# apache/arrow

Hardware: AMD Instinct MI355X
Metric: filter_take_mrows_per_s (higher is better)
Workload: dtype int64; 1 GPU; Filter+Take int64[1000000000] + validity (10% null), boolean mask 10% true, FilterOptions::DROP; take indices = the mask's row numbers (monotonic; indices_nonzero: uint64 through CallFunction, GetTakeIndices: uint32 in the mirror), no boundscheck; inputs = splitmix64 streams of SURVEY.md 8(d) (seeds 1,2,3); rows=1000000000, selected_rows=99992053, parallelism=single-gpu

## Files before the change

### arrow_amd/_lib.py

```python
from __future__ import annotations

import ctypes as C
import os

_HERE = os.path.dirname(os.path.abspath(__file__))
LIB_PATH = os.path.join(_HERE, "libarrow_amd.so")

ARX_OK = 0
ARX_OUT_OF_MEMORY = -1
ARX_INVALID = -4
ARX_CAPACITY_ERROR = -6
ARX_INDEX_ERROR = -7
ARX_NOT_IMPLEMENTED = -10
ARX_DEVICE_ERROR = -100

ABI_VERSION = 5

FILTER_DROP, FILTER_EMIT_NULL = 0, 1
SORT_ASCENDING, SORT_DESCENDING = 0, 1
NULLS_AT_START, NULLS_AT_END = 0, 1


class ArrowAmdError(Exception):
    """Base class; subclasses mirror pyarrow.lib.ArrowInvalid & friends."""


class ArrowInvalid(ArrowAmdError, ValueError):
    pass


class ArrowIndexError(ArrowAmdError, IndexError):
    pass


class ArrowCapacityError(ArrowAmdError):
    pass


class ArrowNotImplementedError(ArrowAmdError, NotImplementedError):
    pass


class ArrowDeviceError(ArrowAmdError, RuntimeError):
    pass


class ArrowMemoryError(ArrowAmdError, MemoryError):
    pass


_ERRORS = {
    ARX_INVALID: ArrowInvalid,
    ARX_CAPACITY_ERROR: ArrowCapacityError,
    ARX_INDEX_ERROR: ArrowIndexError,
    ARX_NOT_IMPLEMENTED: ArrowNotImplementedError,
    ARX_DEVICE_ERROR: ArrowDeviceError,
    ARX_OUT_OF_MEMORY: ArrowMemoryError,
}


class ArxSpan(C.Structure):

    _fields_ = [
        ("validity", C.c_void_p),
        ("data", C.c_void_p),
        ("offset", C.c_int64),
        ("length", C.c_int64),
        ("null_count", C.c_int64),
    ]


class ArxSortKeyWindow(C.Structure):

    _fields_ = [("key_min", C.c_uint64), ("shift", C.c_int32), ("reserved", C.c_int32)]


class ArxRangePlan(C.Structure):

    _fields_ = [("key_min", C.c_int32), ("width", C.c_int32), ("partitions", C.c_int32), ("reserved", C.c_int32),
                ("slots", C.c_int64), ("state_bytes", C.c_uint64), ("workspace_bytes", C.c_uint64)]


class ArxBinarySpan(C.Structure):

    _fields_ = [
        ("validity", C.c_void_p),
        ("offsets", C.c_void_p),
        ("data", C.c_void_p),
        ("offset", C.c_int64),
        ("length", C.c_int64),
        ("null_count", C.c_int64),
    ]


_p, _i64, _int, _u64, _u32, _sz = C.c_void_p, C.c_int64, C.c_int, C.c_uint64, C.c_uint32, C.c_size_t
_span = C.POINTER(ArxSpan)
_bspan = C.POINTER(ArxBinarySpan)

SIGNATURES = {
    "arx_last_error": (C.c_char_p, []),
    "arx_abi_version": (_int, []),
    "arx_device_count": (_int, []),
    "arx_set_option": (_int, [C.c_char_p, _i64]),
    "arx_get_option": (_int, [C.c_char_p, C.POINTER(_i64)]),
    "arx_get_counter": (_i64, [C.c_char_p]),
    "arx_filter_workspace_bytes": (_sz, [_i64]),
    "arx_filter_count": (_int, [_span, _int, _p, _sz, C.POINTER(_i64), _p]),
    "arx_filter_count_async": (_int, [_span, _int, _p, _sz, _p]),
    "arx_filter_count_nulls": (_int, [_span, _span, _int, _p, _sz, C.POINTER(_i64), C.POINTER(_i64), _p]),
    "arx_filter_exec": (_int, [_span, _int, _span, _int, _p, _i64, _p, _p, _p]),
    "arx_mask_to_indices": (_int, [_span, _int, _p, _i64, _int, _p, _p, _p]),
    "arx_filter_compact_form": (_int, [_int, _int, _int, _int, _i64, _i64]),
    "arx_take_workspace_bytes": (_sz, []),
    "arx_check_index_bounds": (_int, [_span, _int, _u64, _p, _sz, _p]),
    "arx_take": (_int, [_span, _int, _span, _int, _p, _p, _p, _p]),
    "arx_take_rows": (_int, [_span, _i64, _span, _int, _p, _p, _p, _p]),
    "arx_take_bits": (_int, [_span, _span, _int, _p, _p, _p, _p]),
    "arx_binary_take_workspace_bytes": (_sz, [_i64]),
    "arx_binary_take_offsets": (_int, [_bspan, _span, _int, _p, _sz, _p, _p, _p, C.POINTER(_i64), _p]),
    "arx_binary_take_data": (_int, [_bspan, _i64, _p, _sz, _p, _i64, _p, _p]),
    "arx_large_binary_take_workspace_bytes": (_sz, [_i64]),
    "arx_large_binary_take_offsets": (_int, [_bspan, _span, _int, _p, _sz, _p, _p, _p, C.POINTER(_i64), _p]),
    "arx_large_binary_take_data": (_int, [_bspan, _i64, _p, _sz, _p, _i64, _p, _p]),
    "arx_list_take_data": (_int, [_bspan, _int, _i64, _p, _sz, _p, _i64, _p, _p]),
    "arx_large_list_take_data": (_int, [_bspan, _int, _i64, _p, _sz, _p, _i64, _p, _p]),
    "arx_plain_byte_array_offsets": (_int, [_p, _sz, _i64, C.c_int32, _p]),
    "arx_rle_scan_runs": (_int, [_p, _sz, _int, _i64, _u32, _u64, _p, _i64, C.POINTER(_i64), C.POINTER(_i64)]),
    "arx_rle_decode_u32": (_int, [_p, _sz, _p, _i64, _int, _i64, _p, _p]),
    "arx_rle_decode_equals_bitmap": (_int, [_p, _sz, _p, _i64, _int, _i64, _u32, _p, _p]),
    "arx_expand_by_mask": (_int, [_p, _int, _span, _p, _p, _p]),
    "arx_rle_levels_to_bitmap": (_int, [_p, _p, _i64, _p, _p, _p, _p]),
    "arx_rle_scan_runs_equals": (_int, [_p, _sz, _int, _i64, _u32, _u32, _u64, _p, _i64, C.POINTER(_i64), C.POINTER(_i64)]),
    "arx_levels_to_list_workspace_bytes": (_sz, [_i64]),
    "arx_def_rep_levels_to_list": (_int, [_p, _p, _i64, _int, _int, _int, _i64, _p, _p, _p, _p, _sz, _p]),
    "arx_levels_ge_bitmap": (_int, [_p, _i64, _u32, _p, _p, _p]),
    "arx_lz4_decompress_streams": (_int, [_p, _p, _p, _i64, _p, _p, _p]),
    "arx_lz4_frame_scan": (_int, [_p, _sz, _u64, _p, _i64, C.POINTER(_i64), C.POINTER(_u64)]),
    "arx_bitmap_copy": (_int, [_p, _i64, _i64, _p, _p]),
    "arx_buffer_copy": (_int, [_p, _p, _i64, _p]),
    "arx_delta_scan_miniblocks": (_int, [_p, _sz, _u64, _p, _i64, C.POINTER(_i64), C.POINTER(_i64), C.POINTER(_i64),
                                         C.POINTER(_i64), C.POINTER(_sz)]),
    "arx_delta_decode_workspace_bytes": (_sz, [_i64]),
    "arx_delta_decode": (_int, [_p, _p, _i64, _i64, _i64, _i64, _int, _p, _sz, _p, _p]),
    "arx_lengths_to_offsets_i32": (_int, [_p, _i64, C.c_int32, _p, _p, _sz, _p]),
    "arx_byte_stream_split_decode": (_int, [_p, _i64, _int, _p, _p]),
    "arx_delta_byte_array_lengths": (_int, [_p, _p, _i64, _p, _i64, _p, _p, _p]),
    "arx_delta_byte_array_expand": (_int, [_p, _p, _p, _i64, _p, C.c_int32, _p, _p, _i64, _p, _p, _p]),
    "arx_bitmap_copy_at": (_int, [_p, _i64, _i64, _p, _i64, _p]),
    "arx_binary_rebase_offsets": (_int, [_p, _i64, C.c_int32, _p, _p]),
    "arx_bitmap_and": (_int, [_p, _i64, _p, _i64, _i64, _p, _p]),
    "arx_reduce_i64_init": (_int, [_p, _p]),
    "arx_reduce_i64_consume": (_int, [_span, _p, _p]),
    "arx_reduce_float_minmax": (_int, [_span, _int, _p, _p]),
    "arx_coalesce2": (_int, [_int, _span, _span, _p, _i64, _p, _p, _p]),
    "arx_sum_float_workspace_bytes": (_sz, [_i64, _i64]),
    "arx_sum_float": (_int, [_span, _int, _p, _sz, C.POINTER(C.c_double), C.POINTER(_i64), _p]),
    "arx_boolean_kleene": (_int, [_int, _span, _span, _p, _p, _p]),
    "arx_boolean_invert": (_int, [_p, _i64, _i64, _p, _p]),
    "arx_bitmap_popcount": (_int, [_p, _i64, _i64, _p, _sz, C.POINTER(_i64), _p]),
    "arx_bytes_to_bitmap": (_int, [_p, _i64, _p, _p, _p]),
    "arx_groupby_key_range_i32": (_int, [_span, _p, _p]),
    "arx_groupby_range_plan": (_int, [_i64, C.c_int32, C.c_int32, _p]),
    "arx_groupby_key_range_sampled_i32": (_int, [_span, _i64, _p, _p]),
    "arx_groupby_range_sum_i64_consume": (_int, [_p, _p, _span, _span, _p, _sz, _p]),
    "arx_groupby_range_merge": (_int, [_p, _p, C.c_int32, _i64, _int, _i64, _p]),
    "arx_groupby_range_finalize_workspace_bytes": (_sz, [_i64]),
    "arx_groupby_range_finalize": (_int, [_p, C.c_int32, C.c_int32, _i64, C.c_uint32, _p, _sz, _p, _p, _p, _p, _p, _p]),
    "arx_hash_bool_finalize": (_int, [_p, _p, _p, _i64, _int, _int, C.c_uint32, _p, _p, _p, _p]),
    "arx_sort_indices_workspace_bytes": (_sz, [_i64]),
    "arx_sort_partition_records_global": (_int, [_span, _int, _int, _int, _p, _p, _int, C.c_uint32, _p, _sz, _p, _p, _p]),
    "arx_sort_records": (_int, [_p, _i64, _p, _sz, _p, _p]),
    "arx_sort_indices": (_int, [_span, _int, _int, _int, _p, _sz, _p, _p]),
    "arx_rank_workspace_bytes": (_sz, [_i64]),
    "arx_rank": (_int, [_span, _int, _p, _int, _p, _sz, _p, _p]),
    "arx_sort_indices_64": (_int, [_span, _int, _int, _int, _p, _sz, _p, _p]),
    "arx_sort_key_histogram": (_int, [_span, _int, _int, _int, _p, _p]),
    "arx_sort_partition_by_bins": (_int, [_span, _int, _int, _int, _p, _int, _p, _sz, _p, _p, _p,
                                          C.POINTER(_i64), _p]),
    "arx_bitmap_to_indices": (_int, [_p, _i64, _i64, _int, _p, _sz, _p, C.POINTER(_i64), _p]),
    "arx_sort_partition_records": (_int, [_span, _int, _int, _int, _int, _p, _int, _p, _sz, _p, _p, C.POINTER(_i64), _p]),
    "arx_sort_key_range": (_int, [_span, _int, _int, _p, _p]),
    "arx_sort_key_histogram_window": (_int, [_span, _int, _int, _int, _p, _p, _p]),
    "arx_sort_key_range_sampled": (_int, [_span, _int, _int, _int, _p, _p]),
    "arx_sort_key_histogram_window_sampled": (_int, [_span, _int, _int, _int, _p, _int, _p, _p]),
    "arx_sort_partition_records_window": (_int, [_span, _int, _int, _int, _int, _p, _p, _int, _p, _sz, _p, _p,
                                                 C.POINTER(_i64), _p]),
    "arx_sort_unpack_records": (_int, [_p, _i64, _p, _int, _int, _p, _p, _p, _p]),
    "arx_groupby_export_partitioned": (_int, [_p, _int, _p, _sz, _p, _p, _p]),
    "arx_groupby_partials_capacity": (_i64, [_i64, _i64, _int]),
    "arx_groupby_sum_i64_consume_partials": (_int, [_p, _i64, _span, _span, _p, _sz, _int, _p, _i64, _p, _p]),
    "arx_groupby_partition_rows": (_int, [_span, _span, _int, _p, _sz, _p, _p, _p]),
    "arx_groupby_unpack_rows": (_int, [_p, _i64, _p, _p, _p, _p, _p]),
    "arx_hash_sum_consume_workspace_bytes": (_sz, [_i64, _i64]),
    "arx_hash_sum_i64_consume_ws": (_int, [_span, _int, _i64, _p, _i64, _i64, _p, _p, _p, _p, _sz, _p]),
    "arx_hash_mean_i64_finalize": (_int, [_p, _p, _i64, C.c_uint64, _p, _p, _p]),
    "arx_compare_numeric": (_int, [_int, _int, _p, _p, _p, _p, _i64, _p, _p]),
    "arx_arith_numeric": (_int, [_int, _int, _int, _p, _p, _p, _i64, _p, _p, _p, _i64, _i64, _p, _p, _p]),
    "arx_divide_numeric": (_int, [_int, _int, _p, _p, _p, _i64, _p, _p, _p, _i64, _i64, _p, _p, _p]),
    "arx_delta_decode_pages": (_int, [_p, _p, _p, _i64, _i64, _int, _p, _sz, _p, _p]),
    "arx_copy_segments": (_int, [_p, _i64, _u64, _p]),
    "arx_bitmap_copy_segments": (_int, [_p, _i64, _i64, _p]),
    "arx_take_columns": (_int, [_p, _p, _int, _span, _int, _p, _p, _p, _p]),
    "arx_grouper_state_bytes": (_sz, [_i64]),
    "arx_grouper_init": (_int, [_p, _i64, _p]),
    "arx_grouper_consume_workspace_bytes": (_sz, [_i64]),
    "arx_grouper_consume": (_int, [_p, _i64, _p, _p, _int, _p, _sz, _p, _p]),
    "arx_grouper_lookup": (_int, [_p, _i64, _p, _p, _int, _p, _sz, _p, _p, _p]),
    "arx_grouper_num_groups": (_int, [_p, _p, _p]),
    "arx_group_ids_skip_group": (_int, [_p, _i64, _u32, _p]),
    "arx_grouper_get_uniques": (_int, [_p, _i64, _p, _int, _int, _p, _p, _p, _p]),
    "arx_binary_key_lengths": (_int, [_bspan, _p, _p, _p, _p]),
    "arx_binary_key_chunk": (_int, [_bspan, _i64, _p, _p, _p]),
    "arx_binary_sort_chunk": (_int, [_bspan, _i64, _p, _p]),
    "arx_binary_key_hash": (_int, [_bspan, _int, _p, _p]),
    "arx_set_lookup_state_bytes": (_sz, [_i64, _int]),
    "arx_set_lookup_build": (_int, [_p, _span, _int, _p]),
    "arx_set_lookup_build_binary": (_int, [_p, _bspan, _int, _int, _p]),
    "arx_set_lookup_is_in": (_int, [_p, _i64, _int, _span, _int, _p, _p]),
    "arx_set_lookup_index_in": (_int, [_p, _i64, _int, _span, _int, _p, _p, _p]),
    "arx_set_lookup_is_in_binary": (_int, [_p, _bspan, _int, _int, _bspan, _int, _int, _p, _p]),
    "arx_set_lookup_index_in_binary": (_int, [_p, _bspan, _int, _int, _bspan, _int, _int, _p, _p, _p]),
    "arx_match_substring": (_int, [_bspan, _int, _int, _p, _i64, _i64, _int, _p, _p]),
    "arx_string_length": (_int, [_bspan, _int, _int, _i64, _int, _p, _p]),
    "arx_string_slice_workspace_bytes": (_sz, [_i64, _int]),
    "arx_string_slice_offsets": (_int, [_bspan, _int, _int, _i64, _i64, _i64, _int, _p, _sz, _p, C.POINTER(_i64), _p]),
    "arx_string_slice_data": (_int, [_bspan, _int, _p, _sz, _p, _i64, _p, _p]),
    "arx_string_trim_offsets": (_int, [_bspan, _int, _int, _int, _p, _i64, _p, _sz, _p, C.POINTER(_i64), _p]),
    "arx_if_else": (_int, [_int, _span, _span, _p, _span, _p, _i64, _p, _p, _p]),
    "arx_temporal_component": (_int, [_int, _int, _span, _i64, _int, _int, _p, _p, _p]),
    "arx_hash_join_workspace_bytes": (_sz, [_i64]),
    "arx_hash_join_key_validity": (_int, [_span, _int, _i64, _p, _p]),
    "arx_hash_join_bool_key": (_int, [_span, _p, _p]),
    "arx_hash_join_group_offsets": (_int, [_p, _p, _i64, _i64, _p, _p, _sz, _p]),
    "arx_hash_join_probe_count": (_int, [_p, _p, _i64, _p, _i64, _int, _p, _i64, _p, _p, _sz, C.POINTER(_i64), _p]),
    "arx_hash_join_expand": (_int, [_p, _p, _p, _i64, _p, _p, _int, _i64, _p, _p, _p, _p]),
    "arx_hash_join_build_mask": (_int, [_p, _p, _i64, _p, _int, _p, _p]),
    "arx_hash_join_append_build_rows": (_int, [_p, _i64, _i64, _p, _p, _p, _p, _p]),
    "arx_hash_join_filter_count": (_int, [_span, _p, _p, _i64, _int, _p, _p, _i64, _p, _p, _p, _p, _sz, C.POINTER(_i64), _p]),
    "arx_hash_join_filter_compact": (_int, [_p, _p, _i64, _p, _p, _i64, _p, _p, _int, _i64, _p, _p, _p, _p]),
    "arx_hash_join_flags_to_mask": (_int, [_p, _i64, _int, _p, _p]),
    "arx_binary_key_verify": (_int, [_bspan, _p, _p, C.POINTER(_i64), _p, _p]),
    "arx_group_first_rows": (_int, [_p, _i64, _i64, _p, _p]),
    "arx_group_edge_rows": (_int, [_p, _p, _i64, _i64, _i64, _int, _p, _p, _p]),
    "arx_ree_bool_expand": (_int, [_p, _int, _i64, _span, _i64, _i64, _p, _p, _p]),
    "arx_snappy_decompress_pages": (_int, [_p, _p, _i64, _p, _p, _p]),
    "arx_gzip_decompress_pages": (_int, [_p, _p, _i64, _p, _p, _p]),
    "arx_cast_numeric": (_int, [_span, _int, _int, _int, _int, _p, _sz, _p, _p]),
    "arx_groupby_mean_i64_finalize": (_int, [_p, _p, _p, _p, _p, _i64, _int, _u32, _p, _p, _p, _p]),
    "arx_groupby_sum_i64_merge_records": (_int, [_p, _i64, _p, _i64, _p]),
    "arx_groupby_state_bytes": (_sz, [_i64]),
    "arx_groupby_init": (_int, [_p, _i64, _p]),
    "arx_groupby_consume_workspace_bytes": (_sz, [_i64, _i64]),
    "arx_groupby_sum_i64_consume": (_int, [_p, _i64, _span, _span, _p, _sz, _p]),
    "arx_groupby_sum_i64_merge": (_int, [_p, _i64, _p, _p, _p, _p, _p, _i64, _p]),
    "arx_groupby_num_groups": (_int, [_p, C.POINTER(_i64), _p]),
    "arx_groupby_sum_i64_export": (_int, [_p, _p, _p, _p, _p, _p, _p]),
    "arx_groupby_lookup_i32": (_int, [_p, _i64, _span, _p, _p]),
    "arx_groupby_minmax_bytes": (_sz, [_i64]),
    "arx_groupby_minmax_init": (_int, [_p, _i64, _p]),
    "arx_groupby_minmax_i64_consume": (_int, [_p, _p, _i64, _span, _span, _p]),
    "arx_groupby_export": (_int, [_p, _p, _p, _p, _p, _p, _p, _p, _p, _p]),
    "arx_groupby_minmax_merge": (_int, [_p, _p, _i64, _p, _p, _p, _p, _p, _i64, _p]),
    "arx_groupby_minmax_finalize": (_int, [_p, _p, _p, _i64, _int, _p, _p]),
    "arx_groupby_sum_i64_finalize": (_int, [_p, _p, _i64, _int, _u32, _p, _p]),
    "arx_hash_sum_i64_consume": (_int, [_span, _int, _i64, _p, _i64, _p, _p, _p, _p]),
    "arx_hash_sum_i64_merge": (_int, [_p, _p, _p, _p, _p, _p, _p, _i64, _p]),
    "arx_hash_sum_dec128_consume": (_int, [_span, _int, C.c_uint64, C.c_uint64, _p, _i64, _p, _p, _p, _p, _p]),
    "arx_hash_sum_dec128_merge": (_int, [_p, _p, _p, _p, _p, _p, _p, _p, _p, _i64, _p]),
# ... 61 lines not shown
```

### arrow_amd/csrc/arrow_plugin.cc

```cpp
#include <arrow/acero/exec_plan.h>
#include <arrow/acero/hash_join_node.h>
#include <arrow/acero/options.h>
#include <arrow/api.h>
#include <arrow/c/abi.h>
#include <arrow/c/bridge.h>
#include <arrow/c/dlpack_abi.h>
#include <arrow/compute/api.h>
#include <arrow/compute/initialize.h>
#include <arrow/compute/kernel.h>
#include <arrow/compute/registry.h>
#include <arrow/device.h>
#include <arrow/util/bit_util.h>
#include <arrow/util/bitmap_builders.h>
#include <arrow/util/bitmap_ops.h>
#include <arrow/acero/util.h>
#include <arrow/acero/query_context.h>

#include <hip/hip_runtime_api.h>
#include <parquet/column_page.h>
#include <parquet/column_reader.h>
#include <parquet/file_reader.h>
#include <parquet/metadata.h>
#include <parquet/schema.h>
#include <parquet/arrow/schema.h>
// ... 398 lines not shown
int64_t arrow_amd_plugin_sharded_sort_records_runs(void) { return g_sharded_sort_records_runs.load(); }
void arrow_amd_plugin_pool_stats(int64_t* cached_bytes, int64_t* hits, int64_t* misses) {
  DevicePool::Get().Stats(cached_bytes, hits, misses);
}
void arrow_amd_plugin_pool_trim(void) { DevicePool::Get().Trim(); }
int arrow_amd_parquet_read_column(const char* path, int row_group, int column, struct ArrowDeviceArray* out,
                                  struct ArrowSchema* out_schema) {
  auto run = [&]() -> Status {
    try {
      ARROW_ASSIGN_OR_RAISE(auto data, ParquetChunkToDevice(path, row_group, column));
      ARROW_RETURN_NOT_OK(arrow::ExportType(*data->type, out_schema));
      return arrow::ExportDeviceArray(*arrow::MakeArray(data), nullptr, out);
    } catch (const parquet::ParquetException& e) {
      return Status::IOError("Parquet: ", e.what());
    }
  };
  const Status st = run();
  if (!st.ok()) {
    t_error = st.ToString();
    return -1;
  }
  return 0;
}
int arrow_amd_parquet_read_field(const char* path, int row_group, int field, struct ArrowDeviceArray* out,
                                 struct ArrowSchema* out_schema) {
  auto run = [&]() -> Status {
    try {
      ARROW_ASSIGN_OR_RAISE(auto data, ParquetFieldToDevice(path, row_group, field));
      ARROW_RETURN_NOT_OK(arrow::ExportType(*data->type, out_schema));
      return arrow::ExportDeviceArray(*arrow::MakeArray(data), nullptr, out);
    } catch (const parquet::ParquetException& e) {
      return Status::IOError("Parquet: ", e.what());
    }
  };
  const Status st = run();
  if (!st.ok()) {
    t_error = st.ToString();
    return -1;
  }
  return 0;
}
namespace {
class ChunkWorkers {
 public:
  static ChunkWorkers& Get() {
#ifdef ARX_EMULATED_HIP_RUNTIME
    static ChunkWorkers* pool = new ChunkWorkers(1);
#else
    static ChunkWorkers* pool = new ChunkWorkers(4);
#endif
    return *pool;
  }
  void Run(int n, const std::function<void(int)>& fn) {
    std::unique_lock<std::mutex> lock(mu_);
    idle_.wait(lock, [&] { return !busy_; });
    busy_ = true;
    fn_ = &fn;
    next_ = 0;
    count_ = n;
    left_ = n;
    work_.notify_all();
    done_.wait(lock, [&] { return left_ == 0; });
    fn_ = nullptr;
    busy_ = false;
    idle_.notify_one();
  }

 private:
  explicit ChunkWorkers(int k) {
    for (int i = 0; i < k; ++i) std::thread([this] { Loop(); }).detach();
  }
  void Loop() {
    std::unique_lock<std::mutex> lock(mu_);
    for (;;) {
      work_.wait(lock, [&] { return fn_ != nullptr && next_ < count_; });
      const int i = next_++;
      const std::function<void(int)>* fn = fn_;
      lock.unlock();
      (*fn)(i);
      lock.lock();
      if (--left_ == 0) done_.notify_all();
    }
  }
  std::mutex mu_;
  std::condition_variable work_, done_, idle_;
  const std::function<void(int)>* fn_ = nullptr;
  int next_ = 0, count_ = 0, left_ = 0;
  bool busy_ = false;
};
}

int arrow_amd_parquet_read_columns(const char* path, int row_group, const int* columns, int num_columns,
                                   struct ArrowDeviceArray* outs, struct ArrowSchema* out_schemas) {
  if (path == nullptr || columns == nullptr || num_columns < 0 || (num_columns > 0 && (outs == nullptr || out_schemas == nullptr))) {
    t_error = "arrow_amd_parquet_read_columns: NULL argument";
    return -1;
  }
  std::vector<arrow::Result<std::shared_ptr<ArrayData>>> results(static_cast<size_t>(num_columns),
                                                                  arrow::Result<std::shared_ptr<ArrayData>>(Status::UnknownError("not run")));
  const std::string file(path);
  int device = 0;
  (void)hipGetDevice(&device);
  ChunkWorkers::Get().Run(num_columns, [&](int i) {
    (void)hipSetDevice(device);
    try {
      results[i] = ParquetChunkToDevice(file, row_group, columns[i]);
    } catch (const parquet::ParquetException& e) {
      results[i] = Status::IOError("Parquet: ", e.what());
    } catch (const std::exception& e) {
      results[i] = Status::UnknownError(e.what());
    }
  });
  for (int i = 0; i < num_columns; ++i) {
    if (!results[i].ok()) {
      t_error = results[i].status().ToString();
      return -1;
    }
  }
  int exported = 0;
  Status st;
  for (; exported < num_columns && st.ok(); ++exported) {
    const std::shared_ptr<ArrayData>& data = *results[exported];
    st = arrow::ExportType(*data->type, &out_schemas[exported]);
    if (st.ok()) {
      st = arrow::ExportDeviceArray(*arrow::MakeArray(data), nullptr, &outs[exported]);
      if (!st.ok() && out_schemas[exported].release != nullptr) out_schemas[exported].release(&out_schemas[exported]);
    }
  }
  if (!st.ok()) {
    for (int i = 0; i + 1 < exported; ++i) {
      if (outs[i].array.release != nullptr) outs[i].array.release(&outs[i].array);
      if (out_schemas[i].release != nullptr) out_schemas[i].release(&out_schemas[i]);
    }
    t_error = st.ToString();
    return -1;
  }
  return 0;
}
int64_t arrow_amd_plugin_acero_guard(int what) {
  return what == 1 ? g_guard_takeovers.load() : what == 2 ? g_guard_refusals.load() : (g_acero_guard_installed.load() ? 1 : 0);
}
int arrow_amd_override_acero_factories(int on) {
  const Status st = OverrideAceroFactories(on);
  if (!st.ok()) {
    t_error = st.ToString();
    return -1;
  }
  return 0;
}
void arrow_amd_plugin_set_min_rows(int64_t n) { g_min_rows.store(n); }
void arrow_amd_plugin_set_string_key_hash_bits(int64_t bits) { g_string_key_hash_bits.store(bits < 0 ? 0 : (bits > 64 ? 64 : bits)); }
int64_t arrow_amd_plugin_string_key_hash_collisions(void) { return g_string_key_hash_collisions.load(); }
void arrow_amd_plugin_set_filter_morsel_rows(int64_t n) { g_filter_morsel_rows.store(n); }
void arrow_amd_plugin_set_parquet_device_snappy(int on) { g_parquet_device_snappy.store(on != 0); }
void arrow_amd_plugin_set_parquet_device_levels(int on) { g_parquet_device_levels.store(on != 0); }
void arrow_amd_plugin_set_parquet_pinned_staging(int on) { g_parquet_pinned_staging.store(on != 0); }
void arrow_amd_plugin_set_parquet_read_threads(int n, int64_t min_part_bytes) {
  g_parquet_read_threads.store(n < 1 ? 1 : (n > 16 ? 16 : n));
  g_parquet_read_part_bytes.store(min_part_bytes < 4096 ? 4096 : min_part_bytes);
}
int64_t arrow_amd_plugin_parquet_device_snappy_pages(void) { return g_parquet_device_snappy_pages.load(); }
void arrow_amd_plugin_set_parquet_device_gzip(int on) { g_parquet_device_gzip.store(on != 0); }
int64_t arrow_amd_plugin_parquet_device_gzip_pages(void) { return g_parquet_device_gzip_pages.load(); }
int64_t arrow_amd_plugin_parquet_copied_pages(void) { return g_parquet_copied_pages.load(); }
void arrow_amd_plugin_set_aggregate_stage_nulls(int on) { g_aggregate_stage_nulls.store(on != 0); }
void arrow_amd_plugin_set_aggregate_flush_rows(int64_t rows) { g_aggregate_flush_rows.store(rows < 1 ? 1 : rows); }
int64_t arrow_amd_plugin_aggregate_flushes(void) { return g_aggregate_flushes.load(); }
void arrow_amd_plugin_set_aggregate_direct_rows(int64_t rows) { g_aggregate_direct_rows.store(rows < 1 ? 1 : rows); }
int64_t arrow_amd_plugin_aggregate_direct_batches(void) { return g_aggregate_direct_batches.load(); }
void arrow_amd_plugin_set_aggregate_range_state(int on) { g_aggregate_range_state.store(on != 0); }
void arrow_amd_plugin_set_aggregate_range_min_rows(int64_t rows) { g_aggregate_range_min_rows.store(rows < 1 ? 1 : rows); }
int64_t arrow_amd_plugin_aggregate_range_plans(void) { return g_aggregate_range_plans.load(); }
int64_t arrow_amd_plugin_aggregate_range_declined(void) { return g_aggregate_range_declined.load(); }
void arrow_amd_plugin_set_aggregate_device_output(int on) { g_aggregate_device_output.store(on != 0); }
void arrow_amd_plugin_set_results_kernel_copy(int on) { g_results_kernel_copy.store(on != 0); }
void arrow_amd_plugin_set_pinned_results(int on) { g_pinned_results.store(on != 0); }
void arrow_amd_plugin_set_coalesce_rows(int64_t rows) { g_coalesce_rows.store(rows < 1 ? 1 : rows); }
int64_t arrow_amd_plugin_coalesced_batches(void) { return g_coalesced_batches.load(); }
void arrow_amd_plugin_set_table_source_rows(int64_t rows) { g_table_source_rows.store(rows < 1 ? 1 : rows); }
void arrow_amd_plugin_set_min_rows_streaming(int64_t n) { g_min_rows_streaming.store(n); }

}
```

### arrow_amd/csrc/plugin/common.inc

```

std::atomic<int64_t> g_gpu_calls{0};
std::atomic<int64_t> g_stock_calls{0};
std::atomic<int64_t> g_min_rows{1 << 16};
std::atomic<int64_t> g_min_rows_streaming{INT64_MAX};
std::atomic<int64_t> g_filter_morsel_rows{[] {
  const char* env = std::getenv("ARROW_AMD_FILTER_MORSEL_ROWS");
  return env != nullptr ? static_cast<int64_t>(std::strtoll(env, nullptr, 10)) : int64_t(1) << 20;
}()};

std::atomic<bool> g_parquet_pinned_staging{true};
std::atomic<bool> g_parquet_device_levels{true};
std::atomic<int> g_parquet_read_threads{4};
std::atomic<int64_t> g_parquet_read_part_bytes{int64_t(1) << 23};
std::atomic<bool> g_parquet_device_snappy{[] {
  const char* env = std::getenv("ARROW_AMD_PARQUET_DEVICE_SNAPPY");
  return env == nullptr || std::strtoll(env, nullptr, 10) != 0;
}()};
std::atomic<int64_t> g_parquet_device_snappy_pages{0};
std::atomic<bool> g_parquet_device_gzip{true};
std::atomic<int64_t> g_parquet_device_gzip_pages{0};
std::atomic<int64_t> g_parquet_copied_pages{0};

std::atomic<int64_t> g_aggregate_flush_rows{[] {
  const char* env = std::getenv("ARROW_AMD_AGGREGATE_FLUSH_ROWS");
  return env != nullptr ? std::max<int64_t>(1, std::strtoll(env, nullptr, 10)) : int64_t(1) << 21;
}()};
std::atomic<int64_t> g_aggregate_direct_rows{int64_t(1) << 22};
std::atomic<int64_t> g_aggregate_direct_batches{0};
std::atomic<bool> g_aggregate_range_state{true};
std::atomic<int64_t> g_aggregate_range_min_rows{int64_t(1) << 22};
std::atomic<int64_t> g_aggregate_range_sample_rows{int64_t(1) << 20};
std::atomic<int64_t> g_aggregate_range_plans{0};
std::atomic<int64_t> g_aggregate_range_declined{0};
std::atomic<int64_t> g_select_k_min_rows{int64_t(1) << 22};
std::atomic<int64_t> g_select_k_threshold_runs{0};
std::atomic<bool> g_sharded_range_state{true};
std::atomic<int64_t> g_sharded_range_min_rows{int64_t(1) << 22};
std::atomic<int64_t> g_sharded_range_runs{0};
std::atomic<int64_t> g_sharded_range_declined{0};
std::atomic<bool> g_sharded_sort_records{true};
std::atomic<int> g_sharded_sort_sample_shift{4};
std::atomic<int64_t> g_sharded_sort_sample_min_rows{int64_t(1) << 20};
std::atomic<int64_t> g_sharded_sort_records_runs{0};
std::atomic<int64_t> g_coalesce_rows{int64_t(1) << 26};
std::atomic<int64_t> g_coalesced_batches{0};
std::atomic<int64_t> g_table_source_rows{int64_t(1) << 27};
std::atomic<bool> g_pinned_results{[] {
  const char* env = std::getenv("ARROW_AMD_PINNED_RESULTS");
  return env == nullptr || std::strtoll(env, nullptr, 10) != 0;
}()};
std::atomic<bool> g_results_kernel_copy{true};
std::atomic<bool> g_aggregate_device_output{false};
std::atomic<bool> g_aggregate_stage_nulls{true};
std::atomic<int64_t> g_aggregate_flushes{0};
std::atomic<int64_t> g_string_key_hash_bits{64};
std::atomic<int64_t> g_string_key_hash_collisions{0};

enum Fn { kFnFilter = 0, kFnTake, kFnGreater, kFnSort, kFnCast, kFnHashSum, kFnAdd, kFnBoolean, kFnCompare, kFnParquet,
          kFnReduce, kFnOrderBy, kFnTakeColumns, kFnUnique, kFnCoalesce, kFnIsIn, kFnIndexIn, kFnHashJoin,
          kFnMatchSubstring, kFnStartsWith, kFnEndsWith, kFnIfElse, kFnYear, kFnQuarter, kFnMonth, kFnDay, kFnDayOfWeek,
          kFnDayOfYear, kFnIsoYear, kFnIsoWeek, kFnHour, kFnMinute, kFnSecond, kFnMillisecond, kFnMicrosecond, kFnNanosecond,
          kFnBinaryLength, kFnUtf8Length, kFnBinarySlice, kFnUtf8SliceCodeunits, kFnAsciiTrimWhitespace, kFnAsciiLtrimWhitespace,
          kFnAsciiRtrimWhitespace, kFnUtf8TrimWhitespace, kFnUtf8LtrimWhitespace, kFnUtf8RtrimWhitespace, kFnAsciiTrim, kFnAsciiLtrim,
          kFnAsciiRtrim, kFnUtf8Trim, kFnUtf8Ltrim, kFnUtf8Rtrim, kNumFn };
const char* const kFnNames[kNumFn] = {"array_filter", "array_take", "greater", "array_sort_indices",
                                      "cast", "hash_sum", "add", "boolean", "compare", "parquet", "reduce", "order_by",
                                      "take_columns", "unique", "coalesce", "is_in", "index_in", "hashjoin",
                                      "match_substring", "starts_with", "ends_with", "if_else", "year", "quarter", "month", "day",
                                      "day_of_week", "day_of_year", "iso_year", "iso_week", "hour", "minute", "second",
                                      "millisecond", "microsecond", "nanosecond", "binary_length", "utf8_length", "binary_slice",
                                      "utf8_slice_codeunits", "ascii_trim_whitespace", "ascii_ltrim_whitespace",
                                      "ascii_rtrim_whitespace", "utf8_trim_whitespace", "utf8_ltrim_whitespace",
                                      "utf8_rtrim_whitespace", "ascii_trim", "ascii_ltrim", "ascii_rtrim", "utf8_trim", "utf8_ltrim",
                                      "utf8_rtrim"};
std::atomic<int64_t> g_fn_gpu[kNumFn];
std::atomic<int64_t> g_fn_stock[kNumFn];
void CountGpu(Fn f) {
  g_gpu_calls.fetch_add(1, std::memory_order_relaxed);
  g_fn_gpu[f].fetch_add(1, std::memory_order_relaxed);
}
void CountStock(Fn f) {
  g_stock_calls.fetch_add(1, std::memory_order_relaxed);
  g_fn_stock[f].fetch_add(1, std::memory_order_relaxed);
}
thread_local std::string t_error;

Status FromArx(int rc) {
  if (rc == ARX_OK) return Status::OK();
  const std::string msg = arx_last_error();
  switch (rc) {
    case ARX_INVALID: return Status::Invalid(msg);
    case ARX_CAPACITY_ERROR: return Status::CapacityError(msg);
    case ARX_INDEX_ERROR: return Status::IndexError(msg);
    case ARX_NOT_IMPLEMENTED: return Status::NotImplemented(msg);
    case ARX_OUT_OF_MEMORY: return Status::OutOfMemory(msg);
    default: return Status::UnknownError(msg);
  }
}

#define HIP_RETURN_NOT_OK(call)                                                        \
  do {                                                                                 \
    hipError_t e__ = (call);                                                           \
    if (e__ != hipSuccess)                                                             \
      return Status::IOError("HIP: ", hipGetErrorString(e__), " in " #call);           \
  } while (0)

thread_local hipStream_t t_stream = nullptr;

class DeviceScratch {
 public:
  ~DeviceScratch() {
    for (auto& s : slots_) {
      if (s.ptr) (void)hipFree(s.ptr);
    }
  }
  hipStream_t PeekStream() const { return stream_; }
  Status Stream(hipStream_t* out) {
    if (!stream_) {
      HIP_RETURN_NOT_OK(hipStreamCreateWithFlags(&stream_, hipStreamNonBlocking));
      t_stream = stream_;
    }
    *out = stream_;
    return Status::OK();
  }
  Status Get(int slot, size_t bytes, void** out) {
    if (slots_.size() <= static_cast<size_t>(slot)) slots_.resize(slot + 1);
    Slot& s = slots_[slot];
    bytes = (bytes + 255) & ~size_t(255);
    if (s.size < bytes) {
      if (s.ptr) HIP_RETURN_NOT_OK(hipFree(s.ptr));
      s.ptr = nullptr;
      s.size = 0;
      const size_t want = std::max<size_t>(bytes + bytes / 4, 1 << 20);
      HIP_RETURN_NOT_OK(hipMalloc(&s.ptr, want));
      s.size = want;
    }
    *out = s.ptr;
    return Status::OK();
  }

 private:
  struct Slot { void* ptr = nullptr; size_t size = 0; };
  std::vector<Slot> slots_;
  hipStream_t stream_ = nullptr;
};
thread_local DeviceScratch t_scratch;

class PinnedStaging {
 public:
  ~PinnedStaging() {
    if (ptr_) (void)hipHostFree(ptr_);
  }
  Status Reserve(size_t bytes, uint8_t** out) {
    if (size_ < bytes) {
      if (ptr_) HIP_RETURN_NOT_OK(hipHostFree(ptr_));
      ptr_ = nullptr;
      size_ = 0;
      const size_t want = std::max<size_t>(bytes + bytes / 4, size_t(1) << 20);
      HIP_RETURN_NOT_OK(hipHostMalloc(&ptr_, want, hipHostMallocDefault));
      size_ = want;
    }
    *out = static_cast<uint8_t*>(ptr_);
    return Status::OK();
  }
  void Trim(size_t keep_at_most) {
    if (size_ > keep_at_most && ptr_ != nullptr) {
      (void)hipHostFree(ptr_);
      ptr_ = nullptr;
      size_ = 0;
    }
  }

 private:
  void* ptr_ = nullptr;
  size_t size_ = 0;
};
thread_local PinnedStaging t_pinned;

enum Slot { kValues = 0, kValidity, kArg2, kArg2Validity, kOutData, kOutValidity, kWs, kCounter, kBinWs, kFlag };

Status Upload(const ArraySpan& a, int byte_width_or_0_for_bool, int data_slot, int validity_slot,
              hipStream_t st, ArxSpan* out) {
  const int64_t o8 = a.offset % 8;
  const int64_t first = a.offset - o8;
  out->offset = o8;
  out->length = a.length;
  out->null_count = a.null_count;
  out->validity = nullptr;
  out->data = nullptr;
  const int64_t span_elems = o8 + a.length;
  if (a.buffers[1].data != nullptr && a.length > 0) {
    const uint8_t* src;
    size_t bytes;
    if (byte_width_or_0_for_bool == 0) {
      src = a.buffers[1].data + first / 8;
      bytes = static_cast<size_t>(arrow::bit_util::BytesForBits(span_elems));
    } else {
      src = a.buffers[1].data + first * byte_width_or_0_for_bool;
      bytes = static_cast<size_t>(span_elems) * byte_width_or_0_for_bool;
    }
    void* d = nullptr;
    ARROW_RETURN_NOT_OK(t_scratch.Get(data_slot, bytes + 16, &d));
    HIP_RETURN_NOT_OK(hipMemcpyAsync(d, src, bytes, hipMemcpyHostToDevice, st));
    out->data = d;
  }
  if (a.buffers[0].data != nullptr && a.null_count != 0 && a.length > 0) {
    const size_t bytes = static_cast<size_t>(arrow::bit_util::BytesForBits(span_elems));
    void* d = nullptr;
    ARROW_RETURN_NOT_OK(t_scratch.Get(validity_slot, bytes + 16, &d));
    HIP_RETURN_NOT_OK(hipMemcpyAsync(d, a.buffers[0].data + first / 8, bytes, hipMemcpyHostToDevice, st));
    out->validity = d;
  } else if (a.null_count != 0 && a.buffers[0].data == nullptr) {
    out->null_count = 0;
  }
  return Status::OK();
}

bool IsHost(const ArraySpan& a) {
  for (int i = 0; i < 2; ++i) {
    if (a.buffers[i].owner != nullptr && *a.buffers[i].owner != nullptr &&
        !(*a.buffers[i].owner)->is_cpu()) {
      return false;
    }
  }
  return true;
}

int FixedByteWidth(const arrow::DataType& t) {
  switch (t.id()) {
    case Type::INT8: case Type::UINT8: return 1;
    case Type::INT16: case Type::UINT16: case Type::HALF_FLOAT: return 2;
    case Type::INT32: case Type::UINT32: case Type::FLOAT: case Type::DATE32: case Type::TIME32:
    case Type::INTERVAL_MONTHS: case Type::DECIMAL32: return 4;
    case Type::INT64: case Type::UINT64: case Type::DOUBLE: case Type::DATE64: case Type::TIME64:
    case Type::TIMESTAMP: case Type::DURATION: case Type::INTERVAL_DAY_TIME: case Type::DECIMAL64: return 8;
    case Type::DECIMAL128: case Type::INTERVAL_MONTH_DAY_NANO: return 16;
    case Type::DECIMAL256: return 32;
    case Type::FIXED_SIZE_BINARY: {
      const int w = static_cast<const arrow::FixedSizeBinaryType&>(t).byte_width();
      return (w == 1 || w == 2 || w == 4 || w == 8 || w == 16 || w == 32) ? w : 0;
    }
    default: return 0;
  }
}

int BinaryOffsetWidth(Type::type id) { return (id == Type::LARGE_STRING || id == Type::LARGE_BINARY) ? 8 : 4; }

template <typename Options>
struct ShimState : public cp::KernelState {
  std::unique_ptr<cp::KernelState> stock;
  Options options;
};

struct StockKernel {
  cp::KernelInit init;
  cp::ArrayKernelExec exec = nullptr;
  cp::VectorKernel::ChunkedExec exec_chunked = nullptr;
};

template <class Exec, class Batch, class Out>
Status RunStock(Fn fn, Exec exec, std::optional<cp::KernelState*> stock_state, cp::KernelContext* ctx, const Batch& batch,
                Out* out) {
  CountStock(fn);
  if (!stock_state.has_value()) return exec(ctx, batch, out);
  cp::KernelState* mine = ctx->state();
  ctx->SetState(*stock_state);
  Status st = exec(ctx, batch, out);
  ctx->SetState(mine);
  return st;
}
Status RunStock(Fn fn, const StockKernel& k, cp::KernelState* stock_state, cp::KernelContext* ctx,
                const cp::ExecSpan& batch, cp::ExecResult* out) {
  return RunStock(fn, k.exec, std::optional<cp::KernelState*>(stock_state), ctx, batch, out);
}
```

### arrow_amd/csrc/plugin/selection.inc

```
StockKernel g_stock_filter;

arrow::Result<std::unique_ptr<cp::KernelState>> FilterInit(cp::KernelContext* ctx,
                                                           const cp::KernelInitArgs& args) {
  auto state = std::make_unique<ShimState<cp::FilterOptions>>();
  if (g_stock_filter.init) {
    ARROW_ASSIGN_OR_RAISE(state->stock, g_stock_filter.init(ctx, args));
  }
  if (args.options != nullptr) {
    state->options = *static_cast<const cp::FilterOptions*>(args.options);
  }
  return state;
}

Status BooleanTakeOnDevice(const ArxSpan& dv, const ArxSpan& di, int tid, hipStream_t st, ArrayData* out_arr) {
  const int64_t m = di.length;
  const int64_t bytes = ((m + 63) / 64) * 8;
  const bool allocate_validity = dv.null_count != 0 || di.null_count != 0;
  out_arr->length = m;
  out_arr->buffers.resize(2);
  out_arr->buffers[0] = nullptr;
  ARROW_ASSIGN_OR_RAISE(out_arr->buffers[1], AllocDevice(bytes));
  void* d_valid = nullptr;
  void* d_counter = nullptr;
  if (allocate_validity) {
    ARROW_ASSIGN_OR_RAISE(out_arr->buffers[0], AllocDevice(bytes));
    d_valid = reinterpret_cast<void*>(out_arr->buffers[0]->mutable_address());
    ARROW_RETURN_NOT_OK(t_scratch.Get(kCounter, 64, &d_counter));
    HIP_RETURN_NOT_OK(hipMemsetAsync(d_counter, 0, 8, st));
  }
  ARROW_RETURN_NOT_OK(FromArx(arx_take_bits(&dv, &di, tid, reinterpret_cast<void*>(out_arr->buffers[1]->mutable_address()),
                                            d_valid, static_cast<int64_t*>(d_counter), st)));
  int64_t valid_count = m;
  if (allocate_validity) HIP_RETURN_NOT_OK(hipMemcpyAsync(&valid_count, d_counter, 8, hipMemcpyDeviceToHost, st));
  HIP_RETURN_NOT_OK(hipStreamSynchronize(st));
  out_arr->null_count = m - valid_count;
  return Status::OK();
}

bool ReeFilterOnRocm(const ArraySpan& filter) {
  return filter.type->id() == Type::RUN_END_ENCODED && filter.child_data.size() == 2 &&
         OnRocm(filter.child_data[0]) && OnRocm(filter.child_data[1]);
}
Status ExpandReeFilterOnDevice(const ArraySpan& filter, hipStream_t st, ArxSpan* dm) {
  const ArraySpan& run_ends = filter.child_data[0];
  const ArraySpan& run_values = filter.child_data[1];
  const int rw = FixedByteWidth(*run_ends.type);
  if (run_values.type->id() != Type::BOOL || (rw != 2 && rw != 4 && rw != 8)) {
    return Status::NotImplemented("arrow_amd: filter of type ", filter.type->ToString());
  }
  ArxSpan ends{}, vals{};
  ARROW_RETURN_NOT_OK(DeviceSpan(run_ends, &ends));
  ARROW_RETURN_NOT_OK(DeviceSpan(run_values, &vals));
  const int64_t n = filter.length;
  const size_t bytes = static_cast<size_t>((n + 63) / 64) * 8 + 64;
  void *d_bits = nullptr, *d_valid = nullptr;
  ARROW_RETURN_NOT_OK(t_scratch.Get(kArg2, bytes, &d_bits));
  const bool may_have_nulls = vals.validity != nullptr && vals.null_count != 0;
  if (may_have_nulls) ARROW_RETURN_NOT_OK(t_scratch.Get(kArg2Validity, bytes, &d_valid));
  ARROW_RETURN_NOT_OK(FromArx(arx_ree_bool_expand(static_cast<const uint8_t*>(ends.data) + ends.offset * rw, rw, run_ends.length,
                                                  &vals, filter.offset, n, d_bits, d_valid, st)));
  *dm = ArxSpan{d_valid, d_bits, 0, n, may_have_nulls ? arrow::kUnknownNullCount : 0};
  return Status::OK();
}

Status FilterExec(cp::KernelContext* ctx, const cp::ExecSpan& batch, cp::ExecResult* out) {
  auto* state = static_cast<ShimState<cp::FilterOptions>*>(ctx->state());
  const ArraySpan& values = batch[0].array;
  const ArraySpan& filter = batch[1].array;
  const int w = FixedByteWidth(*values.type);
  const int null_sel = state->options.null_selection_behavior == cp::FilterOptions::EMIT_NULL
                           ? ARX_FILTER_EMIT_NULL : ARX_FILTER_DROP;
  const bool ree = filter.type->id() == Type::RUN_END_ENCODED;
  const bool on_device = OnRocm(values) || OnRocm(filter) || (ree && ReeFilterOnRocm(filter));
  if (on_device && ree && (!OnRocm(values) || !ReeFilterOnRocm(filter))) {
    return Status::NotImplemented("arrow_amd: a run-end encoded filter and its values must both be device-resident");
  }
  if (on_device) {
    if (values.type->id() == Type::BOOL && ree) {
      return Status::NotImplemented("arrow_amd: run-end encoded filter of boolean values on device-resident arrays");
    }
    if (values.type->id() == Type::BOOL && filter.type->id() == Type::BOOL) {
      if (filter.length > 0xFFFFFFFFll) {
        return Status::NotImplemented("Filter length exceeds UINT32_MAX, consider a different strategy for selecting elements");
      }
      hipStream_t st;
      ARROW_RETURN_NOT_OK(t_scratch.Stream(&st));
      ArxSpan dv{}, dm{};
      ARROW_RETURN_NOT_OK(DeviceSpan(values, &dv));
      ARROW_RETURN_NOT_OK(DeviceSpan(filter, &dm));
      const size_t ws_bytes = arx_filter_workspace_bytes(filter.length);
      void* ws = nullptr;
      ARROW_RETURN_NOT_OK(t_scratch.Get(kWs, ws_bytes, &ws));
      int64_t out_len = 0;
      ARROW_RETURN_NOT_OK(FromArx(arx_filter_count(&dm, null_sel, ws, ws_bytes, &out_len, st)));
      const bool emit = null_sel == ARX_FILTER_EMIT_NULL && dm.null_count != 0;
      void* d_idx = nullptr;
      void* d_idx_valid = nullptr;
      ARROW_RETURN_NOT_OK(t_scratch.Get(kArg2, static_cast<size_t>(out_len) * 4 + 64, &d_idx));
      if (emit) ARROW_RETURN_NOT_OK(t_scratch.Get(kArg2Validity, static_cast<size_t>((out_len + 63) / 64) * 8 + 64, &d_idx_valid));
      ARROW_RETURN_NOT_OK(FromArx(arx_mask_to_indices(&dm, null_sel, ws, out_len, 4, d_idx, d_idx_valid, st)));
      ArxSpan di{d_idx_valid, d_idx, 0, out_len, emit ? arrow::kUnknownNullCount : 0};
      ARROW_RETURN_NOT_OK(BooleanTakeOnDevice(dv, di, ARX_UINT32, st, out->array_data().get()));
      CountGpu(kFnFilter);
      return Status::OK();
    }
    if (w == 0 || (filter.type->id() != Type::BOOL && !ree)) {
      return Status::NotImplemented("arrow_amd: filter of ", values.type->ToString(),
                                    " on device-resident arrays");
    }
    hipStream_t st;
    ARROW_RETURN_NOT_OK(t_scratch.Stream(&st));
    ArxSpan dv{}, dm{};
    ARROW_RETURN_NOT_OK(DeviceSpan(values, &dv));
    if (ree) {
      ARROW_RETURN_NOT_OK(ExpandReeFilterOnDevice(filter, st, &dm));
    } else {
      ARROW_RETURN_NOT_OK(DeviceSpan(filter, &dm));
    }
    const size_t ws_bytes = arx_filter_workspace_bytes(filter.length);
    void* ws = nullptr;
    ARROW_RETURN_NOT_OK(t_scratch.Get(kWs, ws_bytes, &ws));
    ArrayData* out_arr = out->array_data().get();
    const bool allocate_validity = dv.null_count != 0 || dm.null_count != 0;
    if (filter.length > 0 && filter.length <= g_filter_morsel_rows.load()) {
      const int64_t n = filter.length;
      ARROW_RETURN_NOT_OK(FromArx(arx_filter_count_async(&dm, null_sel, ws, ws_bytes, st)));
      out_arr->buffers.resize(2);
      ARROW_ASSIGN_OR_RAISE(out_arr->buffers[1], AllocDevice(n * w));
      out_arr->buffers[0] = nullptr;
      void* d_valid = nullptr;
      if (allocate_validity) {
        ARROW_ASSIGN_OR_RAISE(out_arr->buffers[0], AllocDevice(((n + 63) / 64) * 8));
        d_valid = reinterpret_cast<void*>(out_arr->buffers[0]->mutable_address());
      }
      ARROW_RETURN_NOT_OK(FromArx(arx_filter_exec(&dv, w, &dm, null_sel, ws, n,
                                                  reinterpret_cast<void*>(out_arr->buffers[1]->mutable_address()),
                                                  d_valid, st)));
      int64_t selected = 0, set_bits = 0;
      HIP_RETURN_NOT_OK(hipMemcpyAsync(&selected, ws, 8, hipMemcpyDeviceToHost, st));
      if (allocate_validity) {
        void* cws = nullptr;
        ARROW_RETURN_NOT_OK(t_scratch.Get(kCounter, 64, &cws));
        ARROW_RETURN_NOT_OK(FromArx(arx_bitmap_popcount(d_valid, 0, n, cws, 64, &set_bits, st)));
      } else {
        HIP_RETURN_NOT_OK(hipStreamSynchronize(st));
      }
      out_arr->length = selected;
      out_arr->null_count = allocate_validity ? selected - set_bits : 0;
      static_cast<RocmBuffer*>(out_arr->buffers[1].get())->Shrink(selected * w);
      if (allocate_validity) static_cast<RocmBuffer*>(out_arr->buffers[0].get())->Shrink(((selected + 63) / 64) * 8);
      CountGpu(kFnFilter);
      return Status::OK();
    }
    int64_t out_len = 0, out_nulls = 0;
    if (allocate_validity) {
      ARROW_RETURN_NOT_OK(FromArx(arx_filter_count_nulls(&dv, &dm, null_sel, ws, ws_bytes, &out_len, &out_nulls, st)));
    } else {
      ARROW_RETURN_NOT_OK(FromArx(arx_filter_count(&dm, null_sel, ws, ws_bytes, &out_len, st)));
    }
    out_arr->length = out_len;
    out_arr->buffers.resize(2);
    ARROW_ASSIGN_OR_RAISE(out_arr->buffers[1], AllocDevice(out_len * w));
    out_arr->buffers[0] = nullptr;
    void* d_valid = nullptr;
    if (allocate_validity) {
      ARROW_ASSIGN_OR_RAISE(out_arr->buffers[0], AllocDevice(((out_len + 63) / 64) * 8));
      d_valid = reinterpret_cast<void*>(out_arr->buffers[0]->mutable_address());
    }
    ARROW_RETURN_NOT_OK(FromArx(arx_filter_exec(&dv, w, &dm, null_sel, ws, out_len,
                                                reinterpret_cast<void*>(out_arr->buffers[1]->mutable_address()),
                                                d_valid, st)));
    out_arr->null_count = allocate_validity ? out_nulls : 0;
    HIP_RETURN_NOT_OK(hipStreamSynchronize(st));
    CountGpu(kFnFilter);
    return Status::OK();
  }
  if (w == 0 || filter.type->id() != Type::BOOL || values.length < g_min_rows.load() ||
      !IsHost(values) || !IsHost(filter)) {
    return RunStock(kFnFilter, g_stock_filter, state->stock.get(), ctx, batch, out);
  }
  hipStream_t st;
  ARROW_RETURN_NOT_OK(t_scratch.Stream(&st));
  ArxSpan dv{}, dm{};
  ARROW_RETURN_NOT_OK(Upload(values, w, kValues, kValidity, st, &dv));
  ARROW_RETURN_NOT_OK(Upload(filter, 0, kArg2, kArg2Validity, st, &dm));
  const size_t ws_bytes = arx_filter_workspace_bytes(filter.length);
  void* ws = nullptr;
  ARROW_RETURN_NOT_OK(t_scratch.Get(kWs, ws_bytes, &ws));
  int64_t out_len = 0;
  ARROW_RETURN_NOT_OK(FromArx(arx_filter_count(&dm, null_sel, ws, ws_bytes, &out_len, st)));

  ArrayData* out_arr = out->array_data().get();
  const bool filter_null_count_is_zero = filter.null_count == 0;
  if (values.null_count == 0 && (null_sel == ARX_FILTER_DROP || filter_null_count_is_zero)) {
    out_arr->null_count = 0;
  } else {
    out_arr->null_count = arrow::kUnknownNullCount;
  }
  const bool allocate_validity = values.null_count != 0 || !filter_null_count_is_zero;
  out_arr->length = out_len;
  out_arr->buffers.resize(2);
  ARROW_ASSIGN_OR_RAISE(out_arr->buffers[1], ctx->Allocate(out_len * w));
  void* d_out = nullptr;
  void* d_out_valid = nullptr;
  ARROW_RETURN_NOT_OK(t_scratch.Get(kOutData, static_cast<size_t>(out_len) * w + 16, &d_out));
  const size_t vbytes = static_cast<size_t>((out_len + 63) / 64) * 8;
  if (allocate_validity) {
    ARROW_ASSIGN_OR_RAISE(out_arr->buffers[0], ctx->AllocateBitmap(out_len));
    ARROW_RETURN_NOT_OK(t_scratch.Get(kOutValidity, vbytes + 16, &d_out_valid));
  } else {
    out_arr->buffers[0] = nullptr;
  }
  ARROW_RETURN_NOT_OK(FromArx(arx_filter_exec(&dv, w, &dm, null_sel, ws, out_len, d_out, d_out_valid, st)));
  if (out_len > 0) {
    HIP_RETURN_NOT_OK(hipMemcpyAsync(out_arr->buffers[1]->mutable_data(), d_out,
                                     static_cast<size_t>(out_len) * w, hipMemcpyDeviceToHost, st));
    if (allocate_validity) {
      HIP_RETURN_NOT_OK(hipMemcpyAsync(out_arr->buffers[0]->mutable_data(), d_out_valid,
                                       static_cast<size_t>(arrow::bit_util::BytesForBits(out_len)),
                                       hipMemcpyDeviceToHost, st));
    }
  }
  HIP_RETURN_NOT_OK(hipStreamSynchronize(st));
  CountGpu(kFnFilter);
  return Status::OK();
}

int IndexTypeId(const arrow::DataType& t);

StockKernel g_stock_filter_bin, g_stock_take_bin, g_stock_filter_large_bin, g_stock_take_large_bin;

arrow::Result<std::unique_ptr<cp::KernelState>> BinaryFilterInit(cp::KernelContext* ctx,
                                                                 const cp::KernelInitArgs& args) {
  auto state = std::make_unique<ShimState<cp::FilterOptions>>();
  const bool large_in = !args.inputs.empty() && args.inputs[0].type != nullptr && BinaryOffsetWidth(args.inputs[0].type->id()) == 8;
  const StockKernel& stock_k = large_in ? g_stock_filter_large_bin : g_stock_filter_bin;
  if (stock_k.init) {
    ARROW_ASSIGN_OR_RAISE(state->stock, stock_k.init(ctx, args));
  }
  if (args.options != nullptr) state->options = *static_cast<const cp::FilterOptions*>(args.options);
  return state;
}

arrow::Result<std::unique_ptr<cp::KernelState>> BinaryTakeInit(cp::KernelContext* ctx,
                                                               const cp::KernelInitArgs& args) {
  auto state = std::make_unique<ShimState<cp::TakeOptions>>();
  const bool large_in = !args.inputs.empty() && args.inputs[0].type != nullptr && BinaryOffsetWidth(args.inputs[0].type->id()) == 8;
  const StockKernel& stock_k = large_in ? g_stock_take_large_bin : g_stock_take_bin;
  if (stock_k.init) {
    ARROW_ASSIGN_OR_RAISE(state->stock, stock_k.init(ctx, args));
  }
  if (args.options != nullptr) state->options = *static_cast<const cp::TakeOptions*>(args.options);
  return state;
}

Status CheckBoundsOnDevice(const ArxSpan& indices, int index_type, int64_t values_length, hipStream_t st) {
  void* ws = nullptr;
  ARROW_RETURN_NOT_OK(t_scratch.Get(kWs, arx_take_workspace_bytes(), &ws));
  return FromArx(arx_check_index_bounds(&indices, index_type, static_cast<uint64_t>(values_length), ws,
                                        arx_take_workspace_bytes(), st));
}

bool OnRocm3(const ArraySpan& a) {
  if (OnRocm(a)) return true;
  return a.buffers[2].owner != nullptr && *a.buffers[2].owner != nullptr &&
         (*a.buffers[2].owner)->device_type() == arrow::DeviceAllocationType::kROCM;
}

Status DeviceBinarySpan(const ArraySpan& a, ArxBinarySpan* out) {
  const void* addr[3] = {nullptr, nullptr, nullptr};
  for (int i = 0; i < 3; ++i) {
    const auto* owner = a.buffers[i].owner;
    if (owner == nullptr || *owner == nullptr) continue;
    if ((*owner)->device_type() != arrow::DeviceAllocationType::kROCM) {
      return Status::Invalid("arrow_amd: mixed host / device buffers in one array");
    }
    addr[i] = reinterpret_cast<const void*>((*owner)->address());
  }
  out->validity = addr[0];
  out->offsets = static_cast<const int32_t*>(addr[1]);
  out->data = addr[2];
  out->offset = a.offset;
  out->length = a.length;
  out->null_count = addr[0] == nullptr ? 0 : (a.null_count > 0 ? a.null_count : arrow::kUnknownNullCount);
  return Status::OK();
}

Status BinaryTakeOnDevice(const ArxBinarySpan& dv, const ArxSpan& di, int tid, hipStream_t st, ArrayData* out_arr, bool large = false) {
  const int64_t m = di.length;
  const bool allocate_validity = dv.null_count != 0 || di.null_count != 0;
  out_arr->length = m;
  out_arr->buffers.resize(3);
  out_arr->buffers[0] = nullptr;
  ARROW_ASSIGN_OR_RAISE(out_arr->buffers[1], AllocDevice((m + 1) * (large ? 8 : 4)));
  void* d_valid = nullptr;
  void* d_counter = nullptr;
  if (allocate_validity) {
    ARROW_ASSIGN_OR_RAISE(out_arr->buffers[0], AllocDevice(((m + 63) / 64) * 8));
    d_valid = reinterpret_cast<void*>(out_arr->buffers[0]->mutable_address());
    ARROW_RETURN_NOT_OK(t_scratch.Get(kCounter, 64, &d_counter));
    HIP_RETURN_NOT_OK(hipMemsetAsync(d_counter, 0, 8, st));
  }
  const size_t ws_bytes = large ? arx_large_binary_take_workspace_bytes(m) : arx_binary_take_workspace_bytes(m);
  void* ws = nullptr;
  ARROW_RETURN_NOT_OK(t_scratch.Get(kBinWs, ws_bytes, &ws));
  void* d_off = reinterpret_cast<void*>(out_arr->buffers[1]->mutable_address());
  int64_t total = 0;
  if (large) {
    ARROW_RETURN_NOT_OK(FromArx(arx_large_binary_take_offsets(&dv, &di, tid, ws, ws_bytes, static_cast<int64_t*>(d_off), d_valid,
                                                              static_cast<int64_t*>(d_counter), &total, st)));
  } else {
    ARROW_RETURN_NOT_OK(FromArx(arx_binary_take_offsets(&dv, &di, tid, ws, ws_bytes, static_cast<int32_t*>(d_off), d_valid,
                                                        static_cast<int64_t*>(d_counter), &total, st)));
  }
  ARROW_ASSIGN_OR_RAISE(out_arr->buffers[2], AllocDevice(total));
  void* d_data = reinterpret_cast<void*>(out_arr->buffers[2]->mutable_address());
  if (large) {
    ARROW_RETURN_NOT_OK(FromArx(arx_large_binary_take_data(&dv, m, ws, ws_bytes, static_cast<const int64_t*>(d_off), total, d_data, st)));
  } else {
    ARROW_RETURN_NOT_OK(FromArx(arx_binary_take_data(&dv, m, ws, ws_bytes, static_cast<const int32_t*>(d_off), total, d_data, st)));
  }
  int64_t valid_count = m;
  if (allocate_validity) {
    HIP_RETURN_NOT_OK(hipMemcpyAsync(&valid_count, d_counter, 8, hipMemcpyDeviceToHost, st));
  }
  HIP_RETURN_NOT_OK(hipStreamSynchronize(st));
  out_arr->null_count = m - valid_count;
  return Status::OK();
}

bool IsInt32Binary(const arrow::DataType& t) { return t.id() == Type::STRING || t.id() == Type::BINARY; }

Status BinaryTakeExec(cp::KernelContext* ctx, const cp::ExecSpan& batch, cp::ExecResult* out) {
  auto* state = static_cast<ShimState<cp::TakeOptions>*>(ctx->state());
  const ArraySpan& values = batch[0].array;
  const ArraySpan& indices = batch[1].array;
  if (!OnRocm3(values) && !OnRocm(indices)) {
    return RunStock(kFnTake, BinaryOffsetWidth(values.type->id()) == 8 ? g_stock_take_large_bin : g_stock_take_bin, state->stock.get(), ctx, batch, out);
  }
  const int tid = IndexTypeId(*indices.type);
  const bool large = BinaryOffsetWidth(values.type->id()) == 8;
  if (tid < 0 || !(IsInt32Binary(*values.type) || large)) {
    return Status::NotImplemented("arrow_amd: take of ", values.type->ToString(), " by ",
                                  indices.type->ToString(), " on device-resident arrays");
  }
  hipStream_t st;
  ARROW_RETURN_NOT_OK(t_scratch.Stream(&st));
  ArxBinarySpan dv{};
  ArxSpan di{};
  ARROW_RETURN_NOT_OK(DeviceBinarySpan(values, &dv));
  ARROW_RETURN_NOT_OK(DeviceSpan(indices, &di));
  if (state->options.boundscheck) ARROW_RETURN_NOT_OK(CheckBoundsOnDevice(di, tid, values.length, st));
  ARROW_RETURN_NOT_OK(BinaryTakeOnDevice(dv, di, tid, st, out->array_data().get(), large));
  CountGpu(kFnTake);
  return Status::OK();
}

Status BinaryFilterExec(cp::KernelContext* ctx, const cp::ExecSpan& batch, cp::ExecResult* out) {
  auto* state = static_cast<ShimState<cp::FilterOptions>*>(ctx->state());
  const ArraySpan& values = batch[0].array;
  const ArraySpan& filter = batch[1].array;
  if (!OnRocm3(values) && !OnRocm(filter)) {
    return RunStock(kFnFilter, BinaryOffsetWidth(values.type->id()) == 8 ? g_stock_filter_large_bin : g_stock_filter_bin, state->stock.get(), ctx, batch, out);
  }
  const bool large = BinaryOffsetWidth(values.type->id()) == 8;
  if (filter.type->id() != Type::BOOL || !(IsInt32Binary(*values.type) || large)) {
    return Status::NotImplemented("arrow_amd: filter of ", values.type->ToString(), " on device-resident arrays");
  }
  if (filter.length > 0xFFFFFFFFll) {
    return Status::NotImplemented("Filter length exceeds UINT32_MAX, consider a different strategy for selecting elements");
  }
  const int null_sel = state->options.null_selection_behavior == cp::FilterOptions::EMIT_NULL
                           ? ARX_FILTER_EMIT_NULL : ARX_FILTER_DROP;
  hipStream_t st;
  ARROW_RETURN_NOT_OK(t_scratch.Stream(&st));
  ArxBinarySpan dv{};
  ArxSpan dm{};
  ARROW_RETURN_NOT_OK(DeviceBinarySpan(values, &dv));
  ARROW_RETURN_NOT_OK(DeviceSpan(filter, &dm));
  const size_t ws_bytes = arx_filter_workspace_bytes(filter.length);
  void* ws = nullptr;
  ARROW_RETURN_NOT_OK(t_scratch.Get(kWs, ws_bytes, &ws));
  int64_t out_len = 0;
  ARROW_RETURN_NOT_OK(FromArx(arx_filter_count(&dm, null_sel, ws, ws_bytes, &out_len, st)));
  const bool emit = null_sel == ARX_FILTER_EMIT_NULL && dm.null_count != 0;
  void* d_idx = nullptr;
  void* d_idx_valid = nullptr;
  ARROW_RETURN_NOT_OK(t_scratch.Get(kArg2, static_cast<size_t>(out_len) * 4 + 64, &d_idx));
  if (emit) ARROW_RETURN_NOT_OK(t_scratch.Get(kArg2Validity, static_cast<size_t>((out_len + 63) / 64) * 8 + 64, &d_idx_valid));
  ARROW_RETURN_NOT_OK(FromArx(arx_mask_to_indices(&dm, null_sel, ws, out_len, 4, d_idx, d_idx_valid, st)));
  ArxSpan di{d_idx_valid, d_idx, 0, out_len, emit ? arrow::kUnknownNullCount : 0};
  ARROW_RETURN_NOT_OK(BinaryTakeOnDevice(dv, di, ARX_UINT32, st, out->array_data().get(), large));
  CountGpu(kFnFilter);
  return Status::OK();
}

StockKernel g_stock_take;

arrow::Result<std::unique_ptr<cp::KernelState>> TakeInit(cp::KernelContext* ctx,
                                                         const cp::KernelInitArgs& args) {
  auto state = std::make_unique<ShimState<cp::TakeOptions>>();
  if (g_stock_take.init) {
    ARROW_ASSIGN_OR_RAISE(state->stock, g_stock_take.init(ctx, args));
  }
  if (args.options != nullptr) state->options = *static_cast<const cp::TakeOptions*>(args.options);
  return state;
}

int IndexTypeId(const arrow::DataType& t) {
  switch (t.id()) {
    case Type::UINT8: return ARX_UINT8;
    case Type::INT8: return ARX_INT8;
    case Type::UINT16: return ARX_UINT16;
    case Type::INT16: return ARX_INT16;
    case Type::UINT32: return ARX_UINT32;
    case Type::INT32: return ARX_INT32;
    case Type::UINT64: return ARX_UINT64;
    case Type::INT64: return ARX_INT64;
    default: return -1;
  }
}

Status TakeExec(cp::KernelContext* ctx, const cp::ExecSpan& batch, cp::ExecResult* out) {
  auto* state = static_cast<ShimState<cp::TakeOptions>*>(ctx->state());
  const ArraySpan& values = batch[0].array;
  const ArraySpan& indices = batch[1].array;
  const int w = FixedByteWidth(*values.type);
  const int tid = IndexTypeId(*indices.type);
  static const int kIdxWidth[8] = {1, 1, 2, 2, 4, 4, 8, 8};
  if (OnRocm(values) || OnRocm(indices)) {
    if (values.type->id() == Type::BOOL && tid >= 0) {
      hipStream_t st;
      ARROW_RETURN_NOT_OK(t_scratch.Stream(&st));
      ArxSpan dv{}, di{};
      ARROW_RETURN_NOT_OK(DeviceSpan(values, &dv));
      ARROW_RETURN_NOT_OK(DeviceSpan(indices, &di));
      if (state->options.boundscheck) ARROW_RETURN_NOT_OK(CheckBoundsOnDevice(di, tid, values.length, st));
      ARROW_RETURN_NOT_OK(BooleanTakeOnDevice(dv, di, tid, st, out->array_data().get()));
      CountGpu(kFnTake);
      return Status::OK();
    }
    if (w == 0 || tid < 0) {
      return Status::NotImplemented("arrow_amd: take of ", values.type->ToString(), " by ",
                                    indices.type->ToString(), " on device-resident arrays");
    }
    hipStream_t st;
    ARROW_RETURN_NOT_OK(t_scratch.Stream(&st));
    ArxSpan dv{}, di{};
    ARROW_RETURN_NOT_OK(DeviceSpan(values, &dv));
    ARROW_RETURN_NOT_OK(DeviceSpan(indices, &di));
    if (state->options.boundscheck) ARROW_RETURN_NOT_OK(CheckBoundsOnDevice(di, tid, values.length, st));
    const int64_t m = indices.length;
    const bool allocate_validity = dv.null_count != 0 || di.null_count != 0;
    ArrayData* out_arr = out->array_data().get();
    out_arr->length = m;
    out_arr->buffers.resize(2);
    ARROW_ASSIGN_OR_RAISE(out_arr->buffers[1], AllocDevice(m * w));
    out_arr->buffers[0] = nullptr;
    void* d_valid = nullptr;
    void* d_counter = nullptr;
    if (allocate_validity) {
      ARROW_ASSIGN_OR_RAISE(out_arr->buffers[0], AllocDevice(((m + 63) / 64) * 8));
      d_valid = reinterpret_cast<void*>(out_arr->buffers[0]->mutable_address());
      ARROW_RETURN_NOT_OK(t_scratch.Get(kCounter, 64, &d_counter));
      HIP_RETURN_NOT_OK(hipMemsetAsync(d_counter, 0, 8, st));
    }
    ARROW_RETURN_NOT_OK(FromArx(arx_take(&dv, w, &di, tid,
                                         reinterpret_cast<void*>(out_arr->buffers[1]->mutable_address()), d_valid,
                                         static_cast<int64_t*>(d_counter), st)));
    int64_t valid_count = m;
    if (allocate_validity) {
      HIP_RETURN_NOT_OK(hipMemcpyAsync(&valid_count, d_counter, 8, hipMemcpyDeviceToHost, st));
    }
    HIP_RETURN_NOT_OK(hipStreamSynchronize(st));
    out_arr->null_count = m - valid_count;
    CountGpu(kFnTake);
    return Status::OK();
  }
  if (w == 0 || tid < 0 || indices.length < g_min_rows.load() || !IsHost(values) || !IsHost(indices)) {
    return RunStock(kFnTake, g_stock_take, state->stock.get(), ctx, batch, out);
  }
  hipStream_t st;
  ARROW_RETURN_NOT_OK(t_scratch.Stream(&st));
  ArxSpan dv{}, di{};
  ARROW_RETURN_NOT_OK(Upload(values, w, kValues, kValidity, st, &dv));
  ARROW_RETURN_NOT_OK(Upload(indices, kIdxWidth[tid], kArg2, kArg2Validity, st, &di));
  if (state->options.boundscheck) ARROW_RETURN_NOT_OK(CheckBoundsOnDevice(di, tid, values.length, st));
  const int64_t m = indices.length;
  const bool allocate_validity = values.MayHaveNulls() || indices.MayHaveNulls();
  ArrayData* out_arr = out->array_data().get();
  out_arr->length = m;
  out_arr->buffers.resize(2);
  ARROW_ASSIGN_OR_RAISE(out_arr->buffers[1], ctx->Allocate(m * w));
  void* d_out = nullptr;
  void* d_out_valid = nullptr;
  void* d_counter = nullptr;
  ARROW_RETURN_NOT_OK(t_scratch.Get(kOutData, static_cast<size_t>(m) * w + 16, &d_out));
  if (allocate_validity) {
    ARROW_ASSIGN_OR_RAISE(out_arr->buffers[0], ctx->AllocateBitmap(m));
    ARROW_RETURN_NOT_OK(t_scratch.Get(kOutValidity, static_cast<size_t>((m + 63) / 64) * 8 + 16, &d_out_valid));
    ARROW_RETURN_NOT_OK(t_scratch.Get(kCounter, 64, &d_counter));
    HIP_RETURN_NOT_OK(hipMemsetAsync(d_counter, 0, 8, st));
  } else {
    out_arr->buffers[0] = nullptr;
  }
  ARROW_RETURN_NOT_OK(FromArx(arx_take(&dv, w, &di, tid, d_out, d_out_valid,
                                       static_cast<int64_t*>(d_counter), st)));
  HIP_RETURN_NOT_OK(hipMemcpyAsync(out_arr->buffers[1]->mutable_data(), d_out, static_cast<size_t>(m) * w,
                                   hipMemcpyDeviceToHost, st));
  int64_t valid_count = m;
  if (allocate_validity) {
    HIP_RETURN_NOT_OK(hipMemcpyAsync(out_arr->buffers[0]->mutable_data(), d_out_valid,
                                     static_cast<size_t>(arrow::bit_util::BytesForBits(m)),
                                     hipMemcpyDeviceToHost, st));
    HIP_RETURN_NOT_OK(hipMemcpyAsync(&valid_count, d_counter, 8, hipMemcpyDeviceToHost, st));
  }
  HIP_RETURN_NOT_OK(hipStreamSynchronize(st));
  out_arr->null_count = m - valid_count;
  CountGpu(kFnTake);
  return Status::OK();
}
```

### arrow_amd/csrc/plugin/vector_hash.inc

```
enum HashVectorKind { kHashUnique = 0, kHashValueCounts, kHashDictEncode };

struct DeviceHashState : public cp::KernelState {
  HashVectorKind kind = kHashUnique;
  std::unique_ptr<cp::KernelState> stock;
  bool used_stock = false, used_device = false;
  bool encode_nulls = false;
  std::shared_ptr<arrow::DataType> type;
  int width = 0;
  std::shared_ptr<Buffer> table_buf, counts_buf;
  void* table = nullptr;
  int64_t max_groups = 0, num_groups = 0, counts_cap = 0;
};

StockKernel g_stock_unique, g_stock_value_counts, g_stock_dict_encode;
cp::VectorKernel::FinalizeFunc g_stock_unique_finalize = nullptr, g_stock_value_counts_finalize = nullptr,
                               g_stock_dict_encode_finalize = nullptr;

template <HashVectorKind KIND>
const StockKernel& StockHashKernel() {
  return KIND == kHashUnique ? g_stock_unique : KIND == kHashValueCounts ? g_stock_value_counts : g_stock_dict_encode;
}

Status HashUniques(DeviceHashState* s, hipStream_t st, std::shared_ptr<Buffer>* values, std::shared_ptr<Buffer>* validity,
                   int64_t* null_count) {
// ... 163 lines not shown

Status CompactByBitmap(const ArxSpan& dv, int width, const void* mask_bits, int64_t mask_offset, int64_t n, hipStream_t st,
                       std::shared_ptr<Buffer>* out_values, std::shared_ptr<Buffer>* out_validity, int64_t* out_length,
                       int64_t* out_null_count) {
  ArxSpan dm{nullptr, mask_bits, mask_offset, n, 0};
  const size_t ws_bytes = arx_filter_workspace_bytes(n);
  void* ws = nullptr;
  ARROW_RETURN_NOT_OK(t_scratch.Get(kWs, ws_bytes, &ws));
  int64_t out_len = 0;
  ARROW_RETURN_NOT_OK(FromArx(arx_filter_count(&dm, ARX_FILTER_DROP, ws, ws_bytes, &out_len, st)));
  ARROW_ASSIGN_OR_RAISE(*out_values, AllocDevice(std::max<int64_t>(out_len, 1) * width));
  void* d_valid = nullptr;
  *out_validity = nullptr;
  if (dv.validity != nullptr && dv.null_count != 0) {
    ARROW_ASSIGN_OR_RAISE(*out_validity, AllocDevice(((out_len + 63) / 64) * 8 + 8));
    d_valid = reinterpret_cast<void*>((*out_validity)->mutable_address());
  }
  ARROW_RETURN_NOT_OK(FromArx(arx_filter_exec(&dv, width, &dm, ARX_FILTER_DROP, ws, out_len,
                                              reinterpret_cast<void*>((*out_values)->mutable_address()), d_valid, st)));
  *out_length = out_len;
  *out_null_count = 0;
  if (d_valid != nullptr) {
    ARROW_ASSIGN_OR_RAISE(*out_null_count, DeviceNullCount(**out_validity, out_len, st));
  }
  HIP_RETURN_NOT_OK(hipStreamSynchronize(st));
  return Status::OK();
}

arrow::Result<std::shared_ptr<ArrayData>> HashDictionary(DeviceHashState* s, bool drop_null, hipStream_t st, int64_t* null_id) {
  std::shared_ptr<Buffer> values, validity;
  int64_t nulls = 0;
  ARROW_RETURN_NOT_OK(HashUniques(s, st, &values, &validity, &nulls));
  HIP_RETURN_NOT_OK(hipStreamSynchronize(st));
  const int64_t g = s->num_groups;
  *null_id = -1;
  if (nulls == 0) return ArrayData::Make(s->type, g, {nullptr, std::move(values)}, 0);
  if (!drop_null) return ArrayData::Make(s->type, g, {std::move(validity), std::move(values)}, nulls);
  void* d_idx = nullptr;
  ARROW_RETURN_NOT_OK(t_scratch.Get(kArg2, 256, &d_idx));
  {
    ARROW_ASSIGN_OR_RAISE(auto inv, AllocDevice(((g + 63) / 64) * 8 + 8));
    ARROW_RETURN_NOT_OK(FromArx(arx_boolean_invert(reinterpret_cast<const void*>(validity->address()), 0, g,
                                                   reinterpret_cast<void*>(inv->mutable_address()), st)));
    ArxSpan dm{nullptr, reinterpret_cast<const void*>(inv->address()), 0, g, 0};
    const size_t ws_bytes = arx_filter_workspace_bytes(g);
    void* ws = nullptr;
    ARROW_RETURN_NOT_OK(t_scratch.Get(kWs, ws_bytes, &ws));
    int64_t cnt = 0;
    ARROW_RETURN_NOT_OK(FromArx(arx_filter_count(&dm, ARX_FILTER_DROP, ws, ws_bytes, &cnt, st)));
    if (cnt != 1) return Status::Invalid("arrow_amd: internal error (", cnt, " null entries among the unique values)");
    ARROW_RETURN_NOT_OK(FromArx(arx_mask_to_indices(&dm, ARX_FILTER_DROP, ws, cnt, 4, d_idx, nullptr, st)));
    uint32_t pos = 0;
    HIP_RETURN_NOT_OK(hipMemcpyAsync(&pos, d_idx, 4, hipMemcpyDeviceToHost, st));
    HIP_RETURN_NOT_OK(hipStreamSynchronize(st));
    *null_id = pos;
  }
  ArxSpan dv{nullptr, reinterpret_cast<const void*>(values->address()), 0, g, 0};
  std::shared_ptr<Buffer> kept, kept_validity;
  int64_t kept_len = 0, kept_nulls = 0;
  ARROW_RETURN_NOT_OK(CompactByBitmap(dv, s->width, reinterpret_cast<const void*>(validity->address()), 0, g, st, &kept,
                                      &kept_validity, &kept_len, &kept_nulls));
  return ArrayData::Make(s->type, kept_len, {nullptr, std::move(kept)}, 0);
}

class RocmDropNullMetaFunction : public cp::MetaFunction {
 public:
  explicit RocmDropNullMetaFunction(std::shared_ptr<cp::Function> stock)
      : cp::MetaFunction("drop_null", cp::Arity::Unary(), stock->doc()), stock_(std::move(stock)) {}

  arrow::Result<arrow::Datum> ExecuteImpl(const std::vector<arrow::Datum>& args, const cp::FunctionOptions* options,
                                          cp::ExecContext* ctx) const override {
    if (args.size() == 1 && args[0].is_array() && DataOnRocm(*args[0].array())) {
      const ArrayData& in = *args[0].array();
      const int w = FixedByteWidth(*in.type);
      if (w == 0) return Status::NotImplemented("arrow_amd: drop_null of device-resident ", in.type->ToString(), " arrays");
      if (in.buffers[0] == nullptr || in.null_count.load() == 0 || in.length == 0) return args[0];
      hipStream_t st;
      ARROW_RETURN_NOT_OK(t_scratch.Stream(&st));
      ArxSpan dv{};
      ARROW_RETURN_NOT_OK(DeviceSpan(ArraySpan(in), &dv));
      const void* bits = dv.validity;
      dv.validity = nullptr;
      dv.null_count = 0;
      std::shared_ptr<Buffer> values, validity;
      int64_t len = 0, nulls = 0;
      ARROW_RETURN_NOT_OK(CompactByBitmap(dv, w, bits, in.offset, in.length, st, &values, &validity, &len, &nulls));
      CountGpu(kFnFilter);
      return arrow::Datum(ArrayData::Make(in.type, len, {nullptr, std::move(values)}, 0));
    }
    return stock_->Execute(args, options, ctx);
  }

 private:
  std::shared_ptr<cp::Function> stock_;
};

StockKernel g_stock_nonzero;

int NonZeroNumericTypeId(Type::type id) {
  switch (id) {
    case Type::INT8: return ARX_NUM_INT8;
    case Type::UINT8: return ARX_NUM_UINT8;
    case Type::INT16: return ARX_NUM_INT16;
    case Type::UINT16: return ARX_NUM_UINT16;
    case Type::INT32: return ARX_NUM_INT32;
    case Type::UINT32: return ARX_NUM_UINT32;
    case Type::INT64: return ARX_NUM_INT64;
    case Type::UINT64: return ARX_NUM_UINT64;
    case Type::FLOAT: return ARX_NUM_FLOAT32;
    case Type::DOUBLE: return ARX_NUM_FLOAT64;
    default: return -1;
  }
}

Status IndicesNonZeroExecRocm(cp::KernelContext* ctx, const cp::ExecSpan& batch, cp::ExecResult* out) {
  const ArraySpan& in = batch[0].array;
  if (!OnRocm(in)) {
    CountStock(kFnFilter);
    return g_stock_nonzero.exec(ctx, batch, out);
  }
  const int64_t n = in.length;
  if (n > 0xFFFFFFFFll) return Status::NotImplemented("arrow_amd: indices_nonzero of more than UINT32_MAX device rows");
  hipStream_t st;
  ARROW_RETURN_NOT_OK(t_scratch.Stream(&st));
  ArxSpan dv{};
  ARROW_RETURN_NOT_OK(DeviceSpan(in, &dv));
  ArxSpan dm{dv.validity, nullptr, dv.offset, n, dv.null_count};
  std::shared_ptr<Buffer> bits, rebased;
  if (in.type->id() == Type::BOOL) {
    dm.data = dv.data;
  } else {
    const int num = NonZeroNumericTypeId(in.type->id());
    if (num < 0) return Status::NotImplemented("arrow_amd: indices_nonzero of device-resident ", in.type->ToString(), " arrays");
    static const int widths[10] = {1, 1, 2, 2, 4, 4, 8, 8, 4, 8};
    ARROW_ASSIGN_OR_RAISE(bits, AllocDevice(((n + 63) / 64) * 8 + 8));
    const uint64_t zero = 0;
    const uint8_t* base = static_cast<const uint8_t*>(dv.data) + dv.offset * widths[num];
    if (n > 0) {
      ARROW_RETURN_NOT_OK(FromArx(arx_compare_numeric(ARX_CMP_NOT_EQUAL, num, base, nullptr, nullptr, &zero, n,
                                                      reinterpret_cast<uint64_t*>(bits->mutable_address()), st)));
    }
    dm.data = reinterpret_cast<const void*>(bits->address());
    dm.offset = 0;
    if (dm.validity != nullptr && dv.offset != 0) {
      ARROW_ASSIGN_OR_RAISE(rebased, AllocDevice(((n + 63) / 64) * 8 + 8));
      ARROW_RETURN_NOT_OK(FromArx(arx_bitmap_copy(dv.validity, dv.offset, n, reinterpret_cast<void*>(rebased->mutable_address()), st)));
      dm.validity = reinterpret_cast<const void*>(rebased->address());
    }
  }
  const size_t ws_bytes = arx_filter_workspace_bytes(n);
  void* ws = nullptr;
  ARROW_RETURN_NOT_OK(t_scratch.Get(kWs, ws_bytes, &ws));
  int64_t cnt = 0;
  if (n > 0) ARROW_RETURN_NOT_OK(FromArx(arx_filter_count(&dm, ARX_FILTER_DROP, ws, ws_bytes, &cnt, st)));
  void* d_idx = nullptr;
  ARROW_RETURN_NOT_OK(t_scratch.Get(kArg2, static_cast<size_t>(cnt) * 4 + 64, &d_idx));
  ARROW_ASSIGN_OR_RAISE(auto out_values, AllocDevice(std::max<int64_t>(cnt, 1) * 8));
  bool direct = false;
  if (cnt > 0) {
    direct = arx_mask_to_indices(&dm, ARX_FILTER_DROP, ws, cnt, 8, reinterpret_cast<void*>(out_values->mutable_address()), nullptr, st) == ARX_OK;
  }
  if (cnt > 0 && !direct) {
    ARROW_RETURN_NOT_OK(FromArx(arx_mask_to_indices(&dm, ARX_FILTER_DROP, ws, cnt, 4, d_idx, nullptr, st)));
    ArxSpan di{nullptr, d_idx, 0, cnt, 0};
    void* flag = nullptr;
    ARROW_RETURN_NOT_OK(t_scratch.Get(kFlag, 64, &flag));
    ARROW_RETURN_NOT_OK(FromArx(arx_cast_numeric(&di, ARX_NUM_UINT32, ARX_NUM_UINT64, 1, 1, flag, 64,
                                                 reinterpret_cast<void*>(out_values->mutable_address()), st)));
  }
  HIP_RETURN_NOT_OK(hipStreamSynchronize(st));
  CountGpu(kFnFilter);
  out->value = ArrayData::Make(arrow::uint64(), cnt, {nullptr, std::move(out_values)}, 0);
  return Status::OK();
}

Status RegisterIndicesNonZero(cp::FunctionRegistry* reg) {
  ARROW_ASSIGN_OR_RAISE(auto fn, reg->GetFunction("indices_nonzero"));
  if (fn->kind() != cp::Function::VECTOR) return Status::Invalid("indices_nonzero is not a vector function");
  auto* vfn = static_cast<cp::VectorFunction*>(fn.get());
  for (const auto& ty : {arrow::boolean(), arrow::int8(), arrow::uint8(), arrow::int16(), arrow::uint16(), arrow::int32(),
                         arrow::uint32(), arrow::int64(), arrow::uint64(), arrow::float32(), arrow::float64()}) {
    ARROW_ASSIGN_OR_RAISE(const cp::Kernel* k0, vfn->DispatchExact({ty}));
    cp::VectorKernel copy = *static_cast<const cp::VectorKernel*>(k0);
    if (g_stock_nonzero.exec == nullptr) g_stock_nonzero.exec = copy.exec;
    if (g_stock_nonzero.exec != copy.exec) continue;
    copy.exec = IndicesNonZeroExecRocm;
    ARROW_RETURN_NOT_OK(vfn->AddKernel(std::move(copy)));
  }
  return Status::OK();
}

struct HashValueType {
  std::shared_ptr<arrow::DataType> probe;
  cp::InputType match;
};
std::vector<HashValueType> HashVectorTypes() {
  using arrow::TimeUnit;
  std::vector<HashValueType> t;
  for (const auto& ty : {arrow::int8(), arrow::uint8(), arrow::int16(), arrow::uint16(), arrow::int32(), arrow::uint32(),
                         arrow::int64(), arrow::uint64(), arrow::float32(), arrow::float64(), arrow::date32(), arrow::date64()}) {
    t.push_back({ty, cp::InputType(ty)});
  }
  t.push_back({arrow::time32(TimeUnit::SECOND), cp::InputType(Type::TIME32)});
  t.push_back({arrow::time64(TimeUnit::NANO), cp::InputType(Type::TIME64)});
  t.push_back({arrow::timestamp(TimeUnit::NANO), cp::InputType(Type::TIMESTAMP)});
  t.push_back({arrow::duration(TimeUnit::NANO), cp::InputType(Type::DURATION)});
  return t;
}

template <HashVectorKind KIND>
Status RegisterHashVector(cp::FunctionRegistry* reg, const char* name, StockKernel* stock,
                          cp::VectorKernel::FinalizeFunc* stock_finalize) {
  ARROW_ASSIGN_OR_RAISE(auto fn, reg->GetFunction(name));
  if (fn->kind() != cp::Function::VECTOR) return Status::Invalid(name, " is not a vector function");
  auto* vfn = static_cast<cp::VectorFunction*>(fn.get());
  const std::vector<HashValueType> types = HashVectorTypes();
  for (const auto& vt : types) {
    ARROW_ASSIGN_OR_RAISE(const cp::Kernel* k0, vfn->DispatchExact({vt.probe}));
    cp::VectorKernel copy = *static_cast<const cp::VectorKernel*>(k0);
    if (stock->exec == nullptr) {
      stock->exec = copy.exec;
      *stock_finalize = copy.finalize;
    } else if (stock->exec != copy.exec) {
      continue;
    }
    stock->init = nullptr;
    const cp::KernelInit stock_init = copy.init;
    copy.init = [stock_init](cp::KernelContext* ctx, const cp::KernelInitArgs& args)
        -> arrow::Result<std::unique_ptr<cp::KernelState>> {
      auto state = std::make_unique<DeviceHashState>();
      state->kind = KIND;
      state->type = args.inputs[0].GetSharedPtr();
      state->width = FixedByteWidth(*state->type);
      if (KIND == kHashDictEncode && args.options != nullptr) {
        state->encode_nulls = static_cast<const cp::DictionaryEncodeOptions*>(args.options)->null_encoding_behavior ==
                              cp::DictionaryEncodeOptions::ENCODE;
      }
      ARROW_ASSIGN_OR_RAISE(state->stock, stock_init(ctx, args));
      return state;
    };
    copy.signature = cp::KernelSignature::Make({vt.match}, copy.signature->out_type());
    copy.exec = HashVectorExec<KIND>;
    copy.finalize = HashVectorFinalize<KIND>;
    copy.mem_allocation = cp::MemAllocation::NO_PREALLOCATE;
    ARROW_RETURN_NOT_OK(vfn->AddKernel(std::move(copy)));
  }
  return Status::OK();
}
```

### arrow_amd/csrc/selection.hip

```cpp
#include "arx_common.h"

#include <string.h>

#include <algorithm>
#include <type_traits>

namespace arx {

struct FilterWsHeader {
  int64_t total;
  int64_t ntiles;
  int64_t ngroups;
  int64_t length;
  int64_t valid;
  int64_t pad[3];
};
static_assert(sizeof(FilterWsHeader) == 64, "header is one 64-byte line");

struct FilterWsView {
  FilterWsHeader* hdr;
  int64_t* group_excl;
  int64_t* group_total;
  uint32_t* tile_counts;
  int64_t* group_valid;
};

static inline int64_t num_tiles(int64_t length) { return ceil_div(length, kTileRows); }
static inline int64_t num_groups(int64_t length) {
  return ceil_div(num_tiles(length), kTilesPerGroup);
}

static inline FilterWsView ws_view(void* ws, int64_t length) {
  FilterWsView v;
  const int64_t ng = num_groups(length);
  uint8_t* p = static_cast<uint8_t*>(ws);
  v.hdr = reinterpret_cast<FilterWsHeader*>(p);
  v.group_excl = reinterpret_cast<int64_t*>(p + 64);
  v.group_total = v.group_excl + ng;
  v.tile_counts = reinterpret_cast<uint32_t*>(v.group_total + ng);
  v.group_valid = reinterpret_cast<int64_t*>(v.tile_counts + ng * kTilesPerGroup);
  return v;
}

__device__ __forceinline__ uint64_t emit_word(const Bits& mask, const Bits& mvalid, int64_t w,
                                              bool emit_null, bool invert,
                                              uint64_t* mask_valid_out) {
  uint64_t m = load_word(mask, w);
  const uint64_t mv = load_word(mvalid, w);
  *mask_valid_out = mv;
  if (emit_null || invert) {
    const uint64_t in_range = load_word(Bits{nullptr, 0, mask.length, 0}, w);
    if (invert) m = ~m & in_range;
    if (emit_null) return (m | ~mv) & in_range;
  }
  return m & mv;
}

template <bool VALID>
__global__ __launch_bounds__(kBlock) void count_kernel(Bits mask, Bits mvalid, Bits vvalid, int emit_null,
                                                       int invert, int64_t ntiles,
                                                       uint32_t* tile_counts,
                                                       int64_t* group_total, int64_t* group_valid) {
  __shared__ uint32_t wave_sums[kWavesPerBlock];
  __shared__ uint32_t wave_valid[kWavesPerBlock];
  const int lane = lane_id();
  const int wave = threadIdx.x >> 6;
  const int64_t group = blockIdx.x;
  const int64_t t0 = group * kTilesPerGroup + wave * 16;
  uint32_t mine = 0;
  uint32_t kv = 0;
#pragma unroll 4
  for (int i = 0; i < 16; ++i) {
    const int64_t t = t0 + i;
    uint32_t k = 0;
    if (t < ntiles) {
      uint64_t mv;
      const uint64_t e = emit_word(mask, mvalid, t * 64 + lane, emit_null != 0, invert != 0, &mv);
      k = __popcll(e);
      if constexpr (VALID) kv += __popcll(e & mv & load_word(vvalid, t * 64 + lane));
    }
    const uint32_t s = wave_reduce_sum_u32(k);
    if (lane == i) mine = s;
  }
  if (lane < 16) tile_counts[t0 + lane] = mine;
  const uint32_t wsum = wave_reduce_sum_u32(lane < 16 ? mine : 0u);
  if (lane == 0) wave_sums[wave] = wsum;
  if constexpr (VALID) {
    const uint32_t vsum = wave_reduce_sum_u32(kv);
    if (lane == 0) wave_valid[wave] = vsum;
  }
  __syncthreads();
  if (threadIdx.x == 0) {
    int64_t s = 0, v = 0;
    for (int i = 0; i < kWavesPerBlock; ++i) {
      s += wave_sums[i];
      if constexpr (VALID) v += wave_valid[i];
    }
    group_total[group] = s;
    if constexpr (VALID) group_valid[group] = v;
  }
}

__global__ __launch_bounds__(1024) void scan_kernel(const int64_t* group_total, int64_t ngroups,
                                                    int64_t* group_excl, FilterWsHeader* hdr,
                                                    const int64_t* group_valid = nullptr) {
  __shared__ int64_t wave_tot[16];
  __shared__ int64_t carry_s;
  __shared__ unsigned long long valid_s;
  const int tid = threadIdx.x;
  const int lane = tid & 63;
  const int wave = tid >> 6;
  if (tid == 0) carry_s = 0;
  if (tid == 0) valid_s = 0;
  __syncthreads();
  if (group_valid != nullptr) {
    int64_t mine = 0;
    for (int64_t i = tid; i < ngroups; i += 1024) mine += group_valid[i];
#pragma unroll
    for (int d = 32; d >= 1; d >>= 1) mine += __shfl_xor(mine, d, 64);
    if (lane == 0 && mine != 0) atomicAdd(&valid_s, static_cast<unsigned long long>(mine));
    __syncthreads();
  }
  for (int64_t base = 0; base < ngroups; base += 1024) {
    const int64_t i = base + tid;
    const int64_t v = i < ngroups ? group_total[i] : 0;
    int64_t x = v;
#pragma unroll
    for (int d = 1; d < 64; d <<= 1) {
      const int64_t n = __shfl_up(x, d, 64);
      if (lane >= d) x += n;
    }
    if (lane == 63) wave_tot[wave] = x;
    __syncthreads();
    int64_t wave_prefix = 0;
    for (int k = 0; k < wave; ++k) wave_prefix += wave_tot[k];
    const int64_t carry = carry_s;
    if (i < ngroups) group_excl[i] = carry + wave_prefix + x - v;
    __syncthreads();
    if (tid == 1023) carry_s = carry + wave_prefix + x;
    __syncthreads();
  }
  if (tid == 0) {
    hdr->total = carry_s;
    hdr->valid = static_cast<int64_t>(valid_s);
  }
}

struct CompactArgs {
  const uint8_t* values;
  Bits mask;
  Bits mvalid;
  Bits vvalid;
  int64_t length;
  int64_t ntiles;
  const uint32_t* tile_counts;
  const int64_t* group_excl;
  uint8_t* out_data;
  uint64_t* out_validity;
  int emit_null;
  int invert;
  int values_aligned16;
};

constexpr int kFlushBytes = 2048;

template <int RING>
struct __attribute__((aligned(16))) CompactLds {
  uint8_t ring[kWavesPerBlock][RING];
  uint64_t vbits[kWavesPerBlock][72];
};

template <int W>
struct ElemT;
template <> struct ElemT<1> { using type = uint8_t; };
template <> struct ElemT<2> { using type = uint16_t; };
template <> struct ElemT<4> { using type = uint32_t; };
template <> struct ElemT<8> { using type = uint64_t; };
template <> struct ElemT<16> { using type = uint4; };
struct Elem32 { uint4 lo, hi; };
template <> struct ElemT<32> { using type = Elem32; };

template <int W>
__device__ __forceinline__ typename ElemT<W>::type zero_elem() {
  if constexpr (W == 32) {
    return Elem32{make_uint4(0, 0, 0, 0), make_uint4(0, 0, 0, 0)};
  } else if constexpr (W == 16) {
    return make_uint4(0, 0, 0, 0);
  } else {
    return 0;
  }
}

constexpr int kSelNt = 3;

template <int W>
__device__ __forceinline__ typename ElemT<W>::type sel_load(const typename ElemT<W>::type* p, bool nt) {
  using E = typename ElemT<W>::type;
  if constexpr (W == 32) {
    return *p;
  } else if constexpr (W == 16) {
    return nt ? nt_load16(p) : *p;
  } else {
    return nt ? nt_load<E>(p) : *p;
  }
}
template <int W>
__device__ __forceinline__ void sel_store(typename ElemT<W>::type* p, typename ElemT<W>::type v) {
  using E = typename ElemT<W>::type;
  if constexpr (W == 32) {
    *p = v;
  } else if constexpr (W == 16) {
    if constexpr ((kSelNt & 2) != 0) nt_store16(p, v); else *p = v;
  } else {
    if constexpr ((kSelNt & 2) != 0) nt_store<E>(p, v); else *p = v;
  }
}

__device__ __forceinline__ void wave_lds_sync() {
  __builtin_amdgcn_fence(__ATOMIC_RELEASE, "wavefront");
  __builtin_amdgcn_wave_barrier();
  __builtin_amdgcn_fence(__ATOMIC_ACQUIRE, "wavefront");
}

template <int W, int RING>
__device__ __forceinline__ void flush_region(const uint8_t* ring, uint8_t* gbase, int64_t F,
                                             int64_t lo, int64_t hi, int lane) {
  using E = typename ElemT<W>::type;
  constexpr int R = 16 / W;
  const int ring_off = static_cast<int>(F & (RING - 1));
#pragma unroll
  for (int h = 0; h < kFlushBytes / (16 * kWave); ++h) {
    const int g = h * kWave + lane;
    const int64_t gs = F + g * 16;
    const int64_t ge = gs + 16;
    if (ge <= lo || gs >= hi) continue;
    const uint8_t* src = ring + ring_off + g * 16;
    uint8_t* dst = gbase + gs;
    if (gs >= lo && ge <= hi) {
      sel_store<16>(reinterpret_cast<uint4*>(dst), *reinterpret_cast<const uint4*>(src));
    } else {
#pragma unroll
      for (int e = 0; e < R; ++e) {
        const int64_t es = gs + e * W;
        if (es >= lo && es + W <= hi) {
          *reinterpret_cast<E*>(dst + e * W) = *reinterpret_cast<const E*>(src + e * W);
        }
      }
    }
  }
}

template <int W, int B>
struct Batch {
  using E = typename ElemT<W>::type;
  static constexpr int R = 16 / W;
  uint32_t bits[B];
  uint32_t zbits[B];
  uint32_t rank[B];
  E v[B][R];
};

template <int R, bool EMIT>
__device__ __forceinline__ void select_words(uint64_t Ew, uint32_t p, uint64_t Zw,
                                             int widx_base, int lane, uint64_t* wE, uint32_t* wp,
                                             uint64_t* wZ) {
  constexpr int kLanesPerWord = 64 / R;
  const int q_mine = lane / kLanesPerWord;
  uint64_t e = 0, z = 0;
  uint32_t pp = 0;
#pragma unroll
  for (int q = 0; q < R; ++q) {
    const int src = widx_base + q;
    const uint32_t lo = __builtin_amdgcn_readlane(static_cast<uint32_t>(Ew), src);
    const uint32_t hi = __builtin_amdgcn_readlane(static_cast<uint32_t>(Ew >> 32), src);
    const uint32_t pq = __builtin_amdgcn_readlane(p, src);
    uint64_t zq = 0;
    if constexpr (EMIT) {
      const uint32_t zlo = __builtin_amdgcn_readlane(static_cast<uint32_t>(Zw), src);
      const uint32_t zhi = __builtin_amdgcn_readlane(static_cast<uint32_t>(Zw >> 32), src);
      zq = (static_cast<uint64_t>(zhi) << 32) | zlo;
    }
    if (q == q_mine) {
      e = (static_cast<uint64_t>(hi) << 32) | lo;
      pp = pq;
      z = zq;
    }
  }
  *wE = e;
  *wp = pp;
  *wZ = z;
}

struct TileCtx {
  uint64_t Ew, Zw;
  uint32_t p;
  int lane;
  int64_t tile_row0;
  const uint8_t* values;
  __amdgpu_buffer_rsrc_t rsrc;
};

template <int W, bool IOTA, bool EMIT, bool ALIGNED, int B>
__device__ __forceinline__ void issue_batch(const TileCtx& c, int j0, Batch<W, B>& b) {
  using E = typename ElemT<W>::type;
  constexpr int R = 16 / W;
  constexpr int kRowsPerIter = kWave * R;
#pragma unroll
  for (int i = 0; i < B; ++i) {
    const int j = j0 + i;
    const int row_in_tile = j * kRowsPerIter + c.lane * R;
    const int bpos = row_in_tile & 63;
    uint64_t wE, wZ;
    uint32_t wp;
    select_words<R, EMIT>(c.Ew, c.p, c.Zw, j * R, c.lane, &wE, &wp, &wZ);
    b.bits[i] = static_cast<uint32_t>(wE >> bpos) & ((1u << R) - 1u);
    b.zbits[i] = static_cast<uint32_t>(wZ >> bpos) & ((1u << R) - 1u);
    b.rank[i] = wp + __popcll(wE & low_mask64(bpos));
    if constexpr (IOTA) {
#pragma unroll
      for (int r = 0; r < R; ++r) b.v[i][r] = static_cast<E>(c.tile_row0 + row_in_tile + r);
    } else {
      const int64_t row = c.tile_row0 + row_in_tile;
      const uint8_t* src = c.values + row * static_cast<int64_t>(W);
      if constexpr (ALIGNED) {
        const uint32_t voff = b.bits[i] != 0 ? static_cast<uint32_t>(row_in_tile * W) : kBufferSkip;
        const uint4 q = (kSelNt & 1) ? buffer_load_b128_nt(c.rsrc, voff) : buffer_load_b128(c.rsrc, voff);
        if constexpr (W == 16) {
          b.v[i][0] = q;
        } else {
          const E* qe = reinterpret_cast<const E*>(&q);
#pragma unroll
          for (int r = 0; r < R; ++r) b.v[i][r] = qe[r];
        }
      } else {
#pragma unroll
        for (int r = 0; r < R; ++r) {
          b.v[i][r] = zero_elem<W>();
          if ((b.bits[i] >> r) & 1u) {
            if constexpr (W == 16) {
              const uint64_t* s64 = reinterpret_cast<const uint64_t*>(src + r * W);
              const uint64_t lo64 = s64[0], hi64 = s64[1];
              b.v[i][r] = make_uint4(static_cast<uint32_t>(lo64), static_cast<uint32_t>(lo64 >> 32),
                                     static_cast<uint32_t>(hi64), static_cast<uint32_t>(hi64 >> 32));
            } else {
              b.v[i][r] = *reinterpret_cast<const E*>(src + r * W);
            }
          }
        }
      }
    }
  }
}

template <int W, int B, int RING>
__device__ __forceinline__ void consume_batch(const Batch<W, B>& b, uint8_t* ring, int64_t a0) {
  using E = typename ElemT<W>::type;
  constexpr int R = 16 / W;
#pragma unroll
  for (int i = 0; i < B; ++i) {
    if (b.bits[i] != 0) {
      uint32_t rk = b.rank[i];
#pragma unroll
      for (int r = 0; r < R; ++r) {
        if ((b.bits[i] >> r) & 1u) {
          E e = b.v[i][r];
          if ((b.zbits[i] >> r) & 1u) e = zero_elem<W>();
          const int ro = static_cast<int>((a0 + static_cast<int64_t>(rk) * W) & (RING - 1));
          *reinterpret_cast<E*>(ring + ro) = e;
          ++rk;
        }
      }
    }
  }
}

template <int W, bool IOTA, bool EMIT, bool ALIGNED, int B, bool PIPE>
__global__ __launch_bounds__(kBlock) void compact_kernel(CompactArgs a) {
  using E = typename ElemT<W>::type;
  constexpr int R = 16 / W;
  constexpr int kRowsPerIter = kWave * R;
  constexpr int kIters = kTileRows / kRowsPerIter;
  constexpr int kWordsPerIter = kRowsPerIter / 64;
  constexpr int kBatches = kIters / B;
  constexpr int RING = (B <= 2) ? 4096 : 8192;
  static_assert(kIters % B == 0, "batch must divide the iteration count");
  static_assert(!PIPE || kBatches % 2 == 0, "pipelined form walks the batches in pairs");

  __shared__ CompactLds<RING> lds;

  const int lane = lane_id();
  const int wave = __builtin_amdgcn_readfirstlane(threadIdx.x >> 6);
  const int64_t t = static_cast<int64_t>(blockIdx.x) * kWavesPerBlock + wave;
  if (t >= a.ntiles) return;

  const int64_t w = t * 64 + lane;
  uint64_t mv;
  const uint64_t Ew = emit_word(a.mask, a.mvalid, w, EMIT, a.invert != 0, &mv);
  const uint32_t k = __popcll(Ew);
  const uint32_t incl = wave_inclusive_scan_u32(k);
  const uint32_t p = incl - k;
  const uint32_t total = __shfl(incl, 63, 64);
  if (total == 0) return;

  const int64_t grp = t >> 6;
  const int tin = static_cast<int>(t & 63);
  const uint32_t cprev = lane < tin ? a.tile_counts[grp * kTilesPerGroup + lane] : 0u;
  const int64_t off = a.group_excl[grp] + wave_reduce_sum_u32(cprev);

  uint8_t* ring = lds.ring[wave];
  const int64_t a0 =
      static_cast<int64_t>((reinterpret_cast<uint64_t>(a.out_data) + static_cast<uint64_t>(off) * W) &
                           (kFlushBytes - 1));
  uint8_t* gbase = a.out_data + (off * static_cast<int64_t>(W) - a0);
  int64_t flushed = 0;

  TileCtx c;
  c.Ew = Ew;
  c.Zw = EMIT ? (Ew & ~mv) : 0;
  c.p = p;
  c.lane = lane;
  c.tile_row0 = t * kTileRows;
  c.values = a.values;
  c.rsrc = make_rsrc(IOTA ? nullptr : a.values + c.tile_row0 * static_cast<int64_t>(W),
                     static_cast<uint32_t>(kTileRows * W));

  auto flush_check = [&](int next_batch) {
    const uint32_t cum = next_batch < kBatches
                             ? __builtin_amdgcn_readlane(p, next_batch * B * kWordsPerIter)
                             : total;
    const int64_t written = a0 + static_cast<int64_t>(cum) * W;
    if (written - flushed >= kFlushBytes) {
      wave_lds_sync();
      while (written - flushed >= kFlushBytes) {
        flush_region<W, RING>(ring, gbase, flushed, a0, written, lane);
        flushed += kFlushBytes;
      }
      wave_lds_sync();
    }
  };

  bool tile_done = false;
  if constexpr (IOTA) {
    if (a0 + static_cast<int64_t>(total) * W <= RING) {
      uint64_t m = Ew;
      uint32_t rk = p;
      while (m != 0) {
        const int bpos = __ffsll(static_cast<unsigned long long>(m)) - 1;
        m &= m - 1;
        E val = static_cast<E>(c.tile_row0 + lane * 64 + bpos);
        if constexpr (EMIT) {
          if ((c.Zw >> bpos) & 1ull) val = 0;
        }
        *reinterpret_cast<E*>(ring + a0 + static_cast<int64_t>(rk) * W) = val;
        ++rk;
      }
      tile_done = true;
    }
  }

  if (tile_done) {
  } else if constexpr (PIPE) {
    Batch<W, B> b0, b1;
    issue_batch<W, IOTA, EMIT, ALIGNED, B>(c, 0, b0);
    int jb = 0;
    for (; jb + 2 < kBatches; jb += 2) {
      issue_batch<W, IOTA, EMIT, ALIGNED, B>(c, (jb + 1) * B, b1);
      consume_batch<W, B, RING>(b0, ring, a0);
      flush_check(jb + 1);
      issue_batch<W, IOTA, EMIT, ALIGNED, B>(c, (jb + 2) * B, b0);
      consume_batch<W, B, RING>(b1, ring, a0);
      flush_check(jb + 2);
    }
    issue_batch<W, IOTA, EMIT, ALIGNED, B>(c, (jb + 1) * B, b1);
    consume_batch<W, B, RING>(b0, ring, a0);
    flush_check(jb + 1);
    consume_batch<W, B, RING>(b1, ring, a0);
    flush_check(jb + 2);
  } else {
    for (int jb = 0; jb < kBatches; ++jb) {
      Batch<W, B> b0;
      issue_batch<W, IOTA, EMIT, ALIGNED, B>(c, jb * B, b0);
      consume_batch<W, B, RING>(b0, ring, a0);
      flush_check(jb + 1);
    }
  }

  {
    const int64_t written = a0 + static_cast<int64_t>(total) * W;
    wave_lds_sync();
    while (flushed < written) {
      flush_region<W, RING>(ring, gbase, flushed, a0, written, lane);
      flushed += kFlushBytes;
    }
  }

  if (a.out_validity != nullptr) {
    uint64_t* vb = lds.vbits[wave];
    vb[lane] = 0;
    if (lane < 8) vb[64 + lane] = 0;
    wave_lds_sync();

    const uint64_t vv = load_word(a.vvalid, w);
    const uint64_t Vs = vv & mv;
    uint64_t cbits;
    if (__any((Ew & ~Vs) != 0)) {
      cbits = pext64(Vs, Ew);
    } else {
      cbits = low_mask64(static_cast<int>(k));
    }
    const int64_t obit = (off & 63) + p;
    const int word = static_cast<int>(obit >> 6);
    const int sh = static_cast<int>(obit & 63);
    if (k != 0) {
      atomicOr(reinterpret_cast<unsigned long long*>(&vb[word]),
               static_cast<unsigned long long>(cbits << sh));
      if (sh != 0 && (sh + static_cast<int>(k)) > 64) {
        atomicOr(reinterpret_cast<unsigned long long*>(&vb[word + 1]),
                 static_cast<unsigned long long>(cbits >> (64 - sh)));
      }
    }
    wave_lds_sync();

    const int64_t gw0 = off >> 6;
    const int64_t bit_lo = off;
    const int64_t bit_hi = off + total;
#pragma unroll
    for (int h = 0; h < 2; ++h) {
      const int j = h * 64 + lane;
      if (j <= 64) {
        const int64_t wlo = (gw0 + j) << 6;
        const int64_t whi = wlo + 64;
        if (whi > bit_lo && wlo < bit_hi) {
          const uint64_t val = vb[j];
          if (wlo >= bit_lo && whi <= bit_hi) {
            a.out_validity[gw0 + j] = val;
          } else if (val != 0) {
            atomicOr(reinterpret_cast<unsigned long long*>(&a.out_validity[gw0 + j]),
                     static_cast<unsigned long long>(val));
          }
        }
      }
    }
  }
}


constexpr int kSparseWindow = 1024;
constexpr int kSparseU = 2;

struct __attribute__((aligned(16))) SparseLds {
  uint16_t sel[kWavesPerBlock][kSparseWindow];
  uint64_t vs[kWavesPerBlock][64];
  uint64_t zw[kWavesPerBlock][64];
};

template <int W, bool EMIT, bool IOTA>
__global__ __launch_bounds__(kBlock) void compact_sparse_kernel(CompactArgs a) {
  using E = typename ElemT<W>::type;
  constexpr int U = kSparseU;
  __shared__ SparseLds lds;

  const int lane = lane_id();
  const int wave = __builtin_amdgcn_readfirstlane(threadIdx.x >> 6);
  const int64_t t = static_cast<int64_t>(blockIdx.x) * kWavesPerBlock + wave;
  if (t >= a.ntiles) return;

  const int64_t w = t * 64 + lane;
  uint64_t mv;
  const uint64_t Ew = emit_word(a.mask, a.mvalid, w, EMIT, a.invert != 0, &mv);
  const uint32_t k = __popcll(Ew);
  const uint32_t incl = wave_inclusive_scan_u32(k);
  const uint32_t p = incl - k;
  const int total = static_cast<int>(__shfl(incl, 63, 64));
  if (total == 0) return;

  const int64_t grp = t >> 6;
  const int tin = static_cast<int>(t & 63);
  const uint32_t cprev = lane < tin ? a.tile_counts[grp * kTilesPerGroup + lane] : 0u;
  const int64_t off = a.group_excl[grp] + wave_reduce_sum_u32(cprev);

  uint16_t* sel = lds.sel[wave];
  const bool want_validity = a.out_validity != nullptr;
  if (want_validity) lds.vs[wave][lane] = load_word(a.vvalid, w) & mv;
  if constexpr (EMIT) lds.zw[wave][lane] = Ew & ~mv;

  const E* __restrict__ values = IOTA ? nullptr : reinterpret_cast<const E*>(a.values) + t * kTileRows;
  E* __restrict__ out = reinterpret_cast<E*>(a.out_data);
  const int head = static_cast<int>(off & 63);
  const int nsteps = (head + total + 63) >> 6;
  const int64_t word0 = off >> 6;
  constexpr int kStepsPerWindow = kSparseWindow / 64;

  uint64_t m = Ew;
  uint32_t rk = p;
  for (int step0 = 0; step0 < nsteps; step0 += kStepsPerWindow) {
    const int win_lo = step0 * 64 - head;
    const int win_hi = win_lo + kSparseWindow;
    while (m != 0 && static_cast<int>(rk) < win_hi) {
      const int bpos = __ffsll(static_cast<unsigned long long>(m)) - 1;
      m &= m - 1;
      sel[static_cast<int>(rk) - win_lo] = static_cast<uint16_t>(lane * 64 + bpos);
      ++rk;
    }
    wave_lds_sync();
    const int step_end = (step0 + kStepsPerWindow) < nsteps ? (step0 + kStepsPerWindow) : nsteps;
    const int first_listed = win_lo < 0 ? 0 : win_lo;
    for (int i0 = step0; i0 < step_end; i0 += U) {
      int s[U];
      bool act[U];
      int r[U];
      E v[U];
#pragma unroll
      for (int u = 0; u < U; ++u) {
        s[u] = (i0 + u) * 64 + lane - head;
        act[u] = s[u] >= 0 && s[u] < total && (i0 + u) < step_end;
        r[u] = sel[(act[u] ? s[u] : first_listed) - win_lo];
      }
#pragma unroll
      for (int u = 0; u < U; ++u) {
        if constexpr (IOTA) {
          if constexpr (W <= 8) v[u] = static_cast<E>(t * kTileRows + r[u]);
        } else {
          v[u] = sel_load<W>(values + r[u], (kSelNt & 1) != 0);
        }
      }
#pragma unroll
      for (int u = 0; u < U; ++u) {
        if ((i0 + u) >= step_end) break;
        E e = v[u];
        if constexpr (EMIT) {
          if ((lds.zw[wave][r[u] >> 6] >> (r[u] & 63)) & 1ull) e = zero_elem<W>();
        }
        if (act[u]) sel_store<W>(out + off + s[u], e);
        if (want_validity) {
          const bool vbit = act[u] && ((lds.vs[wave][r[u] >> 6] >> (r[u] & 63)) & 1ull);
          const uint64_t bal = __ballot(vbit);
          const uint64_t owned = __ballot(act[u]);
          if (lane == 0) {
            uint64_t* dst = a.out_validity + word0 + i0 + u;
            if (owned == ~uint64_t(0)) {
              *dst = bal;
            } else if (bal != 0) {
              atomicOr(reinterpret_cast<unsigned long long*>(dst), static_cast<unsigned long long>(bal));
            }
          }
        }
      }
    }
    wave_lds_sync();
  }
}

template <int W>
__global__ __launch_bounds__(kBlock) void expand_kernel(CompactArgs a) {
  using E = typename ElemT<W>::type;
  __shared__ uint64_t words[kWavesPerBlock][64];
  __shared__ uint32_t before[kWavesPerBlock][64];
  const int lane = lane_id();
  const int wave = __builtin_amdgcn_readfirstlane(threadIdx.x >> 6);
  const int64_t t = static_cast<int64_t>(blockIdx.x) * kWavesPerBlock + wave;
  if (t >= a.ntiles) return;
  uint64_t mv;
  const uint64_t mw = emit_word(a.mask, a.mvalid, t * 64 + lane, false, false, &mv);
  const uint32_t k = __popcll(mw);
  const uint32_t incl = wave_inclusive_scan_u32(k);
  words[wave][lane] = mw;
  before[wave][lane] = incl - k;
  const int64_t grp = t >> 6;
  const int tin = static_cast<int>(t & 63);
  const uint32_t cprev = lane < tin ? a.tile_counts[grp * kTilesPerGroup + lane] : 0u;
  const int64_t off = a.group_excl[grp] + wave_reduce_sum_u32(cprev);
  wave_lds_sync();
  const E* __restrict__ dense = reinterpret_cast<const E*>(a.values);
  E* __restrict__ out = reinterpret_cast<E*>(a.out_data);
  const int64_t row0 = t * kTileRows;
  const uint64_t below = lane == 0 ? 0ull : (~0ull >> (64 - lane));
#pragma unroll 4
  for (int j = 0; j < 64; ++j) {
    const int64_t row = row0 + j * 64 + lane;
    if (row >= a.length) break;
    const uint64_t wj = words[wave][j];
    E e = zero_elem<W>();
    if ((wj >> lane) & 1ull) e = dense[off + before[wave][j] + __popcll(wj & below)];
    out[row] = e;
  }
}

template <typename R>
__global__ __launch_bounds__(kBlock) void ree_bool_expand_kernel(const R* __restrict__ run_ends, int64_t num_runs,
                                                                 Bits vsel, Bits vvalid, int64_t logical_offset,
                                                                 int64_t length, uint64_t* __restrict__ out_bits,
                                                                 uint64_t* __restrict__ out_valid) {
  const int64_t nwords = (length + 63) >> 6;
  const int64_t stride = static_cast<int64_t>(gridDim.x) * blockDim.x;
  for (int64_t w = static_cast<int64_t>(blockIdx.x) * blockDim.x + threadIdx.x; w < nwords; w += stride) {
    const int64_t row0 = w << 6;
    const int64_t rows = length - row0 < 64 ? length - row0 : 64;
    const int64_t p0 = logical_offset + row0;
    int64_t lo = 0, hi = num_runs;
    while (lo < hi) {
      const int64_t mid = (lo + hi) >> 1;
      if (static_cast<int64_t>(run_ends[mid]) > p0) hi = mid; else lo = mid + 1;
    }
    uint64_t bits = 0, valid = 0;
    int64_t done = 0;
    for (int64_t r = lo; r < num_runs && done < rows; ++r) {
      const int64_t end = static_cast<int64_t>(run_ends[r]) - p0;
      const int64_t upto = end < rows ? end : rows;
      if (upto > done) {
        const uint64_t span = (upto - done >= 64 ? ~uint64_t(0) : ((uint64_t(1) << (upto - done)) - 1)) << done;
        if ((load_word(vsel, r >> 6) >> (r & 63)) & 1ull) bits |= span;
        if ((load_word(vvalid, r >> 6) >> (r & 63)) & 1ull) valid |= span;
        done = upto;
      }
    }
    out_bits[w] = bits;
    if (out_valid != nullptr) out_valid[w] = valid;
  }
}

struct TakeArgs {
  const uint8_t* values;
  Bits vvalid_unused;
  const uint8_t* src_valid_bytes;
  int64_t src_valid_offset;
  const uint8_t* indices;
  Bits ivalid;
  int64_t length;
  uint8_t* out_data;
  uint64_t* out_validity;
  unsigned long long* valid_count;
};

template <int W, typename IdxT, bool HAS_IV, bool HAS_SV>
__global__ __launch_bounds__(kBlock) void take_kernel(TakeArgs a) {
  using E = typename ElemT<W>::type;
  constexpr int U = 8;
  const int lane = lane_id();
  const int64_t nwaves = static_cast<int64_t>(gridDim.x) * kWavesPerBlock;
  const int64_t wave_g = static_cast<int64_t>(blockIdx.x) * kWavesPerBlock +
                         __builtin_amdgcn_readfirstlane(threadIdx.x >> 6);
  const int64_t nchunks = (a.length + 64 * U - 1) / (64 * U);
  const int64_t last = a.length - 1;
  const IdxT* __restrict__ indices = reinterpret_cast<const IdxT*>(a.indices);
  const E* __restrict__ values = reinterpret_cast<const E*>(a.values);
  E* __restrict__ out = reinterpret_cast<E*>(a.out_data);
  uint64_t nvalid = 0;
  for (int64_t c = wave_g; c < nchunks; c += nwaves) {
    const int64_t base = c * (64 * U);
    int64_t pos[U];
    uint64_t idx[U];
    bool ok[U];
#pragma unroll
    for (int u = 0; u < U; ++u) {
      const int64_t p = base + u * 64 + lane;
      pos[u] = p <= last ? p : last;
      idx[u] = static_cast<uint64_t>((kSelNt & 1) ? nt_load<IdxT>(indices + pos[u]) : indices[pos[u]]);
    }
#pragma unroll
    for (int u = 0; u < U; ++u) {
      ok[u] = (base + u * 64 + lane) <= last;
      if constexpr (HAS_IV) {
        const uint64_t wbits = load_word_nb(a.ivalid, (base >> 6) + u);
        ok[u] = ok[u] && ((wbits >> lane) & 1ull);
      }
    }
    E val[U];
#pragma unroll
    for (int u = 0; u < U; ++u) {
      const E* src = ok[u] ? (values + idx[u]) : (out + pos[u]);
      val[u] = sel_load<W>(src, (kSelNt & 4) != 0);
    }
    if constexpr (HAS_SV) {
      uint8_t vb[U];
#pragma unroll
      for (int u = 0; u < U; ++u) {
        const uint64_t bit = ok[u] ? static_cast<uint64_t>(a.src_valid_offset) + idx[u] : 0;
        vb[u] = a.src_valid_bytes[bit >> 3];
      }
#pragma unroll
      for (int u = 0; u < U; ++u) {
        const uint64_t bit = static_cast<uint64_t>(a.src_valid_offset) + idx[u];
        ok[u] = ok[u] && ((vb[u] >> (bit & 7)) & 1);
      }
    }
#pragma unroll
    for (int u = 0; u < U; ++u) {
      const int64_t p = base + u * 64 + lane;
      if (p <= last) sel_store<W>(out + p, ok[u] ? val[u] : zero_elem<W>());
      const uint64_t vbal = __ballot(ok[u]);
      nvalid += __popcll(vbal);
      if (a.out_validity != nullptr && lane == 0 && (base + u * 64) <= last) {
        a.out_validity[(base >> 6) + u] = vbal;
      }
    }
  }
  if (a.valid_count != nullptr && lane == 0 && nvalid != 0) atomicAdd(a.valid_count, nvalid);
}

template <int UB> struct RowUnit;
template <> struct RowUnit<1> { typedef uint8_t type; };
template <> struct RowUnit<2> { typedef uint16_t type; };
template <> struct RowUnit<4> { typedef uint32_t type; };
template <> struct RowUnit<8> { typedef uint64_t type; };
template <> struct RowUnit<16> { typedef arx_u32x4 type; };

template <int UB, typename IdxT, bool HAS_IV, bool HAS_SV>
__global__ __launch_bounds__(kBlock) void take_rows_kernel(TakeArgs a, uint32_t units_per_row) {
  using E = typename RowUnit<UB>::type;
  const int lane = lane_id();
  const int64_t nwaves = static_cast<int64_t>(gridDim.x) * kWavesPerBlock;
  const int64_t wave_g = static_cast<int64_t>(blockIdx.x) * kWavesPerBlock + __builtin_amdgcn_readfirstlane(threadIdx.x >> 6);
  const int64_t nchunks = (a.length + 63) >> 6;
  const int64_t last = a.length - 1;
  const IdxT* __restrict__ indices = reinterpret_cast<const IdxT*>(a.indices);
  const E* __restrict__ values = reinterpret_cast<const E*>(a.values);
  E* __restrict__ out = reinterpret_cast<E*>(a.out_data);
  uint64_t nvalid = 0;
  for (int64_t c = wave_g; c < nchunks; c += nwaves) {
    const int64_t base = c << 6;
    const int64_t p = base + lane <= last ? base + lane : last;
    uint64_t idx = static_cast<uint64_t>(indices[p]);
    bool ok = base + lane <= last;
    if constexpr (HAS_IV) ok = ok && ((load_word_nb(a.ivalid, base >> 6) >> lane) & 1ull);
    if constexpr (HAS_SV) {
      const uint64_t bit = ok ? static_cast<uint64_t>(a.src_valid_offset) + idx : 0;
      ok = ok && ((a.src_valid_bytes[bit >> 3] >> (bit & 7)) & 1);
    }
    if (!ok) idx = 0;
    const uint64_t vbal = __ballot(ok);
    nvalid += __popcll(vbal);
    if (a.out_validity != nullptr && lane == 0) a.out_validity[base >> 6] = vbal;
    const int rows_here = static_cast<int>(last - base + 1 < 64 ? last - base + 1 : 64);
    const uint32_t total = static_cast<uint32_t>(rows_here) * units_per_row;
    const uint32_t idx_lo = static_cast<uint32_t>(idx), idx_hi = static_cast<uint32_t>(idx >> 32);
    for (uint32_t t = lane; t < ((total + 63u) & ~63u); t += 64) {
      const uint32_t tt = t < total ? t : total - 1;
      const uint32_t row = tt / units_per_row;
      const uint32_t j = tt - row * units_per_row;
      const uint64_t src = (static_cast<uint64_t>(__shfl(idx_hi, static_cast<int>(row), 64)) << 32) | __shfl(idx_lo, static_cast<int>(row), 64);
      const bool row_ok = (vbal >> row) & 1ull;
      E v = E{};
      if (row_ok) v = values[src * units_per_row + j];
      if (t < total) out[(static_cast<uint64_t>(base) + row) * units_per_row + j] = v;
    }
  }
  if (a.valid_count != nullptr && lane == 0 && nvalid != 0) atomicAdd(a.valid_count, nvalid);
}

constexpr int kTakeMaxCols = 16;
struct TakeColsArgs {
  const uint8_t* values[kTakeMaxCols];
  const uint8_t* src_valid_bytes[kTakeMaxCols];
  int64_t src_valid_offset[kTakeMaxCols];
  uint8_t* out_data[kTakeMaxCols];
  uint64_t* out_validity[kTakeMaxCols];
  int width[kTakeMaxCols];
  int num_cols;
  const uint8_t* indices;
  Bits ivalid;
  int64_t length;
  unsigned long long* valid_counts;
};

template <int W, int U>
__device__ __forceinline__ uint64_t take_one_column(const TakeColsArgs& a, int c, const int64_t (&pos)[U],
                                                    const uint64_t (&idx)[U], const bool (&ok0)[U], int64_t base,
                                                    int64_t last, int lane) {
  using E = typename ElemT<W>::type;
  const E* __restrict__ values = reinterpret_cast<const E*>(a.values[c]);
  E* __restrict__ out = reinterpret_cast<E*>(a.out_data[c]);
  const uint8_t* __restrict__ svb = a.src_valid_bytes[c];
  const uint64_t svo = static_cast<uint64_t>(a.src_valid_offset[c]);
  E val[U];
  bool ok[U];
#pragma unroll
  for (int u = 0; u < U; ++u) {
    const E* src = ok0[u] ? (values + idx[u]) : (out + pos[u]);
    val[u] = *src;
    ok[u] = ok0[u];
  }
  if (svb != nullptr) {
    uint8_t vb[U];
#pragma unroll
    for (int u = 0; u < U; ++u) vb[u] = svb[(ok0[u] ? svo + idx[u] : 0) >> 3];
#pragma unroll
    for (int u = 0; u < U; ++u) ok[u] = ok[u] && ((vb[u] >> ((svo + idx[u]) & 7)) & 1);
  }
  uint64_t nvalid = 0;
#pragma unroll
  for (int u = 0; u < U; ++u) {
    const int64_t p = base + u * 64 + lane;
    if (p <= last) out[p] = ok[u] ? val[u] : zero_elem<W>();
    const uint64_t vbal = __ballot(ok[u]);
    nvalid += __popcll(vbal);
    if (a.out_validity[c] != nullptr && lane == 0 && (base + u * 64) <= last) a.out_validity[c][(base >> 6) + u] = vbal;
  }
  return nvalid;
}

template <typename IdxT, bool HAS_IV>
__global__ __launch_bounds__(kBlock) void take_columns_kernel(TakeColsArgs a) {
  constexpr int U = 4;
  const int lane = lane_id();
  const int64_t nwaves = static_cast<int64_t>(gridDim.x) * kWavesPerBlock;
  const int64_t wave_g = static_cast<int64_t>(blockIdx.x) * kWavesPerBlock +
                         __builtin_amdgcn_readfirstlane(threadIdx.x >> 6);
  const int64_t nchunks = (a.length + 64 * U - 1) / (64 * U);
  const int64_t last = a.length - 1;
  const IdxT* __restrict__ indices = reinterpret_cast<const IdxT*>(a.indices);
  uint64_t nvalid[kTakeMaxCols];
  for (int c = 0; c < kTakeMaxCols; ++c) nvalid[c] = 0;
  for (int64_t ch = wave_g; ch < nchunks; ch += nwaves) {
    const int64_t base = ch * (64 * U);
    int64_t pos[U];
    uint64_t idx[U];
    bool ok0[U];
#pragma unroll
    for (int u = 0; u < U; ++u) {
      const int64_t p = base + u * 64 + lane;
      pos[u] = p <= last ? p : last;
      idx[u] = static_cast<uint64_t>(indices[pos[u]]);
    }
#pragma unroll
    for (int u = 0; u < U; ++u) {
      ok0[u] = (base + u * 64 + lane) <= last;
      if constexpr (HAS_IV) {
        const uint64_t wbits = load_word_nb(a.ivalid, (base >> 6) + u);
        ok0[u] = ok0[u] && ((wbits >> lane) & 1ull);
      }
    }
    for (int c = 0; c < a.num_cols; ++c) {
      uint64_t nv;
      switch (a.width[c]) {
        case 1: nv = take_one_column<1, U>(a, c, pos, idx, ok0, base, last, lane); break;
        case 2: nv = take_one_column<2, U>(a, c, pos, idx, ok0, base, last, lane); break;
        case 4: nv = take_one_column<4, U>(a, c, pos, idx, ok0, base, last, lane); break;
        case 8: nv = take_one_column<8, U>(a, c, pos, idx, ok0, base, last, lane); break;
        case 16: nv = take_one_column<16, U>(a, c, pos, idx, ok0, base, last, lane); break;
        default: nv = take_one_column<32, U>(a, c, pos, idx, ok0, base, last, lane); break;
      }
      nvalid[c] += nv;
    }
  }
  if (a.valid_counts != nullptr && lane == 0) {
    for (int c = 0; c < a.num_cols; ++c) {
      if (nvalid[c] != 0) atomicAdd(a.valid_counts + c, nvalid[c]);
    }
  }
}

template <typename IdxT>
__global__ __launch_bounds__(kBlock) void take_bits_kernel(TakeArgs a, int64_t value_bit_offset) {
  const int lane = lane_id();
  const int64_t nwaves = static_cast<int64_t>(gridDim.x) * kWavesPerBlock;
  const int64_t wave_g = static_cast<int64_t>(blockIdx.x) * kWavesPerBlock +
                         __builtin_amdgcn_readfirstlane(threadIdx.x >> 6);
  const int64_t nwords = (a.length + 63) >> 6;
  const int64_t last = a.length - 1;
  const IdxT* __restrict__ indices = reinterpret_cast<const IdxT*>(a.indices);
  uint64_t* __restrict__ out = reinterpret_cast<uint64_t*>(a.out_data);
  uint64_t nvalid = 0;
  for (int64_t w = wave_g; w < nwords; w += nwaves) {
    const int64_t p = (w << 6) + lane;
    const int64_t pc = p <= last ? p : last;
    const uint64_t idx = static_cast<uint64_t>(indices[pc]);
    bool ok = p <= last && ((load_word(a.ivalid, w) >> lane) & 1ull);
    if (ok && a.src_valid_bytes != nullptr) {
      const uint64_t vb = static_cast<uint64_t>(a.src_valid_offset) + idx;
      ok = (a.src_valid_bytes[vb >> 3] >> (vb & 7)) & 1;
    }
    bool bit = false;
    if (ok) {
      const uint64_t b = static_cast<uint64_t>(value_bit_offset) + idx;
      bit = (a.values[b >> 3] >> (b & 7)) & 1;
    }
    const uint64_t data_bal = __ballot(bit);
    const uint64_t valid_bal = __ballot(ok);
    nvalid += __popcll(valid_bal);
    if (lane == 0) {
      out[w] = data_bal;
      if (a.out_validity != nullptr) a.out_validity[w] = valid_bal;
    }
  }
  if (a.valid_count != nullptr && lane == 0 && nvalid != 0) atomicAdd(a.valid_count, nvalid);
}

struct BoundsWs {
  unsigned long long first_bad_pos;
  long long bad_value_signed;
  unsigned long long bad_value_unsigned;
  int64_t pad[5];
};

template <typename IdxT>
__global__ __launch_bounds__(kBlock) void bounds_kernel(const uint8_t* indices, Bits ivalid,
                                                        int64_t length, uint64_t upper,
                                                        BoundsWs* ws) {
  const int64_t stride = static_cast<int64_t>(gridDim.x) * blockDim.x;
  unsigned long long bad = ~0ull;
  for (int64_t i = static_cast<int64_t>(blockIdx.x) * blockDim.x + threadIdx.x; i < length;
       i += stride) {
    const IdxT v = reinterpret_cast<const IdxT*>(indices)[i];
    const bool valid = (load_word(ivalid, i >> 6) >> (i & 63)) & 1ull;
    bool oob;
    if constexpr (std::is_signed<IdxT>::value) {
      oob = v < 0 || static_cast<uint64_t>(v) >= upper;
    } else {
      oob = static_cast<uint64_t>(v) >= upper;
    }
    if (valid && oob) {
      bad = static_cast<unsigned long long>(i);
      break;
    }
  }
  if (bad != ~0ull) atomicMin(&ws->first_bad_pos, bad);
}

template <typename IdxT>
__global__ void bounds_fetch_kernel(const uint8_t* indices, BoundsWs* ws) {
  const unsigned long long pos = ws->first_bad_pos;
  if (pos == ~0ull) return;
  const IdxT v = reinterpret_cast<const IdxT*>(indices)[pos];
  ws->bad_value_signed = static_cast<long long>(v);
  ws->bad_value_unsigned = static_cast<unsigned long long>(v);
}

static int check_mask(const ArxSpan* mask, int null_selection) {
  if (mask == nullptr) {
    set_error("filter mask is NULL");
    return ARX_INVALID;
  }
  if (mask->length < 0 || mask->offset < 0) {
    set_error("negative length/offset");
    return ARX_INVALID;
  }
  if (mask->length > 0 && mask->data == nullptr) {
    set_error("filter mask has no data buffer");
    return ARX_INVALID;
  }
  if (null_selection != ARX_FILTER_DROP && null_selection != ARX_FILTER_EMIT_NULL) {
    set_error("bad null_selection %d", null_selection);
    return ARX_INVALID;
  }
  return ARX_OK;
}

static inline const void* effective_validity(const ArxSpan* s) {
  return (s->null_count != 0) ? s->validity : nullptr;
}

static int launch_count(const ArxSpan* mask, int null_selection, void* ws, size_t ws_bytes,
                        hipStream_t st, int invert = 0, const ArxSpan* values = nullptr) {
  const int rc = check_mask(mask, null_selection);
  if (rc != ARX_OK) return rc;
  const size_t need = arx_filter_workspace_bytes(mask->length);
  if (ws == nullptr || ws_bytes < need) {
    set_error("filter workspace too small: %zu < %zu", ws_bytes, need);
    return ARX_INVALID;
  }
  if ((reinterpret_cast<uint64_t>(ws) & 63) != 0) {
    set_error("filter workspace must be 64-byte aligned");
    return ARX_INVALID;
  }
  FilterWsView v = ws_view(ws, mask->length);
  const int64_t nt = num_tiles(mask->length);
  const int64_t ng = num_groups(mask->length);
  FilterWsHeader h{};
  h.total = 0;
  h.ntiles = nt;
  h.ngroups = ng;
  h.length = mask->length;
  ARX_HIP(hipMemcpyAsync(v.hdr, &h, sizeof(h), hipMemcpyHostToDevice, st));
  if (mask->length == 0) return ARX_OK;
  const Bits mb = make_bits(mask->data, mask->offset, mask->length);
  const Bits mvb = make_bits(effective_validity(mask), mask->offset, mask->length);
  if (values != nullptr) {
    const Bits vvb = make_bits(effective_validity(values), values->offset, mask->length);
    hipLaunchKernelGGL((count_kernel<true>), dim3(static_cast<unsigned>(ng)), dim3(kBlock), 0, st, mb, mvb, vvb,
                       null_selection, invert, nt, v.tile_counts, v.group_total, v.group_valid);
    ARX_CHECK_LAUNCH("count_kernel");
    hipLaunchKernelGGL(scan_kernel, dim3(1), dim3(1024), 0, st, v.group_total, ng, v.group_excl, v.hdr,
                       static_cast<const int64_t*>(v.group_valid));
  } else {
    hipLaunchKernelGGL((count_kernel<false>), dim3(static_cast<unsigned>(ng)), dim3(kBlock), 0, st, mb, mvb, mvb,
                       null_selection, invert, nt, v.tile_counts, v.group_total, static_cast<int64_t*>(nullptr));
    ARX_CHECK_LAUNCH("count_kernel");
    hipLaunchKernelGGL(scan_kernel, dim3(1), dim3(1024), 0, st, v.group_total, ng, v.group_excl, v.hdr,
                       static_cast<const int64_t*>(nullptr));
  }
  ARX_CHECK_LAUNCH("scan_kernel");
  return ARX_OK;
}

static Knob<int> g_filter_batch{4};
static Knob<int> g_filter_pipe{1};
static Knob<int> g_filter_sparse{-1};
static const KnobRow kSelectionKnobs[] = {
    {"filter_batch", g_filter_batch, knob_snap_down<1, 4>},
    {"filter_pipe", g_filter_pipe, knob_bool},
    {"filter_sparse", g_filter_sparse, knob_tri},
};
KnobTable selection_knobs() { return knob_table(kSelectionKnobs); }

template <int W, bool IOTA, bool EMIT, bool ALIGNED>
static void launch_compact_e(const CompactArgs& a, unsigned grid, hipStream_t st) {
  constexpr int kIters = kTileRows / (kWave * (16 / W));
  constexpr int kBig = kIters >= 8 ? 4 : 2;
  if (ALIGNED && g_filter_batch >= 4 && g_filter_pipe) {
    hipLaunchKernelGGL((compact_kernel<W, IOTA, EMIT, ALIGNED, kBig, true>), dim3(grid),
                       dim3(kBlock), 0, st, a);
  } else {
    hipLaunchKernelGGL((compact_kernel<W, IOTA, EMIT, ALIGNED, 1, false>), dim3(grid), dim3(kBlock),
                       0, st, a);
  }
}

template <int W, bool IOTA>
static void launch_compact_w(const CompactArgs& a, unsigned grid, hipStream_t st) {
  const bool aligned = IOTA || a.values_aligned16 != 0;
  if (a.emit_null) {
    if (aligned) launch_compact_e<W, IOTA, true, true>(a, grid, st);
    else if constexpr (!IOTA) launch_compact_e<W, IOTA, true, false>(a, grid, st);
  } else {
    if (aligned) launch_compact_e<W, IOTA, false, true>(a, grid, st);
    else if constexpr (!IOTA) launch_compact_e<W, IOTA, false, false>(a, grid, st);
  }
}

template <int W, bool IOTA = false>
static void launch_sparse_w(const CompactArgs& a, unsigned grid, hipStream_t st) {
  if (a.emit_null) {
    hipLaunchKernelGGL((compact_sparse_kernel<W, true, IOTA>), dim3(grid), dim3(kBlock), 0, st, a);
  } else {
    hipLaunchKernelGGL((compact_sparse_kernel<W, false, IOTA>), dim3(grid), dim3(kBlock), 0, st, a);
  }
}

static int launch_compact(bool iota, int W, const CompactArgs& a, hipStream_t st,
                          int64_t out_length = -1) {
  const unsigned grid = static_cast<unsigned>(ceil_div(a.ntiles, kWavesPerBlock));
  const int filter_sparse = g_filter_sparse;
  const bool sparse = !iota && !a.invert &&
                      (filter_sparse == 1 ||
                       (filter_sparse < 0 &&
                        (W >= 8 || (out_length >= 0 && out_length * 4 <= a.length))));
  if (iota && !a.invert && filter_sparse != 0 && (W == 2 || W == 4 || W == 8)) {
    if (W == 2) launch_sparse_w<2, true>(a, grid, st);
    else if (W == 4) launch_sparse_w<4, true>(a, grid, st);
    else launch_sparse_w<8, true>(a, grid, st);
    ARX_CHECK_LAUNCH("compact_sparse_kernel<IOTA>");
    return ARX_OK;
  }
  if (sparse) {
    switch (W) {
      case 1: launch_sparse_w<1>(a, grid, st); break;
      case 2: launch_sparse_w<2>(a, grid, st); break;
      case 4: launch_sparse_w<4>(a, grid, st); break;
      case 8: launch_sparse_w<8>(a, grid, st); break;
      case 16: launch_sparse_w<16>(a, grid, st); break;
      case 32: launch_sparse_w<32>(a, grid, st); break;
      default:
        set_error("unsupported byte width %d for the gfx950 filter", W);
        return ARX_NOT_IMPLEMENTED;
    }
    ARX_CHECK_LAUNCH("compact_sparse_kernel");
    return ARX_OK;
  }
  if (iota) {
    switch (W) {
      case 2: launch_compact_w<2, true>(a, grid, st); break;
      case 4: launch_compact_w<4, true>(a, grid, st); break;
      default:
        set_error("unsupported index width %d", W);
        return ARX_NOT_IMPLEMENTED;
    }
  } else {
    switch (W) {
      case 1: launch_compact_w<1, false>(a, grid, st); break;
      case 2: launch_compact_w<2, false>(a, grid, st); break;
      case 4: launch_compact_w<4, false>(a, grid, st); break;
      case 8: launch_compact_w<8, false>(a, grid, st); break;
      case 16: launch_compact_w<16, false>(a, grid, st); break;
      default:
        set_error("unsupported byte width %d for the gfx950 filter", W);
        return ARX_NOT_IMPLEMENTED;
    }
  }
  ARX_CHECK_LAUNCH("compact_kernel");
  return ARX_OK;
}

static int compact_form(bool iota, int W, bool values_aligned16, bool invert, int64_t length, int64_t out_length) {
  const int filter_sparse = g_filter_sparse;
  if (iota) {
    if (!invert && filter_sparse != 0 && (W == 2 || W == 4 || W == 8)) return ARX_COMPACT_GATHER;
    if (W != 2 && W != 4) return ARX_NOT_IMPLEMENTED;
  } else {
    const bool sparse = !invert && (filter_sparse == 1 ||
                                    (filter_sparse < 0 && (W >= 8 || (out_length >= 0 && out_length * 4 <= length))));
    if (sparse) return W == 1 || W == 2 || W == 4 || W == 8 || W == 16 || W == 32 ? ARX_COMPACT_GATHER : ARX_NOT_IMPLEMENTED;
    if (W != 1 && W != 2 && W != 4 && W != 8 && W != 16) return ARX_NOT_IMPLEMENTED;
  }
  if (!iota && !values_aligned16) return ARX_COMPACT_SWEEP_UNALIGNED;
  return g_filter_batch >= 4 && g_filter_pipe ? ARX_COMPACT_SWEEP_PIPELINED : ARX_COMPACT_SWEEP_PLAIN;
}

static int zero_out_validity(void* out_validity, int64_t out_length, hipStream_t st) {
  if (out_validity == nullptr) return ARX_OK;
  if ((reinterpret_cast<uint64_t>(out_validity) & 7) != 0) {
    set_error("out_validity must be 8-byte aligned");
    return ARX_INVALID;
  }
  if (out_length < 0) {
    set_error("out_length (from arx_filter_count) is required when out_validity is given");
    return ARX_INVALID;
  }
  if (out_length > 0) {
    ARX_HIP(hipMemsetAsync(out_validity, 0, static_cast<size_t>(ceil_div(out_length, 64)) * 8, st));
  }
  return ARX_OK;
}

size_t selection_workspace_bytes(int64_t length) { return arx_filter_workspace_bytes(length); }

int selection_bit_positions(const void* bitmap, int64_t bit_offset, int64_t length, bool invert,
                            void* ws, size_t ws_bytes, uint32_t* out, int64_t* out_count_host,
                            hipStream_t st) {
  ArxSpan m{};
  m.validity = nullptr;
  m.data = bitmap;
  m.offset = bit_offset;
  m.length = length;
  m.null_count = 0;
  int rc = launch_count(&m, ARX_FILTER_DROP, ws, ws_bytes, st, invert ? 1 : 0);
  if (rc != ARX_OK) return rc;
  int64_t total = 0;
  ARX_HIP(hipMemcpyAsync(&total, ws, sizeof(int64_t), hipMemcpyDeviceToHost, st));
  ARX_HIP(hipStreamSynchronize(st));
  *out_count_host = total;
  if (total == 0) return ARX_OK;
  FilterWsView v = ws_view(ws, length);
  CompactArgs a{};
  a.values = nullptr;
  a.mask = make_bits(bitmap, bit_offset, length);
  a.mvalid = make_bits(nullptr, 0, length);
  a.vvalid = make_bits(nullptr, 0, length);
  a.length = length;
  a.ntiles = num_tiles(length);
  a.tile_counts = v.tile_counts;
  a.group_excl = v.group_excl;
  a.out_data = reinterpret_cast<uint8_t*>(out);
  a.out_validity = nullptr;
  a.emit_null = 0;
  a.invert = invert ? 1 : 0;
  a.values_aligned16 = 1;
  return launch_compact(true, 4, a, st);
}

}

using namespace arx;

extern "C" {

size_t arx_filter_workspace_bytes(int64_t length) {
  if (length < 0) length = 0;
  const int64_t ng = num_groups(length);
  return static_cast<size_t>(64 + ng * 16 + ng * kTilesPerGroup * 4 + ng * 8 + 64);
}

int arx_filter_count_async(const ArxSpan* mask, int null_selection, void* ws, size_t ws_bytes,
                           void* stream) {
  return launch_count(mask, null_selection, ws, ws_bytes, as_stream(stream));
}

int arx_filter_count_nulls(const ArxSpan* values, const ArxSpan* mask, int null_selection, void* ws, size_t ws_bytes,
                           int64_t* out_length, int64_t* out_null_count, void* stream) {
  if (out_length == nullptr || out_null_count == nullptr || values == nullptr) {
    set_error("values / out_length / out_null_count is NULL");
    return ARX_INVALID;
  }
  if (mask != nullptr && values->length != mask->length) {
    set_error("filter values and mask differ in length (%lld vs %lld)", static_cast<long long>(values->length),
              static_cast<long long>(mask->length));
    return ARX_INVALID;
  }
  hipStream_t st = as_stream(stream);
  const int rc = launch_count(mask, null_selection, ws, ws_bytes, st, 0, values);
  if (rc != ARX_OK) return rc;
  int64_t hdr[5] = {0, 0, 0, 0, 0};
  ARX_HIP(hipMemcpyAsync(hdr, ws, sizeof(hdr), hipMemcpyDeviceToHost, st));
  ARX_HIP(hipStreamSynchronize(st));
  *out_length = hdr[0];
  *out_null_count = mask->length == 0 ? 0 : hdr[0] - hdr[4];
  return ARX_OK;
}

int arx_filter_count(const ArxSpan* mask, int null_selection, void* ws, size_t ws_bytes,
                     int64_t* out_length, void* stream) {
  if (out_length == nullptr) {
    set_error("out_length is NULL");
    return ARX_INVALID;
  }
  hipStream_t st = as_stream(stream);
  const int rc = launch_count(mask, null_selection, ws, ws_bytes, st);
  if (rc != ARX_OK) return rc;
  int64_t total = 0;
  ARX_HIP(hipMemcpyAsync(&total, ws, sizeof(int64_t), hipMemcpyDeviceToHost, st));
  ARX_HIP(hipStreamSynchronize(st));
  *out_length = total;
  return ARX_OK;
}

int arx_filter_exec(const ArxSpan* values, int byte_width, const ArxSpan* mask, int null_selection,
                    const void* ws, int64_t out_length, void* out_data, void* out_validity,
                    void* stream) {
  int rc = check_mask(mask, null_selection);
  if (rc != ARX_OK) return rc;
  if (values == nullptr || ws == nullptr) {
    set_error("values/ws is NULL");
    return ARX_INVALID;
  }
  if (values->length != mask->length) {
    set_error("Array arguments must all be the same length (values %lld vs filter %lld)",
              static_cast<long long>(values->length), static_cast<long long>(mask->length));
    return ARX_INVALID;
  }
  if (mask->length == 0) return ARX_OK;
  if (values->data == nullptr || out_data == nullptr) {
    set_error("values/out data buffer is NULL");
    return ARX_INVALID;
  }
  hipStream_t st = as_stream(stream);
  FilterWsView v = ws_view(const_cast<void*>(ws), mask->length);
  CompactArgs a{};
  a.values = static_cast<const uint8_t*>(values->data) + values->offset * byte_width;
  a.mask = make_bits(mask->data, mask->offset, mask->length);
  a.mvalid = make_bits(effective_validity(mask), mask->offset, mask->length);
  a.vvalid = make_bits(effective_validity(values), values->offset, values->length);
  a.length = mask->length;
  a.ntiles = num_tiles(mask->length);
  a.tile_counts = v.tile_counts;
  a.group_excl = v.group_excl;
  a.out_data = static_cast<uint8_t*>(out_data);
  a.out_validity = static_cast<uint64_t*>(out_validity);
  a.emit_null = null_selection == ARX_FILTER_EMIT_NULL && a.mvalid.base != nullptr;
  a.values_aligned16 = (reinterpret_cast<uint64_t>(a.values) & 15) == 0;
  if ((reinterpret_cast<uint64_t>(out_data) % byte_width) != 0) {
    set_error("out_data is not aligned to the element width");
    return ARX_INVALID;
  }
  rc = zero_out_validity(out_validity, out_length, st);
  if (rc != ARX_OK) return rc;
  return launch_compact(false, byte_width, a, st, out_length);
}

int arx_expand_by_mask(const void* dense, int byte_width, const ArxSpan* mask, const void* ws, void* out_data,
                       void* stream) {
  int rc = check_mask(mask, ARX_FILTER_DROP);
  if (rc != ARX_OK) return rc;
  if (ws == nullptr) {
    set_error("ws is NULL (run arx_filter_count on the mask first)");
    return ARX_INVALID;
  }
  if (mask->length == 0) return ARX_OK;
  if (out_data == nullptr || (reinterpret_cast<uint64_t>(out_data) % byte_width) != 0 ||
      (dense != nullptr && (reinterpret_cast<uint64_t>(dense) % byte_width) != 0)) {
    set_error("expand: NULL or misaligned buffer");
    return ARX_INVALID;
  }
  FilterWsView v = ws_view(const_cast<void*>(ws), mask->length);
  CompactArgs a{};
  a.values = static_cast<const uint8_t*>(dense);
  a.mask = make_bits(mask->data, mask->offset, mask->length);
  a.mvalid = make_bits(effective_validity(mask), mask->offset, mask->length);
  a.length = mask->length;
  a.ntiles = num_tiles(mask->length);
  a.tile_counts = v.tile_counts;
  a.group_excl = v.group_excl;
  a.out_data = static_cast<uint8_t*>(out_data);
  const unsigned grid = static_cast<unsigned>(ceil_div(a.ntiles, kWavesPerBlock));
  hipStream_t st = as_stream(stream);
  switch (byte_width) {
    case 1: hipLaunchKernelGGL((expand_kernel<1>), dim3(grid), dim3(kBlock), 0, st, a); break;
    case 2: hipLaunchKernelGGL((expand_kernel<2>), dim3(grid), dim3(kBlock), 0, st, a); break;
    case 4: hipLaunchKernelGGL((expand_kernel<4>), dim3(grid), dim3(kBlock), 0, st, a); break;
    case 8: hipLaunchKernelGGL((expand_kernel<8>), dim3(grid), dim3(kBlock), 0, st, a); break;
    case 16: hipLaunchKernelGGL((expand_kernel<16>), dim3(grid), dim3(kBlock), 0, st, a); break;
    default:
      set_error("unsupported byte width %d for expand", byte_width);
      return ARX_NOT_IMPLEMENTED;
  }
  ARX_CHECK_LAUNCH("expand_kernel");
  return ARX_OK;
}

int arx_mask_to_indices(const ArxSpan* mask, int null_selection, const void* ws, int64_t out_length,
                        int index_width, void* out_indices, void* out_validity, void* stream) {
  int rc = check_mask(mask, null_selection);
  if (rc != ARX_OK) return rc;
  if (ws == nullptr) {
    set_error("ws is NULL");
    return ARX_INVALID;
  }
  if (index_width != 2 && index_width != 4 && index_width != 8) {
    set_error("index_width must be 2, 4 or 8");
    return ARX_INVALID;
  }
  if (index_width == 8 && (g_filter_sparse == 0 || null_selection == ARX_FILTER_EMIT_NULL)) {
    set_error("index_width 8 is served by the gather form with DROP only");
    return ARX_NOT_IMPLEMENTED;
  }
  if (mask->length > static_cast<int64_t>(UINT32_MAX)) {
    set_error("Filter length exceeds UINT32_MAX, consider a different strategy for selecting elements");
    return ARX_NOT_IMPLEMENTED;
  }
  if (index_width == 2 && mask->length > 65535) {
    set_error("index_width 2 requires length <= 65535");
    return ARX_INVALID;
  }
  if (mask->length == 0) return ARX_OK;
  if (out_indices == nullptr) {
    set_error("out_indices is NULL");
    return ARX_INVALID;
  }
  hipStream_t st = as_stream(stream);
  FilterWsView v = ws_view(const_cast<void*>(ws), mask->length);
  CompactArgs a{};
  a.values = nullptr;
  a.mask = make_bits(mask->data, mask->offset, mask->length);
  a.mvalid = make_bits(effective_validity(mask), mask->offset, mask->length);
  a.vvalid = make_bits(nullptr, 0, mask->length);
  a.length = mask->length;
  a.ntiles = num_tiles(mask->length);
  a.tile_counts = v.tile_counts;
  a.group_excl = v.group_excl;
  a.out_data = static_cast<uint8_t*>(out_indices);
  a.out_validity = static_cast<uint64_t*>(out_validity);
  a.emit_null = null_selection == ARX_FILTER_EMIT_NULL && a.mvalid.base != nullptr;
  a.values_aligned16 = 1;
  const bool emit = a.emit_null != 0;
  if (emit && out_validity == nullptr) {
    set_error("EMIT_NULL with a nullable mask needs out_validity");
    return ARX_INVALID;
  }
  rc = zero_out_validity(out_validity, out_length, st);
  if (rc != ARX_OK) return rc;
  return launch_compact(true, index_width, a, st);
}

int arx_filter_compact_form(int row_numbers, int byte_width, int values_aligned16, int invert, int64_t length,
                            int64_t out_length) {
  return compact_form(row_numbers != 0, byte_width, values_aligned16 != 0, invert != 0, length, out_length);
}

size_t arx_take_workspace_bytes(void) { return sizeof(BoundsWs); }

int arx_check_index_bounds(const ArxSpan* indices, int index_type, uint64_t upper_limit, void* ws,
                           size_t ws_bytes, void* stream) {
  if (indices == nullptr || ws == nullptr || ws_bytes < sizeof(BoundsWs)) {
    set_error("bad arguments to arx_check_index_bounds");
    return ARX_INVALID;
  }
  if (indices->length == 0) return ARX_OK;
  hipStream_t st = as_stream(stream);
  static const int widths[8] = {1, 1, 2, 2, 4, 4, 8, 8};
  if (index_type < 0 || index_type > 7) {
    set_error("Invalid index type for boundschecking");
    return ARX_INVALID;
  }
  const int iw = widths[index_type];
  const uint8_t* idx = static_cast<const uint8_t*>(indices->data) + indices->offset * iw;
  const Bits iv = make_bits(effective_validity(indices), indices->offset, indices->length);
  BoundsWs* bws = static_cast<BoundsWs*>(ws);
  BoundsWs init{};
  init.first_bad_pos = ~0ull;
  ARX_HIP(hipMemcpyAsync(bws, &init, sizeof(init), hipMemcpyHostToDevice, st));
  const int64_t blocks = std::min<int64_t>(ceil_div(indices->length, kBlock), 256 * 8);
  const dim3 grid(static_cast<unsigned>(blocks)), block(kBlock);
#define ARX_BOUNDS(T)                                                                        \
  hipLaunchKernelGGL((bounds_kernel<T>), grid, block, 0, st, idx, iv, indices->length,       \
                     upper_limit, bws);                                                      \
  hipLaunchKernelGGL((bounds_fetch_kernel<T>), dim3(1), dim3(1), 0, st, idx, bws)
  switch (index_type) {
    case ARX_UINT8: ARX_BOUNDS(uint8_t); break;
    case ARX_INT8: ARX_BOUNDS(int8_t); break;
    case ARX_UINT16: ARX_BOUNDS(uint16_t); break;
    case ARX_INT16: ARX_BOUNDS(int16_t); break;
    case ARX_UINT32: ARX_BOUNDS(uint32_t); break;
    case ARX_INT32: ARX_BOUNDS(int32_t); break;
    case ARX_UINT64: ARX_BOUNDS(uint64_t); break;
    default: ARX_BOUNDS(int64_t); break;
  }
#undef ARX_BOUNDS
  ARX_CHECK_LAUNCH("bounds_kernel");
  BoundsWs res{};
  ARX_HIP(hipMemcpyAsync(&res, bws, sizeof(res), hipMemcpyDeviceToHost, st));
  ARX_HIP(hipStreamSynchronize(st));
  if (res.first_bad_pos != ~0ull) {
    const bool is_signed = (index_type & 1) != 0;
    if (is_signed) {
      set_error("Index %lld out of bounds", res.bad_value_signed);
    } else {
      set_error("Index %llu out of bounds", res.bad_value_unsigned);
    }
    return ARX_INDEX_ERROR;
  }
  return ARX_OK;
}

int arx_take(const ArxSpan* values, int byte_width, const ArxSpan* indices, int index_type,
             void* out_data, void* out_validity, int64_t* valid_count, void* stream) {
  if (values == nullptr || indices == nullptr) {
    set_error("values/indices is NULL");
    return ARX_INVALID;
  }
  if (index_type < 0 || index_type > 7) {
    set_error("Unsupported index type %d for take", index_type);
    return ARX_NOT_IMPLEMENTED;
  }
  if (indices->length == 0) return ARX_OK;
  if (out_data == nullptr || indices->data == nullptr) {
    set_error("indices/out data buffer is NULL");
    return ARX_INVALID;
  }
  static const int widths[8] = {1, 1, 2, 2, 4, 4, 8, 8};
  const int iw = widths[index_type];
  hipStream_t st = as_stream(stream);
  TakeArgs a{};
  a.values = static_cast<const uint8_t*>(values->data) + values->offset * byte_width;
  a.src_valid_bytes = static_cast<const uint8_t*>(effective_validity(values));
  a.src_valid_offset = values->offset;
  a.indices = static_cast<const uint8_t*>(indices->data) + indices->offset * iw;
  a.ivalid = make_bits(effective_validity(indices), indices->offset, indices->length);
  a.length = indices->length;
  a.out_data = static_cast<uint8_t*>(out_data);
  a.out_validity = static_cast<uint64_t*>(out_validity);
  a.valid_count = reinterpret_cast<unsigned long long*>(valid_count);
  const bool needs_validity = a.src_valid_bytes != nullptr || a.ivalid.base != nullptr;
  if (needs_validity && out_validity == nullptr) {
    set_error("take: inputs may have nulls but out_validity is NULL");
    return ARX_INVALID;
  }
  const int64_t nchunks = ceil_div(indices->length, 512);
  const int64_t blocks = std::min<int64_t>(ceil_div(nchunks, kWavesPerBlock), 256 * 32);
  const dim3 grid(static_cast<unsigned>(blocks)), block(kBlock);
  const bool has_iv = a.ivalid.base != nullptr;
  const bool has_sv = a.src_valid_bytes != nullptr;
#define ARX_TAKE_V(WW, IT)                                                                     \
  do {                                                                                         \
    if (has_iv && has_sv) hipLaunchKernelGGL((take_kernel<WW, IT, true, true>), grid, block, 0, st, a);        \
    else if (has_iv) hipLaunchKernelGGL((take_kernel<WW, IT, true, false>), grid, block, 0, st, a);            \
    else if (has_sv) hipLaunchKernelGGL((take_kernel<WW, IT, false, true>), grid, block, 0, st, a);            \
    else hipLaunchKernelGGL((take_kernel<WW, IT, false, false>), grid, block, 0, st, a);                       \
  } while (0)
#define ARX_TAKE_W(WW)                      \
  switch (iw) {                             \
    case 1: ARX_TAKE_V(WW, uint8_t); break; \
    case 2: ARX_TAKE_V(WW, uint16_t); break;\
    case 4: ARX_TAKE_V(WW, uint32_t); break;\
    default: ARX_TAKE_V(WW, uint64_t); break;\
  }
  switch (byte_width) {
    case 1: ARX_TAKE_W(1); break;
    case 2: ARX_TAKE_W(2); break;
    case 4: ARX_TAKE_W(4); break;
    case 8: ARX_TAKE_W(8); break;
    case 16: ARX_TAKE_W(16); break;
    case 32: ARX_TAKE_W(32); break;
    default:
      set_error("Unsupported primitive type for take: byte width %d", byte_width);
      return ARX_NOT_IMPLEMENTED;
  }
#undef ARX_TAKE_W
#undef ARX_TAKE_V
  ARX_CHECK_LAUNCH("take_kernel");
  return ARX_OK;
}

int arx_take_rows(const ArxSpan* values, int64_t row_bytes, const ArxSpan* indices, int index_type, void* out_data,
                  void* out_validity, int64_t* valid_count, void* stream) {
  if (values == nullptr || indices == nullptr) {
    set_error("values/indices is NULL");
    return ARX_INVALID;
  }
  if (index_type < 0 || index_type > 7) {
    set_error("Unsupported index type %d for take", index_type);
    return ARX_NOT_IMPLEMENTED;
  }
  if (row_bytes <= 0 || row_bytes > (int64_t(1) << 24)) {
    set_error("arx_take_rows: rows of %lld bytes (1 .. 2^24)", static_cast<long long>(row_bytes));
    return row_bytes < 0 ? ARX_INVALID : ARX_NOT_IMPLEMENTED;
  }
  if (indices->length == 0) return ARX_OK;
  if (out_data == nullptr || indices->data == nullptr) {
    set_error("indices/out data buffer is NULL");
    return ARX_INVALID;
  }
  static const int widths[8] = {1, 1, 2, 2, 4, 4, 8, 8};
  const int iw = widths[index_type];
  TakeArgs a{};
  a.values = static_cast<const uint8_t*>(values->data) + values->offset * row_bytes;
  a.src_valid_bytes = static_cast<const uint8_t*>(effective_validity(values));
  a.src_valid_offset = values->offset;
  a.indices = static_cast<const uint8_t*>(indices->data) + indices->offset * iw;
  a.ivalid = make_bits(effective_validity(indices), indices->offset, indices->length);
  a.length = indices->length;
  a.out_data = static_cast<uint8_t*>(out_data);
  a.out_validity = static_cast<uint64_t*>(out_validity);
  a.valid_count = reinterpret_cast<unsigned long long*>(valid_count);
  const bool has_iv = a.ivalid.base != nullptr, has_sv = a.src_valid_bytes != nullptr;
  if ((has_iv || has_sv) && out_validity == nullptr) {
    set_error("take: inputs may have nulls but out_validity is NULL");
    return ARX_INVALID;
  }
  int ub = 16;
  while (ub > 1 && (row_bytes % ub != 0 || reinterpret_cast<uintptr_t>(a.values) % ub != 0 || reinterpret_cast<uintptr_t>(out_data) % ub != 0)) ub >>= 1;
  const uint32_t upr = static_cast<uint32_t>(row_bytes / ub);
  const int64_t nchunks = ceil_div(indices->length, 64);
  const int64_t blocks = std::min<int64_t>(ceil_div(nchunks, kWavesPerBlock), 256 * 32);
  const dim3 grid(static_cast<unsigned>(blocks)), block(kBlock);
  hipStream_t st = as_stream(stream);
#define ARX_ROWS_V(UB, IT)                                                                                        \
  do {                                                                                                            \
    if (has_iv && has_sv) hipLaunchKernelGGL((take_rows_kernel<UB, IT, true, true>), grid, block, 0, st, a, upr);  \
    else if (has_iv) hipLaunchKernelGGL((take_rows_kernel<UB, IT, true, false>), grid, block, 0, st, a, upr);      \
    else if (has_sv) hipLaunchKernelGGL((take_rows_kernel<UB, IT, false, true>), grid, block, 0, st, a, upr);      \
    else hipLaunchKernelGGL((take_rows_kernel<UB, IT, false, false>), grid, block, 0, st, a, upr);                 \
  } while (0)
#define ARX_ROWS_U(UB)                        \
  switch (iw) {                               \
    case 1: ARX_ROWS_V(UB, uint8_t); break;   \
    case 2: ARX_ROWS_V(UB, uint16_t); break;  \
    case 4: ARX_ROWS_V(UB, uint32_t); break;  \
    default: ARX_ROWS_V(UB, uint64_t); break; \
  }
  switch (ub) {
    case 16: ARX_ROWS_U(16); break;
    case 8: ARX_ROWS_U(8); break;
    case 4: ARX_ROWS_U(4); break;
    case 2: ARX_ROWS_U(2); break;
    default: ARX_ROWS_U(1); break;
  }
#undef ARX_ROWS_U
#undef ARX_ROWS_V
  ARX_CHECK_LAUNCH("take_rows_kernel");
  return ARX_OK;
}

int arx_take_columns(const ArxSpan* columns, const int32_t* byte_widths, int num_columns, const ArxSpan* indices,
                     int index_type, void* const* out_data, void* const* out_validity, int64_t* valid_counts,
                     void* stream) {
  if (columns == nullptr || byte_widths == nullptr || indices == nullptr || out_data == nullptr || out_validity == nullptr) {
    set_error("take_columns: NULL argument");
    return ARX_INVALID;
  }
  if (num_columns < 1 || num_columns > kTakeMaxCols) {
    set_error("take_columns: 1 to %d columns per call (got %d)", kTakeMaxCols, num_columns);
    return ARX_INVALID;
  }
  if (index_type < 0 || index_type > 7) {
    set_error("Unsupported index type %d for take", index_type);
    return ARX_NOT_IMPLEMENTED;
  }
  if (indices->length == 0) return ARX_OK;
  if (indices->data == nullptr) {
    set_error("indices data buffer is NULL");
    return ARX_INVALID;
  }
  static const int widths[8] = {1, 1, 2, 2, 4, 4, 8, 8};
  const int iw = widths[index_type];
  TakeColsArgs a{};
  a.num_cols = num_columns;
  a.indices = static_cast<const uint8_t*>(indices->data) + indices->offset * iw;
  a.ivalid = make_bits(effective_validity(indices), indices->offset, indices->length);
  a.length = indices->length;
  a.valid_counts = reinterpret_cast<unsigned long long*>(valid_counts);
  for (int c = 0; c < num_columns; ++c) {
    const int w = byte_widths[c];
    if (w != 1 && w != 2 && w != 4 && w != 8 && w != 16 && w != 32) {
      set_error("Unsupported primitive type for take: byte width %d", w);
      return ARX_NOT_IMPLEMENTED;
    }
    if (out_data[c] == nullptr) {
      set_error("take_columns: out data buffer of column %d is NULL", c);
      return ARX_INVALID;
    }
    a.width[c] = w;
    a.values[c] = static_cast<const uint8_t*>(columns[c].data) + columns[c].offset * w;
    a.src_valid_bytes[c] = static_cast<const uint8_t*>(effective_validity(&columns[c]));
    a.src_valid_offset[c] = columns[c].offset;
    a.out_data[c] = static_cast<uint8_t*>(out_data[c]);
    a.out_validity[c] = static_cast<uint64_t*>(out_validity[c]);
    if ((a.src_valid_bytes[c] != nullptr || a.ivalid.base != nullptr) && out_validity[c] == nullptr) {
      set_error("take: inputs may have nulls but out_validity is NULL");
      return ARX_INVALID;
    }
  }
  hipStream_t st = as_stream(stream);
  const int64_t nchunks = ceil_div(indices->length, 256);
  const int64_t blocks = std::min<int64_t>(ceil_div(nchunks, kWavesPerBlock), 256 * 32);
  const dim3 grid(static_cast<unsigned>(blocks)), block(kBlock);
  const bool has_iv = a.ivalid.base != nullptr;
#define ARX_TAKEC(IT)                                                                                   \
  do {                                                                                                  \
    if (has_iv) hipLaunchKernelGGL((take_columns_kernel<IT, true>), grid, block, 0, st, a);             \
    else hipLaunchKernelGGL((take_columns_kernel<IT, false>), grid, block, 0, st, a);                   \
  } while (0)
  switch (iw) {
    case 1: ARX_TAKEC(uint8_t); break;
    case 2: ARX_TAKEC(uint16_t); break;
    case 4: ARX_TAKEC(uint32_t); break;
    default: ARX_TAKEC(uint64_t); break;
  }
#undef ARX_TAKEC
  ARX_CHECK_LAUNCH("take_columns_kernel");
  return ARX_OK;
}

int arx_take_bits(const ArxSpan* values, const ArxSpan* indices, int index_type, void* out_bits, void* out_validity,
                  int64_t* valid_count, void* stream) {
  if (values == nullptr || indices == nullptr) {
    set_error("values/indices is NULL");
    return ARX_INVALID;
  }
  if (index_type < 0 || index_type > 7) {
    set_error("Unsupported index type %d for take", index_type);
    return ARX_NOT_IMPLEMENTED;
  }
  if (indices->length == 0) return ARX_OK;
// ... 70 lines not shown
```

### include/arrow_amd.h

```cpp
#ifndef ARROW_AMD_H_
#define ARROW_AMD_H_

#include <stddef.h>
#include <stdint.h>

#ifdef __cplusplus
extern "C" {
#endif

#define ARX_ABI_VERSION 5

typedef enum ArxStatus {
  ARX_OK = 0,
  ARX_OUT_OF_MEMORY = -1,
  ARX_INVALID = -4,
  ARX_CAPACITY_ERROR = -6,
  ARX_INDEX_ERROR = -7,
  ARX_NOT_IMPLEMENTED = -10,
  ARX_DEVICE_ERROR = -100
} ArxStatus;

enum { ARX_FILTER_DROP = 0, ARX_FILTER_EMIT_NULL = 1 };
enum { ARX_SORT_ASCENDING = 0, ARX_SORT_DESCENDING = 1 };
enum { ARX_NULLS_AT_START = 0, ARX_NULLS_AT_END = 1 };

enum {
  ARX_UINT8 = 0, ARX_INT8 = 1, ARX_UINT16 = 2, ARX_INT16 = 3,
  ARX_UINT32 = 4, ARX_INT32 = 5, ARX_UINT64 = 6, ARX_INT64 = 7
};

typedef struct ArxSpan {
  const void* validity;
  const void* data;
  int64_t offset;
  int64_t length;
  int64_t null_count;
} ArxSpan;

const char* arx_last_error(void);
int arx_abi_version(void);
int arx_device_count(void);
int arx_set_option(const char* name, int64_t value);
int arx_get_option(const char* name, int64_t* out_value);
int64_t arx_get_counter(const char* name);


size_t arx_filter_workspace_bytes(int64_t length);

int arx_filter_count(const ArxSpan* mask, int null_selection, void* ws, size_t ws_bytes,
                     int64_t* out_length, void* stream);

int arx_filter_count_nulls(const ArxSpan* values, const ArxSpan* mask, int null_selection, void* ws, size_t ws_bytes,
                           int64_t* out_length, int64_t* out_null_count, void* stream);

int arx_filter_count_async(const ArxSpan* mask, int null_selection, void* ws,
                           size_t ws_bytes, void* stream);

int arx_filter_exec(const ArxSpan* values, int byte_width, const ArxSpan* mask,
                    int null_selection, const void* ws, int64_t out_length, void* out_data,
                    void* out_validity, void* stream);

int arx_mask_to_indices(const ArxSpan* mask, int null_selection, const void* ws,
                        int64_t out_length, int index_width, void* out_indices,
                        void* out_validity, void* stream);

enum { ARX_COMPACT_GATHER = 0, ARX_COMPACT_SWEEP_PIPELINED = 1, ARX_COMPACT_SWEEP_PLAIN = 2, ARX_COMPACT_SWEEP_UNALIGNED = 3 };

int arx_filter_compact_form(int row_numbers, int byte_width, int values_aligned16, int invert,
                            int64_t length, int64_t out_length);

size_t arx_take_workspace_bytes(void);

int arx_check_index_bounds(const ArxSpan* indices, int index_type, uint64_t upper_limit,
                           void* ws, size_t ws_bytes, void* stream);

int arx_take(const ArxSpan* values, int byte_width, const ArxSpan* indices, int index_type,
             void* out_data, void* out_validity, int64_t* valid_count, void* stream);

int arx_take_rows(const ArxSpan* values, int64_t row_bytes, const ArxSpan* indices, int index_type, void* out_data,
                  void* out_validity, int64_t* valid_count, void* stream);

int arx_take_columns(const ArxSpan* columns, const int32_t* byte_widths, int num_columns, const ArxSpan* indices,
                     int index_type, void* const* out_data, void* const* out_validity, int64_t* valid_counts,
                     void* stream);
int arx_take_bits(const ArxSpan* values, const ArxSpan* indices, int index_type, void* out_bits, void* out_validity,
                  int64_t* valid_count, void* stream);

typedef struct ArxBinarySpan {
  const void* validity;
  const int32_t* offsets;
  const void* data;
  int64_t offset;
  int64_t length;
  int64_t null_count;
} ArxBinarySpan;
size_t arx_binary_take_workspace_bytes(int64_t num_indices);
int arx_binary_take_offsets(const ArxBinarySpan* values, const ArxSpan* indices, int index_type, void* ws,
                            size_t ws_bytes, int32_t* out_offsets, void* out_validity, int64_t* valid_count,
                            int64_t* out_total_bytes, void* stream);
int arx_binary_take_data(const ArxBinarySpan* values, int64_t num_indices, const void* ws, size_t ws_bytes,
                         const int32_t* out_offsets, int64_t total_bytes, void* out_data, void* stream);
size_t arx_large_binary_take_workspace_bytes(int64_t num_indices);
int arx_large_binary_take_offsets(const ArxBinarySpan* values, const ArxSpan* indices, int index_type, void* ws,
                                  size_t ws_bytes, int64_t* out_offsets, void* out_validity, int64_t* valid_count,
                                  int64_t* out_total_bytes, void* stream);
int arx_large_binary_take_data(const ArxBinarySpan* values, int64_t num_indices, const void* ws, size_t ws_bytes,
                               const int64_t* out_offsets, int64_t total_bytes, void* out_data, void* stream);

int arx_list_take_data(const ArxBinarySpan* values, int elem_shift, int64_t num_indices, const void* ws, size_t ws_bytes,
                       const int32_t* out_offsets, int64_t total_elements, void* out_data, void* stream);
int arx_large_list_take_data(const ArxBinarySpan* values, int elem_shift, int64_t num_indices, const void* ws,
                             size_t ws_bytes, const int64_t* out_offsets, int64_t total_elements, void* out_data,
                             void* stream);

enum {
  ARX_NUM_INT8 = 0, ARX_NUM_UINT8 = 1, ARX_NUM_INT16 = 2, ARX_NUM_UINT16 = 3, ARX_NUM_INT32 = 4, ARX_NUM_UINT32 = 5,
  ARX_NUM_INT64 = 6, ARX_NUM_UINT64 = 7, ARX_NUM_FLOAT32 = 8, ARX_NUM_FLOAT64 = 9
};

int arx_cast_numeric(const ArxSpan* values, int in_type, int out_type, int allow_int_overflow, int allow_float_truncate,
                     void* ws, size_t ws_bytes, void* out, void* stream);

#define ARX_CMP_EQUAL 0
#define ARX_CMP_NOT_EQUAL 1
#define ARX_CMP_GREATER 2
#define ARX_CMP_GREATER_EQUAL 3
#define ARX_CMP_LESS 4
#define ARX_CMP_LESS_EQUAL 5
int arx_compare_numeric(int op, int num_type, const void* left, const void* left_scalar, const void* right,
                        const void* right_scalar, int64_t length, uint64_t* out_bits, void* stream);

#define ARX_ARITH_ADD 0
#define ARX_ARITH_SUBTRACT 1
#define ARX_ARITH_MULTIPLY 2
int arx_arith_numeric(int op, int checked, int num_type, const void* left, const void* left_scalar,
                      const void* left_validity, int64_t left_offset, const void* right, const void* right_scalar,
                      const void* right_validity, int64_t right_offset, int64_t length, void* out,
                      uint32_t* overflow_flag, void* stream);
int arx_divide_numeric(int checked, int num_type, const void* left, const void* left_scalar, const void* left_validity,
                       int64_t left_offset, const void* right, const void* right_scalar, const void* right_validity,
                       int64_t right_offset, int64_t length, void* out, uint64_t* errors, void* stream);

int arx_buffer_copy(const void* src, void* dst, int64_t nbytes, void* stream);
int arx_bitmap_copy(const void* bits, int64_t bit_offset, int64_t length, void* out,
                    void* stream);
int arx_bitmap_and(const void* left, int64_t left_offset, const void* right,
                   int64_t right_offset, int64_t length, void* out, void* stream);
int arx_bitmap_copy_at(const void* bits, int64_t bit_offset, int64_t length, void* out,
                       int64_t out_bit_offset, void* stream);

typedef struct ArxCopySeg {
  const void* src;
  void* dst;
  uint64_t nbytes;
} ArxCopySeg;
int arx_copy_segments(const ArxCopySeg* segments, int64_t num_segments, uint64_t max_segment_bytes, void* stream);
typedef struct ArxBitSeg {
  const void* src;
  int64_t src_bit_offset;
  void* dst;
  int64_t dst_bit_offset;
  int64_t nbits;
} ArxBitSeg;
int arx_bitmap_copy_segments(const ArxBitSeg* segments, int64_t num_segments, int64_t max_segment_bits, void* stream);
int arx_binary_rebase_offsets(const int32_t* offsets, int64_t length, int32_t base, int32_t* out,
                              void* stream);
int arx_reduce_i64_init(void* acc, void* stream);
int arx_reduce_i64_consume(const ArxSpan* values, void* acc, void* stream);
int arx_coalesce2(int byte_width, const ArxSpan* values, const ArxSpan* fill, const void* fill_scalar, int64_t length,
                  void* out_data, void* out_validity, void* stream);
int arx_reduce_float_minmax(const ArxSpan* values, int num_type, void* acc, void* stream);
size_t arx_sum_float_workspace_bytes(int64_t length, int64_t null_count);
int arx_sum_float(const ArxSpan* values, int num_type, void* ws, size_t ws_bytes, double* out_sum, int64_t* out_count,
                  void* stream);

#define ARX_AND_KLEENE 0
#define ARX_OR_KLEENE 1
int arx_boolean_kleene(int op, const ArxSpan* left, const ArxSpan* right, void* out_data, void* out_validity,
                       void* stream);
int arx_boolean_invert(const void* bits, int64_t bit_offset, int64_t length, void* out, void* stream);
int arx_bytes_to_bitmap(const uint8_t* bytes, int64_t length, void* out_bits, int64_t* set_count, void* stream);
int arx_bitmap_popcount(const void* bits, int64_t bit_offset, int64_t length, void* ws,
                        size_t ws_bytes, int64_t* out_count, void* stream);

int arx_ree_bool_expand(const void* run_ends, int run_end_width, int64_t num_runs, const ArxSpan* values,
                        int64_t logical_offset, int64_t length, void* out_bits, void* out_validity, void* stream);

enum {
  ARX_KEY_UINT64 = 0, ARX_KEY_INT64 = 1, ARX_KEY_UINT32 = 2, ARX_KEY_INT32 = 3,
  ARX_KEY_FLOAT64 = 4, ARX_KEY_FLOAT32 = 5
};
size_t arx_sort_indices_workspace_bytes(int64_t length);
int arx_sort_indices(const ArxSpan* values, int key_type, int order, int null_placement, void* ws,
                     size_t ws_bytes, uint64_t* out_indices, void* stream);
enum { ARX_RANK_MIN = 0, ARX_RANK_MAX = 1, ARX_RANK_FIRST = 2, ARX_RANK_DENSE = 3, ARX_RANK_QUANTILE = 4, ARX_RANK_NORMAL = 5 };
size_t arx_rank_workspace_bytes(int64_t length);
int arx_rank(const ArxSpan* values, int key_type, const uint64_t* sorted_rows, int tiebreaker, void* ws, size_t ws_bytes,
             void* out, void* stream);
int arx_sort_indices_64(const ArxSpan* values, int is_signed, int order, int null_placement,
                        void* ws, size_t ws_bytes, uint64_t* out_indices, void* stream);

int arx_sort_key_histogram(const ArxSpan* values, int is_signed, int order, int bits,
                           uint64_t* out_hist, void* stream);
int arx_sort_partition_by_bins(const ArxSpan* values, int is_signed, int order, int bits,
                               const uint32_t* splitter_bins , int num_parts, void* ws,
                               size_t ws_bytes, uint64_t* out_keys, uint32_t* out_rows,
                               int64_t* out_counts, int64_t* out_num_valid , void* stream);
int arx_bitmap_to_indices(const void* bits, int64_t bit_offset, int64_t length, int invert, void* ws,
                          size_t ws_bytes, uint32_t* out_indices, int64_t* out_count ,
                          void* stream);
typedef struct ArxSortRecord {
  uint32_t key_lo, key_hi;
  uint32_t row;
} ArxSortRecord;
int arx_sort_partition_records(const ArxSpan* values, int is_signed, int order, int null_placement, int bits,
                               const uint32_t* splitter_bins , int num_parts, void* ws, size_t ws_bytes,
                               ArxSortRecord* out_records ,
                               int64_t* out_counts ,
                               int64_t* out_num_valid , void* stream);
int arx_sort_unpack_records(const ArxSortRecord* records, int64_t num_records, const int64_t* block_meta,
                            int num_blocks, int nulls_first, uint64_t* out_keys, int64_t* out_rows,
                            int64_t* out_null_rows, void* stream);
typedef struct ArxSortKeyWindow {
  uint64_t key_min;
  int32_t shift;
  int32_t reserved;
} ArxSortKeyWindow;
int arx_sort_key_range(const ArxSpan* values, int is_signed, int order, uint64_t* out_range, void* stream);
int arx_sort_key_range_sampled(const ArxSpan* values, int is_signed, int order, int sample_shift, uint64_t* out_range, void* stream);
int arx_sort_key_histogram_window(const ArxSpan* values, int is_signed, int order, int bits,
// ... 423 lines not shown
```

Baseline: 304,400 Mrows/s.

## Speculate filter output sizes and write counts to pinned host memory

Filter and indices_nonzero now write the selected count straight into a coherent pinned host slot from the scan kernel. When the last two calls predict the same size class, the output buffer is allocated and a capacity-guarded compaction is queued before the host waits for the count, which removes the count→allocate→launch round trip. Take writes its valid count through a ticket into the host slot instead of doing a memset plus a D2H memcpy. The scan kernel is also rewritten to give each thread a contiguous chunk. A misprediction costs a wasted compaction and a rerun, and correctness now depends on the guarded kernels respecting capacity.

```diff
diff --git a/arrow_amd/_lib.py b/arrow_amd/_lib.py
--- a/arrow_amd/_lib.py
+++ b/arrow_amd/_lib.py
@@ -108,12 +108,16 @@
     "arx_filter_count": (_int, [_span, _int, _p, _sz, C.POINTER(_i64), _p]),
     "arx_filter_count_async": (_int, [_span, _int, _p, _sz, _p]),
     "arx_filter_count_nulls": (_int, [_span, _span, _int, _p, _sz, C.POINTER(_i64), C.POINTER(_i64), _p]),
+    "arx_filter_count_to": (_int, [_span, _span, _int, _p, _sz, _p, _p]),
+    "arx_filter_exec_guarded": (_int, [_span, _int, _span, _int, _p, _i64, _i64, _p, _p, _p]),
+    "arx_mask_to_indices_guarded": (_int, [_span, _int, _p, _i64, _int, _p, _p, _p]),
     "arx_filter_exec": (_int, [_span, _int, _span, _int, _p, _i64, _p, _p, _p]),
     "arx_mask_to_indices": (_int, [_span, _int, _p, _i64, _int, _p, _p, _p]),
     "arx_filter_compact_form": (_int, [_int, _int, _int, _int, _i64, _i64]),
     "arx_take_workspace_bytes": (_sz, []),
     "arx_check_index_bounds": (_int, [_span, _int, _u64, _p, _sz, _p]),
     "arx_take": (_int, [_span, _int, _span, _int, _p, _p, _p, _p]),
+    "arx_take_counted": (_int, [_span, _int, _span, _int, _p, _p, _p, _p, _p]),
     "arx_take_rows": (_int, [_span, _i64, _span, _int, _p, _p, _p, _p]),
     "arx_take_bits": (_int, [_span, _span, _int, _p, _p, _p, _p]),
     "arx_binary_take_workspace_bytes": (_sz, [_i64]),
diff --git a/arrow_amd/csrc/arrow_plugin.cc b/arrow_amd/csrc/arrow_plugin.cc
--- a/arrow_amd/csrc/arrow_plugin.cc
+++ b/arrow_amd/csrc/arrow_plugin.cc
@@ -574,6 +574,12 @@
 void arrow_amd_plugin_set_string_key_hash_bits(int64_t bits) { g_string_key_hash_bits.store(bits < 0 ? 0 : (bits > 64 ? 64 : bits)); }
 int64_t arrow_amd_plugin_string_key_hash_collisions(void) { return g_string_key_hash_collisions.load(); }
 void arrow_amd_plugin_set_filter_morsel_rows(int64_t n) { g_filter_morsel_rows.store(n); }
+void arrow_amd_plugin_set_speculative_sizes(int on) { g_speculative_sizes.store(on != 0); }
+void arrow_amd_plugin_speculation_stats(int64_t* hits, int64_t* misses, int64_t* reruns) {
+  if (hits != nullptr) *hits = g_speculation_hits.load();
+  if (misses != nullptr) *misses = g_speculation_misses.load();
+  if (reruns != nullptr) *reruns = g_speculation_reruns.load();
+}
 void arrow_amd_plugin_set_parquet_device_snappy(int on) { g_parquet_device_snappy.store(on != 0); }
 void arrow_amd_plugin_set_parquet_device_levels(int on) { g_parquet_device_levels.store(on != 0); }
 void arrow_amd_plugin_set_parquet_pinned_staging(int on) { g_parquet_pinned_staging.store(on != 0); }
diff --git a/arrow_amd/csrc/plugin/common.inc b/arrow_amd/csrc/plugin/common.inc
--- a/arrow_amd/csrc/plugin/common.inc
+++ b/arrow_amd/csrc/plugin/common.inc
@@ -3,6 +3,11 @@
 std::atomic<int64_t> g_stock_calls{0};
 std::atomic<int64_t> g_min_rows{1 << 16};
 std::atomic<int64_t> g_min_rows_streaming{INT64_MAX};
+std::atomic<bool> g_speculative_sizes{[] {
+  const char* env = std::getenv("ARROW_AMD_SPECULATIVE_SIZES");
+  return env == nullptr || std::strtoll(env, nullptr, 10) != 0;
+}()};
+std::atomic<int64_t> g_speculation_hits{0}, g_speculation_misses{0}, g_speculation_reruns{0};
 std::atomic<int64_t> g_filter_morsel_rows{[] {
   const char* env = std::getenv("ARROW_AMD_FILTER_MORSEL_ROWS");
   return env != nullptr ? static_cast<int64_t>(std::strtoll(env, nullptr, 10)) : int64_t(1) << 20;
@@ -113,6 +118,8 @@
     for (auto& s : slots_) {
       if (s.ptr) (void)hipFree(s.ptr);
     }
+    if (host_slot_) (void)hipHostFree(host_slot_);
+    if (take_ticket_) (void)hipFree(take_ticket_);
   }
   hipStream_t PeekStream() const { return stream_; }
   Status Stream(hipStream_t* out) {
@@ -138,11 +145,46 @@
     *out = s.ptr;
     return Status::OK();
   }
+  Status HostSlot(int64_t** out) {
+    if (!host_slot_) {
+      void* p = nullptr;
+#ifdef ARX_EMULATED_HIP_RUNTIME
+      HIP_RETURN_NOT_OK(hipHostMalloc(&p, 64, hipHostMallocDefault));
+#else
+      HIP_RETURN_NOT_OK(hipHostMalloc(&p, 64, hipHostMallocCoherent));
+#endif
+      host_slot_ = static_cast<int64_t*>(p);
+      std::memset(host_slot_, 0, 64);
+    }
+    *out = host_slot_;
+    return Status::OK();
+  }
+  Status Event(hipEvent_t* out) {
+    if (!event_) HIP_RETURN_NOT_OK(hipEventCreateWithFlags(&event_, hipEventDisableTiming));
+    *out = event_;
+    return Status::OK();
+  }
+  Status TakeTicket(void** out) {
+    if (!take_ticket_) {
+      hipStream_t st;
+      ARROW_RETURN_NOT_OK(Stream(&st));
+      void* p = nullptr;
+      HIP_RETURN_NOT_OK(hipMalloc(&p, 256));
+      HIP_RETURN_NOT_OK(hipMemsetAsync(p, 0, 256, st));
+      HIP_RETURN_NOT_OK(hipStreamSynchronize(st));
+      take_ticket_ = p;
+    }
+    *out = take_ticket_;
+    return Status::OK();
+  }
 
  private:
   struct Slot { void* ptr = nullptr; size_t size = 0; };
   std::vector<Slot> slots_;
   hipStream_t stream_ = nullptr;
+  int64_t* host_slot_ = nullptr;
+  void* take_ticket_ = nullptr;
+  hipEvent_t event_ = nullptr;
 };
 thread_local DeviceScratch t_scratch;
 
diff --git a/arrow_amd/csrc/plugin/selection.inc b/arrow_amd/csrc/plugin/selection.inc
--- a/arrow_amd/csrc/plugin/selection.inc
+++ b/arrow_amd/csrc/plugin/selection.inc
@@ -61,6 +61,47 @@
                                                   &vals, filter.offset, n, d_bits, d_valid, st)));
   *dm = ArxSpan{d_valid, d_bits, 0, n, may_have_nulls ? arrow::kUnknownNullCount : 0};
   return Status::OK();
+}
+
+struct SizeHistory {
+  int64_t selected[2] = {0, 0};
+  int64_t rows[2] = {1, 1};
+  int seen = 0;
+
+  void Record(int64_t sel, int64_t n) {
+    if (n <= 0) return;
+    selected[0] = selected[1];
+    rows[0] = rows[1];
+    selected[1] = sel;
+    rows[1] = n;
+    if (seen < 2) ++seen;
+  }
+  static int64_t Scaled(int64_t sel, int64_t of, int64_t n) {
+    return static_cast<int64_t>((static_cast<__int128>(sel) * n + of - 1) / of);
+  }
+  size_t Predict(int64_t n, int width, int64_t* expected_rows) const {
+    if (seen < 2 || n <= 0 || !g_speculative_sizes.load()) return 0;
+    const int64_t r0 = Scaled(selected[0], rows[0], n), r1 = Scaled(selected[1], rows[1], n);
+    const size_t c0 = DevicePool::SizeClass(static_cast<size_t>(std::max<int64_t>(r0, 1)) * width);
+    const size_t c1 = DevicePool::SizeClass(static_cast<size_t>(std::max<int64_t>(r1, 1)) * width);
+    if (c0 != c1) return 0;
+    *expected_rows = r1;
+    return c1;
+  }
+};
+thread_local SizeHistory t_filter_sizes, t_nonzero_sizes;
+
+bool SpeculationAccepted(int64_t total, int64_t capacity_rows, size_t block, int width) {
+  if (total > capacity_rows) {
+    g_speculation_misses.fetch_add(1, std::memory_order_relaxed);
+    return false;
+  }
+  if (block > 2 * DevicePool::SizeClass(static_cast<size_t>(std::max<int64_t>(total, 1)) * width)) {
+    g_speculation_reruns.fetch_add(1, std::memory_order_relaxed);
+    return false;
+  }
+  g_speculation_hits.fetch_add(1, std::memory_order_relaxed);
+  return true;
 }
 
 Status FilterExec(cp::KernelContext* ctx, const cp::ExecSpan& batch, cp::ExecResult* out) {
@@ -152,14 +193,48 @@
       CountGpu(kFnFilter);
       return Status::OK();
     }
-    int64_t out_len = 0, out_nulls = 0;
-    if (allocate_validity) {
-      ARROW_RETURN_NOT_OK(FromArx(arx_filter_count_nulls(&dv, &dm, null_sel, ws, ws_bytes, &out_len, &out_nulls, st)));
+    int64_t* slot = nullptr;
+    ARROW_RETURN_NOT_OK(t_scratch.HostSlot(&slot));
+    ARROW_RETURN_NOT_OK(FromArx(arx_filter_count_to(allocate_validity ? &dv : nullptr, &dm, null_sel, ws, ws_bytes, slot, st)));
+    out_arr->buffers.resize(2);
+    int64_t expected_rows = 0;
+    const size_t block = ree ? 0 : t_filter_sizes.Predict(filter.length, w, &expected_rows);
+    if (block != 0) {
+      const int64_t capacity_rows = static_cast<int64_t>(block / w);
+      hipEvent_t counted;
+      ARROW_RETURN_NOT_OK(t_scratch.Event(&counted));
+      HIP_RETURN_NOT_OK(hipEventRecord(counted, st));
+      ARROW_ASSIGN_OR_RAISE(out_arr->buffers[1], AllocDevice(static_cast<int64_t>(block)));
+      out_arr->buffers[0] = nullptr;
+      void* d_spec_valid = nullptr;
+      if (allocate_validity) {
+        ARROW_ASSIGN_OR_RAISE(out_arr->buffers[0], AllocDevice(((capacity_rows + 63) / 64) * 8));
+        d_spec_valid = reinterpret_cast<void*>(out_arr->buffers[0]->mutable_address());
+      }
+      ARROW_RETURN_NOT_OK(FromArx(arx_filter_exec_guarded(&dv, w, &dm, null_sel, ws, std::min(expected_rows, capacity_rows),
+                                                          capacity_rows, reinterpret_cast<void*>(out_arr->buffers[1]->mutable_address()),
+                                                          d_spec_valid, st)));
+      HIP_RETURN_NOT_OK(hipEventSynchronize(counted));
+      const int64_t total = slot[0], valid = slot[1];
+      t_filter_sizes.Record(total, filter.length);
+      if (SpeculationAccepted(total, capacity_rows, block, w)) {
+        out_arr->length = total;
+        out_arr->null_count = allocate_validity ? total - valid : 0;
+        static_cast<RocmBuffer*>(out_arr->buffers[1].get())->Shrink(total * w);
+        if (allocate_validity) static_cast<RocmBuffer*>(out_arr->buffers[0].get())->Shrink(((total + 63) / 64) * 8);
+        HIP_RETURN_NOT_OK(hipStreamSynchronize(st));
+        CountGpu(kFnFilter);
+        return Status::OK();
+      }
+      out_arr->buffers[0] = nullptr;
+      out_arr->buffers[1] = nullptr;
     } else {
-      ARROW_RETURN_NOT_OK(FromArx(arx_filter_count(&dm, null_sel, ws, ws_bytes, &out_len, st)));
-    }
+      HIP_RETURN_NOT_OK(hipStreamSynchronize(st));
+      if (!ree) t_filter_sizes.Record(slot[0], filter.length);
+    }
+    const int64_t out_len = slot[0];
+    const int64_t out_nulls = allocate_validity ? out_len - slot[1] : 0;
     out_arr->length = out_len;
-    out_arr->buffers.resize(2);
     ARROW_ASSIGN_OR_RAISE(out_arr->buffers[1], AllocDevice(out_len * w));
     out_arr->buffers[0] = nullptr;
     void* d_valid = nullptr;
@@ -459,21 +534,22 @@
     out_arr->buffers[0] = nullptr;
     void* d_valid = nullptr;
     void* d_counter = nullptr;
+    int64_t* slot = nullptr;
     if (allocate_validity) {
       ARROW_ASSIGN_OR_RAISE(out_arr->buffers[0], AllocDevice(((m + 63) / 64) * 8));
       d_valid = reinterpret_cast<void*>(out_arr->buffers[0]->mutable_address());
-      ARROW_RETURN_NOT_OK(t_scratch.Get(kCounter, 64, &d_counter));
-      HIP_RETURN_NOT_OK(hipMemsetAsync(d_counter, 0, 8, st));
-    }
-    ARROW_RETURN_NOT_OK(FromArx(arx_take(&dv, w, &di, tid,
-                                         reinterpret_cast<void*>(out_arr->buffers[1]->mutable_address()), d_valid,
-                                         static_cast<int64_t*>(d_counter), st)));
-    int64_t valid_count = m;
-    if (allocate_validity) {
-      HIP_RETURN_NOT_OK(hipMemcpyAsync(&valid_count, d_counter, 8, hipMemcpyDeviceToHost, st));
+      ARROW_RETURN_NOT_OK(t_scratch.TakeTicket(&d_counter));
+      ARROW_RETURN_NOT_OK(t_scratch.HostSlot(&slot));
+      ARROW_RETURN_NOT_OK(FromArx(arx_take_counted(&dv, w, &di, tid,
+                                                   reinterpret_cast<void*>(out_arr->buffers[1]->mutable_address()), d_valid,
+                                                   d_counter, slot + 2, st)));
+    } else {
+      ARROW_RETURN_NOT_OK(FromArx(arx_take(&dv, w, &di, tid,
+                                           reinterpret_cast<void*>(out_arr->buffers[1]->mutable_address()), d_valid,
+                                           nullptr, st)));
     }
     HIP_RETURN_NOT_OK(hipStreamSynchronize(st));
-    out_arr->null_count = m - valid_count;
+    out_arr->null_count = allocate_validity ? m - slot[2] : 0;
     CountGpu(kFnTake);
     return Status::OK();
   }
diff --git a/arrow_amd/csrc/plugin/vector_hash.inc b/arrow_amd/csrc/plugin/vector_hash.inc
--- a/arrow_amd/csrc/plugin/vector_hash.inc
+++ b/arrow_amd/csrc/plugin/vector_hash.inc
@@ -339,7 +339,40 @@
   void* ws = nullptr;
   ARROW_RETURN_NOT_OK(t_scratch.Get(kWs, ws_bytes, &ws));
   int64_t cnt = 0;
-  if (n > 0) ARROW_RETURN_NOT_OK(FromArx(arx_filter_count(&dm, ARX_FILTER_DROP, ws, ws_bytes, &cnt, st)));
+  if (n > 0) {
+    int64_t* slot = nullptr;
+    ARROW_RETURN_NOT_OK(t_scratch.HostSlot(&slot));
+    ARROW_RETURN_NOT_OK(FromArx(arx_filter_count_to(nullptr, &dm, ARX_FILTER_DROP, ws, ws_bytes, slot, st)));
+    int64_t expected_rows = 0;
+    const size_t block = t_nonzero_sizes.Predict(n, 8, &expected_rows);
+    bool queued = false;
+    if (block != 0) {
+      const int64_t capacity_rows = static_cast<int64_t>(block / 8);
+      hipEvent_t counted;
+      ARROW_RETURN_NOT_OK(t_scratch.Event(&counted));
+      HIP_RETURN_NOT_OK(hipEventRecord(counted, st));
+      ARROW_ASSIGN_OR_RAISE(auto spec_values, AllocDevice(static_cast<int64_t>(block)));
+      queued = arx_mask_to_indices_guarded(&dm, ARX_FILTER_DROP, ws, capacity_rows, 8,
+                                           reinterpret_cast<void*>(spec_values->mutable_address()), nullptr, st) == ARX_OK;
+      if (queued) {
+        HIP_RETURN_NOT_OK(hipEventSynchronize(counted));
+        cnt = slot[0];
+        t_nonzero_sizes.Record(cnt, n);
+        if (SpeculationAccepted(cnt, capacity_rows, block, 8)) {
+          static_cast<RocmBuffer*>(spec_values.get())->Shrink(std::max<int64_t>(cnt, 1) * 8);
+          HIP_RETURN_NOT_OK(hipStreamSynchronize(st));
+          CountGpu(kFnFilter);
+          out->value = ArrayData::Make(arrow::uint64(), cnt, {nullptr, std::move(spec_values)}, 0);
+          return Status::OK();
+        }
+      }
+    }
+    if (!queued) {
+      HIP_RETURN_NOT_OK(hipStreamSynchronize(st));
+      cnt = slot[0];
+      t_nonzero_sizes.Record(cnt, n);
+    }
+  }
   void* d_idx = nullptr;
   ARROW_RETURN_NOT_OK(t_scratch.Get(kArg2, static_cast<size_t>(cnt) * 4 + 64, &d_idx));
   ARROW_ASSIGN_OR_RAISE(auto out_values, AllocDevice(std::max<int64_t>(cnt, 1) * 8));
diff --git a/arrow_amd/csrc/selection.hip b/arrow_amd/csrc/selection.hip
--- a/arrow_amd/csrc/selection.hip
+++ b/arrow_amd/csrc/selection.hip
@@ -103,46 +103,57 @@
 
 __global__ __launch_bounds__(1024) void scan_kernel(const int64_t* group_total, int64_t ngroups,
                                                     int64_t* group_excl, FilterWsHeader* hdr,
-                                                    const int64_t* group_valid = nullptr) {
+                                                    const int64_t* group_valid, int64_t ntiles, int64_t length,
+                                                    int64_t* host_slot) {
   __shared__ int64_t wave_tot[16];
-  __shared__ int64_t carry_s;
-  __shared__ unsigned long long valid_s;
+  __shared__ int64_t wave_valid[16];
   const int tid = threadIdx.x;
   const int lane = tid & 63;
   const int wave = tid >> 6;
-  if (tid == 0) carry_s = 0;
-  if (tid == 0) valid_s = 0;
+  const int64_t per = (ngroups + 1023) / 1024;
+  const int64_t lo = tid * per < ngroups ? tid * per : ngroups;
+  const int64_t hi = lo + per < ngroups ? lo + per : ngroups;
+  int64_t mine = 0, vmine = 0;
+  for (int64_t i = lo; i < hi; ++i) mine += group_total[i];
+  if (group_valid != nullptr) {
+    for (int64_t i = lo; i < hi; ++i) vmine += group_valid[i];
+  }
+  int64_t x = mine;
+#pragma unroll
+  for (int d = 1; d < 64; d <<= 1) {
+    const int64_t n = __shfl_up(x, d, 64);
+    if (lane >= d) x += n;
+  }
+#pragma unroll
+  for (int d = 32; d >= 1; d >>= 1) vmine += __shfl_xor(vmine, d, 64);
+  if (lane == 63) wave_tot[wave] = x;
+  if (lane == 0) wave_valid[wave] = vmine;
   __syncthreads();
-  if (group_valid != nullptr) {
-    int64_t mine = 0;
-    for (int64_t i = tid; i < ngroups; i += 1024) mine += group_valid[i];
-#pragma unroll
-    for (int d = 32; d >= 1; d >>= 1) mine += __shfl_xor(mine, d, 64);
-    if (lane == 0 && mine != 0) atomicAdd(&valid_s, static_cast<unsigned long long>(mine));
-    __syncthreads();
-  }
-  for (int64_t base = 0; base < ngroups; base += 1024) {
-    const int64_t i = base + tid;
-    const int64_t v = i < ngroups ? group_total[i] : 0;
-    int64_t x = v;
-#pragma unroll
-    for (int d = 1; d < 64; d <<= 1) {
-      const int64_t n = __shfl_up(x, d, 64);
-      if (lane >= d) x += n;
-    }
-    if (lane == 63) wave_tot[wave] = x;
-    __syncthreads();
-    int64_t wave_prefix = 0;
-    for (int k = 0; k < wave; ++k) wave_prefix += wave_tot[k];
-    const int64_t carry = carry_s;
-    if (i < ngroups) group_excl[i] = carry + wave_prefix + x - v;
-    __syncthreads();
-    if (tid == 1023) carry_s = carry + wave_prefix + x;
-    __syncthreads();
+  int64_t wave_prefix = 0, carry_s = 0, valid_s = 0;
+  for (int k = 0; k < 16; ++k) {
+    if (k < wave) wave_prefix += wave_tot[k];
+    carry_s += wave_tot[k];
+    valid_s += wave_valid[k];
+  }
+  int64_t run = wave_prefix + x - mine;
+  for (int64_t i = lo; i < hi; ++i) {
+    group_excl[i] = run;
+    run += group_total[i];
   }
   if (tid == 0) {
-    hdr->total = carry_s;
-    hdr->valid = static_cast<int64_t>(valid_s);
+    const int64_t total = carry_s;
+    const int64_t valid = valid_s;
+    hdr->total = total;
+    hdr->ntiles = ntiles;
+    hdr->ngroups = ngroups;
+    hdr->length = length;
+    hdr->valid = valid;
+    hdr->pad[0] = hdr->pad[1] = hdr->pad[2] = 0;
+    if (host_slot != nullptr) {
+      host_slot[0] = total;
+      host_slot[1] = valid;
+      __builtin_amdgcn_fence(__ATOMIC_RELEASE, "");
+    }
   }
 }
 
@@ -160,7 +171,13 @@
   int emit_null;
   int invert;
   int values_aligned16;
+  const int64_t* total = nullptr;
+  int64_t capacity_rows = -1;
 };
+
+__device__ __forceinline__ bool compact_guard_trips(const CompactArgs& a) {
+  return a.capacity_rows >= 0 && *a.total > a.capacity_rows;
+}
 
 constexpr int kFlushBytes = 2048;
 
@@ -392,6 +409,7 @@
   const int wave = __builtin_amdgcn_readfirstlane(threadIdx.x >> 6);
   const int64_t t = static_cast<int64_t>(blockIdx.x) * kWavesPerBlock + wave;
   if (t >= a.ntiles) return;
+  if (compact_guard_trips(a)) return;
 
   const int64_t w = t * 64 + lane;
   uint64_t mv;
@@ -564,6 +582,7 @@
   const int wave = __builtin_amdgcn_readfirstlane(threadIdx.x >> 6);
   const int64_t t = static_cast<int64_t>(blockIdx.x) * kWavesPerBlock + wave;
   if (t >= a.ntiles) return;
+  if (compact_guard_trips(a)) return;
 
   const int64_t w = t * 64 + lane;
   uint64_t mv;
@@ -730,7 +749,10 @@
   uint8_t* out_data;
   uint64_t* out_validity;
   unsigned long long* valid_count;
+  unsigned long long* count_ticket;
+  int64_t* host_count;
 };
+constexpr int kTakeTicketShift = 44;
 
 template <int W, typename IdxT, bool HAS_IV, bool HAS_SV>
 __global__ __launch_bounds__(kBlock) void take_kernel(TakeArgs a) {
@@ -794,6 +816,23 @@
         a.out_validity[(base >> 6) + u] = vbal;
       }
     }
+  }
+  if (a.count_ticket != nullptr) {
+    __shared__ unsigned long long block_valid;
+    if (threadIdx.x == 0) block_valid = 0;
+    __syncthreads();
+    if (lane == 0 && nvalid != 0) atomicAdd(&block_valid, static_cast<unsigned long long>(nvalid));
+    __syncthreads();
+    if (threadIdx.x == 0) {
+      const unsigned long long mine = block_valid + (1ull << kTakeTicketShift);
+      const unsigned long long before = atomicAdd(a.count_ticket, mine);
+      if ((before >> kTakeTicketShift) == gridDim.x - 1) {
+        a.host_count[0] = static_cast<int64_t>((before + mine) & ((1ull << kTakeTicketShift) - 1));
+        *a.count_ticket = 0;
+        __builtin_amdgcn_fence(__ATOMIC_RELEASE, "");
+      }
+    }
+    return;
   }
   if (a.valid_count != nullptr && lane == 0 && nvalid != 0) atomicAdd(a.valid_count, nvalid);
 }
@@ -1051,7 +1090,7 @@
 }
 
 static int launch_count(const ArxSpan* mask, int null_selection, void* ws, size_t ws_bytes,
-                        hipStream_t st, int invert = 0, const ArxSpan* values = nullptr) {
+                        hipStream_t st, int invert = 0, const ArxSpan* values = nullptr, int64_t* host_slot = nullptr) {
   const int rc = check_mask(mask, null_selection);
   if (rc != ARX_OK) return rc;
   const size_t need = arx_filter_workspace_bytes(mask->length);
@@ -1066,13 +1105,12 @@
   FilterWsView v = ws_view(ws, mask->length);
   const int64_t nt = num_tiles(mask->length);
   const int64_t ng = num_groups(mask->length);
-  FilterWsHeader h{};
-  h.total = 0;
-  h.ntiles = nt;
-  h.ngroups = ng;
-  h.length = mask->length;
-  ARX_HIP(hipMemcpyAsync(v.hdr, &h, sizeof(h), hipMemcpyHostToDevice, st));
-  if (mask->length == 0) return ARX_OK;
+  if (mask->length == 0) {
+    hipLaunchKernelGGL(scan_kernel, dim3(1), dim3(1024), 0, st, v.group_total, ng, v.group_excl, v.hdr,
+                       static_cast<const int64_t*>(nullptr), nt, mask->length, host_slot);
+    ARX_CHECK_LAUNCH("scan_kernel");
+    return ARX_OK;
+  }
   const Bits mb = make_bits(mask->data, mask->offset, mask->length);
   const Bits mvb = make_bits(effective_validity(mask), mask->offset, mask->length);
   if (values != nullptr) {
@@ -1081,13 +1119,13 @@
                        null_selection, invert, nt, v.tile_counts, v.group_total, v.group_valid);
     ARX_CHECK_LAUNCH("count_kernel");
     hipLaunchKernelGGL(scan_kernel, dim3(1), dim3(1024), 0, st, v.group_total, ng, v.group_excl, v.hdr,
-                       static_cast<const int64_t*>(v.group_valid));
+                       static_cast<const int64_t*>(v.group_valid), nt, mask->length, host_slot);
   } else {
     hipLaunchKernelGGL((count_kernel<false>), dim3(static_cast<unsigned>(ng)), dim3(kBlock), 0, st, mb, mvb, mvb,
                        null_selection, invert, nt, v.tile_counts, v.group_total, static_cast<int64_t*>(nullptr));
     ARX_CHECK_LAUNCH("count_kernel");
     hipLaunchKernelGGL(scan_kernel, dim3(1), dim3(1024), 0, st, v.group_total, ng, v.group_excl, v.hdr,
-                       static_cast<const int64_t*>(nullptr));
+                       static_cast<const int64_t*>(nullptr), nt, mask->length, host_slot);
   }
   ARX_CHECK_LAUNCH("scan_kernel");
   return ARX_OK;
@@ -1275,6 +1313,20 @@
   return launch_count(mask, null_selection, ws, ws_bytes, as_stream(stream));
 }
 
+int arx_filter_count_to(const ArxSpan* values, const ArxSpan* mask, int null_selection, void* ws, size_t ws_bytes,
+                        int64_t* host_slot, void* stream) {
+  if (host_slot == nullptr) {
+    set_error("host_slot is NULL");
+    return ARX_INVALID;
+  }
+  if (values != nullptr && mask != nullptr && values->length != mask->length) {
+    set_error("filter values and mask differ in length (%lld vs %lld)", static_cast<long long>(values->length),
+              static_cast<long long>(mask->length));
+    return ARX_INVALID;
+  }
+  return launch_count(mask, null_selection, ws, ws_bytes, as_stream(stream), 0, values, host_slot);
+}
+
 int arx_filter_count_nulls(const ArxSpan* values, const ArxSpan* mask, int null_selection, void* ws, size_t ws_bytes,
                            int64_t* out_length, int64_t* out_null_count, void* stream) {
   if (out_length == nullptr || out_null_count == nullptr || values == nullptr) {
@@ -1313,9 +1365,9 @@
   return ARX_OK;
 }
 
-int arx_filter_exec(const ArxSpan* values, int byte_width, const ArxSpan* mask, int null_selection,
-                    const void* ws, int64_t out_length, void* out_data, void* out_validity,
-                    void* stream) {
+static int filter_exec_impl(const ArxSpan* values, int byte_width, const ArxSpan* mask, int null_selection,
+                            const void* ws, int64_t out_length, int64_t capacity_rows, void* out_data, void* out_validity,
+                            void* stream) {
   int rc = check_mask(mask, null_selection);
   if (rc != ARX_OK) return rc;
   if (values == nullptr || ws == nullptr) {
@@ -1351,9 +1403,30 @@
     set_error("out_data is not aligned to the element width");
     return ARX_INVALID;
   }
-  rc = zero_out_validity(out_validity, out_length, st);
+  if (capacity_rows >= 0) {
+    a.total = &v.hdr->total;
+    a.capacity_rows = capacity_rows;
+  }
+  rc = zero_out_validity(out_validity, capacity_rows >= 0 ? capacity_rows : out_length, st);
   if (rc != ARX_OK) return rc;
   return launch_compact(false, byte_width, a, st, out_length);
+}
+
+int arx_filter_exec(const ArxSpan* values, int byte_width, const ArxSpan* mask, int null_selection,
+                    const void* ws, int64_t out_length, void* out_data, void* out_validity,
+                    void* stream) {
+  return filter_exec_impl(values, byte_width, mask, null_selection, ws, out_length, -1, out_data, out_validity, stream);
+}
+
+int arx_filter_exec_guarded(const ArxSpan* values, int byte_width, const ArxSpan* mask, int null_selection,
+                            const void* ws, int64_t expected_length, int64_t capacity_rows, void* out_data,
+                            void* out_validity, void* stream) {
+  if (capacity_rows < 0 || expected_length < 0) {
+    set_error("arx_filter_exec_guarded: negative capacity_rows / expected_length");
+    return ARX_INVALID;
+  }
+  return filter_exec_impl(values, byte_width, mask, null_selection, ws, expected_length, capacity_rows, out_data,
+                          out_validity, stream);
 }
 
 int arx_expand_by_mask(const void* dense, int byte_width, const ArxSpan* mask, const void* ws, void* out_data,
@@ -1396,8 +1469,9 @@
   return ARX_OK;
 }
 
-int arx_mask_to_indices(const ArxSpan* mask, int null_selection, const void* ws, int64_t out_length,
-                        int index_width, void* out_indices, void* out_validity, void* stream) {
+static int mask_to_indices_impl(const ArxSpan* mask, int null_selection, const void* ws, int64_t out_length,
+                                int64_t capacity_rows, int index_width, void* out_indices, void* out_validity,
+                                void* stream) {
   int rc = check_mask(mask, null_selection);
   if (rc != ARX_OK) return rc;
   if (ws == nullptr) {
@@ -1445,9 +1519,28 @@
     set_error("EMIT_NULL with a nullable mask needs out_validity");
     return ARX_INVALID;
   }
-  rc = zero_out_validity(out_validity, out_length, st);
+  if (capacity_rows >= 0) {
+    a.total = &v.hdr->total;
+    a.capacity_rows = capacity_rows;
+  }
+  rc = zero_out_validity(out_validity, capacity_rows >= 0 ? capacity_rows : out_length, st);
   if (rc != ARX_OK) return rc;
   return launch_compact(true, index_width, a, st);
+}
+
+int arx_mask_to_indices(const ArxSpan* mask, int null_selection, const void* ws, int64_t out_length,
+                        int index_width, void* out_indices, void* out_validity, void* stream) {
+  return mask_to_indices_impl(mask, null_selection, ws, out_length, -1, index_width, out_indices, out_validity, stream);
+}
+
+int arx_mask_to_indices_guarded(const ArxSpan* mask, int null_selection, const void* ws, int64_t capacity_rows,
+                                int index_width, void* out_indices, void* out_validity, void* stream) {
+  if (capacity_rows < 0) {
+    set_error("arx_mask_to_indices_guarded: negative capacity_rows");
+    return ARX_INVALID;
+  }
+  return mask_to_indices_impl(mask, null_selection, ws, capacity_rows, capacity_rows, index_width, out_indices,
+                              out_validity, stream);
 }
 
 int arx_filter_compact_form(int row_numbers, int byte_width, int values_aligned16, int invert, int64_t length,
@@ -1510,8 +1603,9 @@
   return ARX_OK;
 }
 
-int arx_take(const ArxSpan* values, int byte_width, const ArxSpan* indices, int index_type,
-             void* out_data, void* out_validity, int64_t* valid_count, void* stream) {
+static int take_impl(const ArxSpan* values, int byte_width, const ArxSpan* indices, int index_type,
+                     void* out_data, void* out_validity, int64_t* valid_count, void* count_ticket, int64_t* host_count,
+                     void* stream) {
   if (values == nullptr || indices == nullptr) {
     set_error("values/indices is NULL");
     return ARX_INVALID;
@@ -1538,6 +1632,8 @@
   a.out_data = static_cast<uint8_t*>(out_data);
   a.out_validity = static_cast<uint64_t*>(out_validity);
   a.valid_count = reinterpret_cast<unsigned long long*>(valid_count);
+  a.count_ticket = static_cast<unsigned long long*>(count_ticket);
+  a.host_count = host_count;
   const bool needs_validity = a.src_valid_bytes != nullptr || a.ivalid.base != nullptr;
   if (needs_validity && out_validity == nullptr) {
     set_error("take: inputs may have nulls but out_validity is NULL");
@@ -1577,6 +1673,26 @@
 #undef ARX_TAKE_V
   ARX_CHECK_LAUNCH("take_kernel");
   return ARX_OK;
+}
+
+int arx_take(const ArxSpan* values, int byte_width, const ArxSpan* indices, int index_type,
+             void* out_data, void* out_validity, int64_t* valid_count, void* stream) {
+  return take_impl(values, byte_width, indices, index_type, out_data, out_validity, valid_count, nullptr, nullptr, stream);
+}
+
+int arx_take_counted(const ArxSpan* values, int byte_width, const ArxSpan* indices, int index_type, void* out_data,
+                     void* out_validity, void* count_ticket, int64_t* host_valid_count, void* stream) {
+  if (count_ticket == nullptr || host_valid_count == nullptr || (reinterpret_cast<uint64_t>(count_ticket) & 7) != 0) {
+    set_error("arx_take_counted: count_ticket (8-byte aligned) and host_valid_count are required");
+    return ARX_INVALID;
+  }
+  if (indices != nullptr && (indices->length >> kTakeTicketShift) != 0) {
+    set_error("arx_take_counted: more than 2^44 indices");
+    return ARX_NOT_IMPLEMENTED;
+  }
+  if (indices != nullptr && indices->length == 0) *host_valid_count = 0;
+  return take_impl(values, byte_width, indices, index_type, out_data, out_validity, nullptr, count_ticket,
+                   host_valid_count, stream);
 }
 
 int arx_take_rows(const ArxSpan* values, int64_t row_bytes, const ArxSpan* indices, int index_type, void* out_data,
diff --git a/include/arrow_amd.h b/include/arrow_amd.h
--- a/include/arrow_amd.h
+++ b/include/arrow_amd.h
@@ -56,10 +56,19 @@
 int arx_filter_count_async(const ArxSpan* mask, int null_selection, void* ws,
                            size_t ws_bytes, void* stream);
 
+int arx_filter_count_to(const ArxSpan* values, const ArxSpan* mask, int null_selection, void* ws, size_t ws_bytes,
+                        int64_t* host_slot, void* stream);
+
 int arx_filter_exec(const ArxSpan* values, int byte_width, const ArxSpan* mask,
                     int null_selection, const void* ws, int64_t out_length, void* out_data,
                     void* out_validity, void* stream);
 
+int arx_filter_exec_guarded(const ArxSpan* values, int byte_width, const ArxSpan* mask, int null_selection,
+                            const void* ws, int64_t expected_length, int64_t capacity_rows, void* out_data,
+                            void* out_validity, void* stream);
+int arx_mask_to_indices_guarded(const ArxSpan* mask, int null_selection, const void* ws, int64_t capacity_rows,
+                                int index_width, void* out_indices, void* out_validity, void* stream);
+
 int arx_mask_to_indices(const ArxSpan* mask, int null_selection, const void* ws,
                         int64_t out_length, int index_width, void* out_indices,
                         void* out_validity, void* stream);
@@ -76,6 +85,9 @@
 
 int arx_take(const ArxSpan* values, int byte_width, const ArxSpan* indices, int index_type,
              void* out_data, void* out_validity, int64_t* valid_count, void* stream);
+
+int arx_take_counted(const ArxSpan* values, int byte_width, const ArxSpan* indices, int index_type, void* out_data,
+                     void* out_validity, void* count_ticket, int64_t* host_valid_count, void* stream);
 
 int arx_take_rows(const ArxSpan* values, int64_t row_bytes, const ArxSpan* indices, int index_type, void* out_data,
                   void* out_validity, int64_t* valid_count, void* stream);
```

Result: faster. 309,100 Mrows/s, median of 6 (+1.6%).
